# roeiherz/CanonicalSg2Im

Hardware: AMD Instinct MI355X
Metric: 256x256 images/sec/node (G+D step) (higher is better)
Workload: dtype f32; 1 GPU; BASELINE config C3: COCO-shaped AttSPADE 256x256, batch 16/GPU, 1-30 objects/img, ngf=64 ndf=64, --no_vgg_loss --use_img_disc 0; Sg2Layout GCN + SPADE G + 2-scale PatchGAN D + object-crop D, fwd+bwd+Adam; global_batch=16, parallelism=dp1

## Files before the change

canonicalsg2im_amd/_lib.py:

```python
import ctypes
import os

import torch

_HERE = os.path.dirname(os.path.abspath(__file__))
LIB_PATH = os.environ.get("CSG_HIP_LIB") or os.path.join(_HERE, "libcsg_hip.so")

MAX_TAPS = 16
ACT_NONE, ACT_LEAKY, ACT_TANH = 0, 1, 2

c_i32, c_i64, c_f32, c_f64, c_p = ctypes.c_int32, ctypes.c_int64, ctypes.c_float, ctypes.c_double, ctypes.c_void_p


class ConvDesc(ctypes.Structure):
    _fields_ = [
        ("B", c_i32), ("IHp", c_i32), ("IWp", c_i32), ("Cin", c_i32), ("x_cs", c_i32),
        ("IHv", c_i32), ("IWv", c_i32), ("in_up", c_i32),
        ("OHg", c_i32), ("OWg", c_i32), ("OHf", c_i32), ("OWf", c_i32), ("os", c_i32), ("ooy", c_i32), ("oox", c_i32),
        ("Cout", c_i32), ("y_cs", c_i32),
        ("istride", c_i32), ("ntaps", c_i32), ("wtaps", c_i32),
        ("tap_dy", c_i32 * MAX_TAPS), ("tap_dx", c_i32 * MAX_TAPS), ("tap_w", c_i32 * MAX_TAPS),
        ("act", c_i32), ("slope", c_f32), ("accumulate", c_i32), ("res_gate", c_i32),
    ]

# ... 22 lines not shown
                ("sigma", c_p), ("u_used", c_p), ("v_used", c_p), ("workspace", c_p), ("workspace_bytes", c_i64)]


class SnBwdItem(ctypes.Structure):
    _fields_ = [("dweff", c_p), ("Cout", c_i64), ("Cin", c_i64), ("KH", c_i64), ("KW", c_i64), ("s0", c_i64), ("s1", c_i64),
                ("s2", c_i64), ("s3", c_i64), ("w", c_p), ("u_used", c_p), ("v_used", c_p), ("sigma", c_p), ("dw", c_p),
                ("workspace", c_p), ("workspace_bytes", c_i64)]


class GemmDesc(ctypes.Structure):
    _fields_ = [("M", ctypes.c_int64), ("N", ctypes.c_int64), ("K", ctypes.c_int64),
                ("lda", ctypes.c_int64), ("ldb", ctypes.c_int64), ("ldy", ctypes.c_int64), ("ldg", ctypes.c_int64),
                ("act", ctypes.c_int32), ("slope", ctypes.c_float), ("gate_slope", ctypes.c_float)]


SIGNATURES = {
    "csg_version": (c_i32, []),
    "csg_last_error": (ctypes.c_char_p, []),
    "csg_prof_enable": (c_i32, [c_i32]),
    "csg_prof_reset": (c_i32, []),
    "csg_prof_num_kernels": (c_i32, []),
    "csg_prof_kernel_name": (ctypes.c_char_p, [c_i32]),
    "csg_prof_read": (c_i32, [c_i32, ctypes.POINTER(c_f64), ctypes.POINTER(c_i64), ctypes.POINTER(c_f64)]),
    "csg_embed_fwd": (c_i32, [c_p, c_i64, c_i64, c_p, c_i64, c_i64, c_p, c_i64, c_i64, c_p]),
    "csg_embed_bwd_workspace": (c_i64, [c_i64, c_i64, c_i64]),
    "csg_embed_bwd": (c_i32, [c_p, c_i64, c_i64, c_p, c_i64, c_i64, c_i64, c_i64, c_p, c_p, c_i64, c_p]),
    "csg_real_object_mask": (c_i32, [c_p, c_i64, c_i64, c_i64, c_i64, c_p, c_p]),
    "csg_graph_csr_build": (c_i32, [c_p, c_i64, c_i64, c_i64, c_p, c_p, c_p]),
    "csg_gather_concat_fwd": (c_i32, [c_p, c_p, c_p, c_i64, c_i64, c_i64, c_i64, c_i64, c_p, c_p]),
    "csg_gather_concat_bwd_workspace": (c_i64, [c_i64, c_i64, c_i64, c_i64]),
    "csg_gather_concat_bwd": (c_i32, [c_p, c_p, c_p, c_i64, c_i64, c_i64, c_i64, c_i64, c_p, c_p, c_p, c_i64, c_p]),
    "csg_segment_avg_fwd_workspace": (c_i64, [c_i64, c_i64, c_i64, c_i64]),
    "csg_segment_avg_fwd": (c_i32, [c_p, c_p, c_p, c_p, c_p, c_i64, c_i64, c_i64, c_i64, c_i64, c_p, c_p, c_p, c_p,
                                    c_i64, c_p]),
    "csg_segment_avg_bwd": (c_i32, [c_p, c_p, c_p, c_p, c_p, c_p, c_p, c_p, c_i64, c_i64, c_i64, c_i64, c_i64, c_i32,
                                    c_p, c_p, c_p, c_p]),
    "csg_layout_fwd": (c_i32, [c_p, c_p, c_p, c_p, c_i64, c_i64, c_i64, c_i64, c_i64, c_i64, c_i64, c_i64, c_p, c_i64,
                               c_i64, c_p]),
    "csg_disc_input_fwd": (c_i32, [c_p, c_p, c_p, c_p, c_i64, c_i64, c_i64, c_i64, c_i64, c_i64, c_p, c_i64, c_i64, c_i64,
                                   c_i64, c_p, c_i64, c_p]),
    "csg_layout_bwd_workspace": (c_i64, [c_i64, c_i64, c_i64, c_i64, c_i64, c_i32, c_i32]),
    "csg_layout_bwd": (c_i32, [c_p, c_i64, c_i64, c_p, c_p, c_p, c_i64, c_i64, c_i64, c_i64, c_i64, c_i64, c_i64,
                               c_i64, c_p, c_i32, c_p, c_p, c_p, c_i64, c_p]),
    "csg_layout_bwd_masks": (c_i32, [c_p, c_i64, c_i64, c_p, c_p, c_i64, c_i64, c_i64, c_i64, c_i64, c_i64, c_i64, c_i64,
                                     c_p, c_p, c_i32, c_p]),
    "csg_layout_mass": (c_i32, [c_p, c_p, c_p, c_p, c_i64, c_i64, c_i64, c_i64, c_i64, c_i64, c_p, c_p]),
    "csg_layout_paint": (c_i32, [c_p, c_p, c_p, c_i64, c_p, c_i64, c_i64, c_i64, c_i64, c_i64, c_i64, c_i64, c_p, c_i64,
                                 c_i64, c_p]),
    "csg_conv_fwd_workspace": (c_i64, [ctypes.POINTER(ConvDesc)]),
    "csg_conv_fwd": (c_i32, [ctypes.POINTER(ConvDesc), c_p, c_p, c_p, c_p, c_p, c_p, c_i64, c_p]),
    "csg_conv_bwd_weight_workspace": (c_i64, [ctypes.POINTER(ConvDesc)]),
    "csg_conv_bwd_weight": (c_i32, [ctypes.POINTER(ConvDesc), c_p, c_p, c_p, c_p, c_p, c_i64, c_p]),
    "csg_wino_pack_bytes": (c_i64, [c_i64, c_i64]),
    "csg_wino_pack_weights": (c_i32, [c_p, c_i64, c_i64, c_i64, c_i64, c_i64, c_i64, c_i32, c_p, c_p, c_p]),
    "csg_conv_fwd_multi_workspace": (c_i64, [ctypes.POINTER(ConvDesc), c_i32]),
    "csg_conv_fwd_multi": (c_i32, [ctypes.POINTER(ConvDesc), c_i32, c_p, c_p, c_p, c_p, c_p, c_p, c_i64, c_p]),
    "csg_gemm_supported": (c_i32, [ctypes.POINTER(GemmDesc)]),
    "csg_gemm_nt": (c_i32, [ctypes.POINTER(GemmDesc), c_p, c_p, c_p, c_p, c_p, c_p]),
    "csg_gemm_tn_workspace": (c_i64, [c_i64, c_i64, c_i64]),
    "csg_gemm_tn": (c_i32, [c_i64, c_i64, c_i64, c_p, c_i64, c_p, c_i64, c_p, c_p, c_p, c_i64, c_p]),
    "csg_conv_few_supported": (c_i32, [ctypes.POINTER(FewDesc)]),
    "csg_conv_few_fwd_workspace": (c_i64, [ctypes.POINTER(FewDesc)]),
    "csg_conv_few_fwd": (c_i32, [ctypes.POINTER(FewDesc), c_p, c_p, c_p, c_p, c_p, c_i64, c_p]),
    "csg_conv_few_bwd_data": (c_i32, [ctypes.POINTER(FewDesc), c_p, c_p, c_p, c_p]),
    "csg_conv_few_bwd_weight_workspace": (c_i64, [ctypes.POINTER(FewDesc)]),
    "csg_conv_few_bwd_weight": (c_i32, [ctypes.POINTER(FewDesc), c_p, c_p, c_p, c_p, c_p, c_i64, c_p]),
    "csg_wino_conv_workspace": (c_i64, [ctypes.POINTER(WinoDesc)]),
    "csg_wino_conv": (c_i32, [ctypes.POINTER(WinoDesc), c_p, c_p, c_p, c_p, c_p, c_f32, c_p, c_p, c_i64, c_p]),
    "csg_wino_bwd_weight_workspace": (c_i64, [ctypes.POINTER(WinoDesc)]),
    "csg_wino_bwd_weight": (c_i32, [ctypes.POINTER(WinoDesc), c_p, c_p, c_p, c_p, c_p, c_i64, c_p]),
    "csg_wino4_bwd_weight_workspace": (c_i64, [ctypes.POINTER(WinoDesc)]),
    "csg_wino4_bwd_weight": (c_i32, [ctypes.POINTER(WinoDesc), c_p, c_p, c_p, c_p, c_p, c_i64, c_p]),
    "csg_wino4_supported": (c_i32, [ctypes.POINTER(WinoDesc)]),
    "csg_wino4_persistent": (c_i32, [c_i32]),
    "csg_wino_pack_weights_multi": (c_i32, [ctypes.POINTER(WinoPackItem), c_i32, c_p]),
    "csg_wino4_pack_bytes": (c_i64, [c_i64, c_i64]),
    "csg_wino4_pack_weights": (c_i32, [c_p, c_i64, c_i64, c_i64, c_i64, c_i64, c_i64, c_i32, c_p, c_p, c_p]),
    "csg_wino4_conv_workspace": (c_i64, [ctypes.POINTER(WinoDesc)]),
    "csg_wino4_conv": (c_i32, [ctypes.POINTER(WinoDesc), c_p, c_p, c_p, c_p, c_p, c_f32, c_p, c_p, c_i64, c_p]),
    "csg_wino4_conv_part": (c_i32, [ctypes.POINTER(WinoDesc), c_p, c_p, c_i64, c_i64, c_p, c_p, c_p, c_i64, c_p, c_p, c_f32,
                                    c_p, c_p]),
    "csg_wino4_conv_spade_supported": (c_i32, [ctypes.POINTER(WinoDesc)]),
    "csg_wino4_conv_spade": (c_i32, [ctypes.POINTER(WinoDesc), c_p, c_p, c_p, c_p, c_p, c_i64, c_p, c_p, c_f32, c_p, c_p]),
    "csg_wino34_supported": (c_i32, [ctypes.POINTER(WinoDesc), c_i32]),
    "csg_wino34_pack_weights": (c_i32, [c_p, c_i64, c_i64, c_i64, c_i64, c_i64, c_i64, c_i32, c_p, c_p, c_p]),
    "csg_wino34_conv_workspace": (c_i64, [ctypes.POINTER(WinoDesc), c_i32]),
    "csg_wino34_conv": (c_i32, [ctypes.POINTER(WinoDesc), c_i32, c_p, c_p, c_p, c_p, c_p, c_f32, c_p, c_p, c_i64, c_p]),
    "csg_act_bwd": (c_i32, [c_p, c_p, c_i64, c_i32, c_f32, c_p, c_p]),
    "csg_colsum": (c_i32, [c_p, c_i64, c_i64, c_i64, c_p, c_p, c_i64, c_p]),
    "csg_norm_stats": (c_i32, [c_p, c_i64, c_i64, c_i64, c_p, c_p, c_i64, c_p]),
    "csg_norm_finalize": (c_i32, [c_p, c_i64, c_i64, c_f64, c_f32, c_i32, c_p, c_p, c_p, c_p, c_f32, c_p]),
    "csg_norm_stats_finalize": (c_i32, [c_p, c_i64, c_i64, c_i64, c_p, c_i64, c_f64, c_f32, c_p, c_p, c_p, c_p, c_p, c_p, c_f32,
                                        c_p]),
    "csg_norm_apply_fwd": (c_i32, [c_p, c_p, c_p, c_p, c_f32, c_i64, c_i64, c_i64, c_p, c_p, c_f32, c_p, c_p]),
    "csg_norm_apply_bwd_reduce": (c_i32, [c_p, c_p, c_p, c_p, c_p, c_p, c_f32, c_i64, c_i64, c_i64, c_p, c_p, c_p, c_i64,
                                          c_i64, c_p]),
    "csg_norm_apply_bwd_dx": (c_i32, [c_p, c_p, c_p, c_p, c_p, c_f32, c_p, c_f64, c_i64, c_i64, c_i64, c_p, c_p, c_p, c_f32,
                                      c_p, c_p, c_i64, c_p]),
    "csg_nearest_resize_fwd": (c_i32, [c_p, c_i64, c_i64, c_i64, c_i64, c_i64, c_i64, c_p, c_p]),
    "csg_nearest_resize_bwd": (c_i32, [c_p, c_i64, c_i64, c_i64, c_i64, c_i64, c_i64, c_p, c_p]),
    "csg_upsample2x_fwd": (c_i32, [c_p, c_i64, c_i64, c_i64, c_i64, c_p, c_p]),
    "csg_upsample2x_bwd": (c_i32, [c_p, c_i64, c_i64, c_i64, c_i64, c_p, c_p]),
    "csg_avgpool3s2_fwd": (c_i32, [c_p, c_i64, c_i64, c_i64, c_i64, c_p, c_p]),
    "csg_avgpool3s2_bwd": (c_i32, [c_p, c_i64, c_i64, c_i64, c_i64, c_p, c_p]),
    "csg_avgpool3s2_bwd_add": (c_i32, [c_p, c_i64, c_i64, c_i64, c_i64, c_p, c_p, c_p]),
    "csg_crop_fwd": (c_i32, [c_p, c_i64, c_i64, c_i64, c_i64, c_i64, c_p, c_p, c_i64, c_i64, c_i64, c_p, c_i64, c_p]),
    "csg_crop_bwd": (c_i32, [c_p, c_i64, c_i64, c_i64, c_i64, c_i64, c_p, c_p, c_i64, c_i64, c_i64, c_i64, c_p, c_p]),
    "csg_crop_bwd_boxes": (c_i32, [c_p, c_p, c_i64, c_i64, c_i64, c_i64, c_i64, c_p, c_p, c_i64, c_i64, c_i64, c_i64, c_p,
                                   c_p]),
    "csg_maxpool2_fwd": (c_i32, [c_p, c_i64, c_i64, c_i64, c_i64, c_p, c_p]),
    "csg_maxpool2_bwd": (c_i32, [c_p, c_p, c_i64, c_i64, c_i64, c_i64, c_p, c_p]),
    "csg_avgpool2_fwd": (c_i32, [c_p, c_i64, c_i64, c_i64, c_i64, c_p, c_p]),
    "csg_avgpool2_bwd": (c_i32, [c_p, c_i64, c_i64, c_i64, c_i64, c_p, c_p]),
    "csg_l1_mean_workspace": (c_i64, [c_i64]),
    "csg_l1_mean_fwd": (c_i32, [c_p, c_p, c_i64, c_p, c_p, c_i64, c_p]),
    "csg_l1_mean_bwd": (c_i32, [c_p, c_p, c_p, c_i64, c_p, c_p]),
    "csg_hinge_mean_fwd": (c_i32, [ctypes.POINTER(HingeItem), c_i32, c_i32, c_p, c_p]),
    "csg_hinge_mean_bwd": (c_i32, [ctypes.POINTER(HingeItem), c_i32, c_i32, c_p, c_p]),
    "csg_spectral_norm_workspace": (c_i64, [c_i64, c_i64]),
    "csg_spectral_norm_fwd": (c_i32, [c_p, c_p, c_p, c_i64, c_i64, c_i32, c_f32, c_p, c_i64, c_p, c_p, c_p, c_p, c_i64,
                                      c_p]),
    "csg_spectral_norm_bwd": (c_i32, [c_p, c_i64, c_i64, c_i64, c_i64, c_i64, c_i64, c_i64, c_i64, c_p, c_p, c_p, c_p,
                                      c_p, c_p, c_i64, c_p]),
    "csg_spectral_norm_fwd_multi": (c_i32, [ctypes.POINTER(SnFwdItem), c_i32, c_i32, c_f32, c_p]),
    "csg_spectral_norm_bwd_multi": (c_i32, [ctypes.POINTER(SnBwdItem), c_i32, c_p]),
    "csg_canon_workspace": (c_i64, [c_i64]),
    "csg_canon_build": (c_i32, [c_p, c_p, c_p, c_p, c_i64, c_i64, ctypes.POINTER(c_i32), c_i64, c_i32, c_i32, c_p, c_i64,
                                c_p, c_p]),
    "csg_canon_emit": (c_i32, [c_p, c_p, c_i64, c_i64, ctypes.POINTER(c_i32), c_i64, c_i32, c_i32, c_p, c_p, c_i64, c_p,
                               c_p, c_p]),
    "csg_canon_converse": (c_i32, [c_p, c_p, c_i64, c_i64, ctypes.POINTER(c_i32), c_i64, c_i32, c_i32, c_p, c_p, c_p, c_p,
                                   c_i64, c_p, c_p, c_p]),
    "csg_canon_general_workspace": (c_i64, [c_i64, c_i64, c_i64]),
    "csg_canon_general_build": (c_i32, [c_p, c_p, c_p, c_p, c_i64, c_i64, c_p, c_p, c_i64, ctypes.POINTER(c_i32), c_i64,
                                        c_i64, c_i32, c_p, c_i64, c_p, c_p]),
    "csg_canon_general_converse": (c_i32, [c_i64, ctypes.POINTER(c_i32), c_i64, c_p, c_i64, c_p, c_p, c_p, c_p, c_p]),
    "csg_canon_general_close": (c_i32, [c_i64, ctypes.POINTER(c_i32), c_i64, c_i32, c_p, c_i64, c_p, c_p]),
    "csg_canon_general_emit": (c_i32, [c_i64, ctypes.POINTER(c_i32), c_i64, c_p, c_i64, c_p, c_i64, c_p, c_p, c_p]),
}


def _load():
    if not os.path.exists(LIB_PATH):
        raise ImportError(
            "libcsg_hip.so is not built (%s). Run `python -c 'import __graft_entry__ as g; g.build()'` "
            "from the repository root; there is no CPU fallback." % LIB_PATH)
    lib = ctypes.CDLL(LIB_PATH)
    for name, (res, args) in SIGNATURES.items():
        fn = getattr(lib, name)
        fn.restype = res
        fn.argtypes = args
    return lib


lib = _load()


def last_error():
    return lib.csg_last_error().decode("utf-8", "replace")


def check(rc, what=""):
    if rc != 0:
        raise RuntimeError("libcsg_hip %s failed (%d): %s" % (what, rc, last_error()))


# ... 35 lines not shown
```

canonicalsg2im_amd/csrc/csg_api.hip:

```cpp
#include <stdarg.h>
#include <string.h>

#include <mutex>
#include <vector>

#include "csg_common.h"

namespace csg {

static thread_local char g_err[512] = "";

void set_error(const char* fmt, ...) {
  va_list ap;
  va_start(ap, fmt);
  vsnprintf(g_err, sizeof(g_err), fmt, ap);
  va_end(ap);
}

int check_launch(const char* what) {
  hipError_t e = hipGetLastError();
  if (e != hipSuccess) {
    set_error("%s: %s", what, hipGetErrorString(e));
    return CSG_E_LAUNCH;
  }
// ... 22 lines not shown
      return true;
    default:
      return false;
  }
}

bool prof_on(int kid) {
  return g_prof == 1 || (g_prof == 2 && (kid == K_IGEMM_FWD || kid == K_WINO_CONV || kid == K_WINO4_CONV)) ||
         (g_prof == 3 && hbm_kernel(kid));
}

bool prof_serialize() { return g_prof == 1 || g_prof == 3; }

ProfCur& prof_cur() {
  static thread_local ProfCur cur = {0, 0.0, false, false};
  return cur;
}

static hipEvent_t get_event() {
  std::lock_guard<std::mutex> lk(g_mu);
  if (!g_free.empty()) {
    hipEvent_t e = g_free.back();
    g_free.pop_back();
    return e;
  }
  hipEvent_t e;
  hipEventCreate(&e);
  return e;
}

void prof_begin(int kid, double work) {
  ProfCur& c = prof_cur();
  c.kid = kid;
  c.work = work;
  c.armed = true;
  c.used = false;
}

void prof_next(hipEvent_t& e0, hipEvent_t& e1) {
  ProfCur& c = prof_cur();
  e0 = get_event();
  e1 = get_event();
  std::lock_guard<std::mutex> lk(g_mu);
  g_pending.push_back(Rec{c.kid, c.used ? 0.0 : c.work, e0, e1, !c.used});
  c.used = true;
}

void prof_end() {
  ProfCur& c = prof_cur();
  c.armed = c.used = false;
}

static void resolve() {
  std::lock_guard<std::mutex> lk(g_mu);
  for (auto& r : g_pending) {
    hipEventSynchronize(r.e1);
    float ms = 0.f;
    hipEventElapsedTime(&ms, r.e0, r.e1);
    g_ms[r.kid] += ms;
    g_work[r.kid] += r.work;
    g_n[r.kid] += r.first ? 1 : 0;
    g_free.push_back(r.e0);
    g_free.push_back(r.e1);
  }
  g_pending.clear();
}

static const char* kNames[K_COUNT] = {
    "embed_fwd",      "embed_bwd",      "real_object_mask", "graph_csr_build", "gather_concat_fwd", "gather_concat_bwd",
    "segment_avg_fwd", "segment_avg_bwd", "layout_fwd",       "layout_bwd",      "igemm_fwd",         "igemm_fwd64",   "splitk_epilogue", "igemm_wgrad",
    "wgrad_reduce",   "act_bwd",        "colsum",           "norm_stats",      "norm_finalize",     "norm_apply_fwd",
    "norm_bwd_reduce", "norm_bwd_dx",    "upsample2x_fwd",   "upsample2x_bwd",  "avgpool3s2_fwd",    "avgpool3s2_bwd", "crop_fwd", "crop_bwd",
    "maxpool2_fwd",   "maxpool2_bwd",   "l1_mean_fwd",      "l1_mean_bwd",
    "canon_build",    "canon_emit",     "spectral_norm_fwd", "spectral_norm_bwd",
    "wino_conv",      "wino_pack",      "wino_wgrad",
    "few_fwd",        "few_bwd_data",   "few_bwd_weight",
    "wino4_conv",     "wino4_wgrad",
    "gemm_nt",        "gemm_tn"};

}

extern "C" {

int csg_version(void) { return 109; }
const char* csg_last_error(void) { return csg::g_err; }

int csg_prof_enable(int on) {
  csg::resolve();
  csg::g_prof = on < 0 ? 0 : (on > 3 ? 1 : on);
  return CSG_OK;
}

int csg_prof_reset(void) {
  csg::resolve();
  memset(csg::g_ms, 0, sizeof(csg::g_ms));
  memset(csg::g_work, 0, sizeof(csg::g_work));
  memset(csg::g_n, 0, sizeof(csg::g_n));
  return CSG_OK;
}

int csg_prof_num_kernels(void) { return csg::K_COUNT; }

const char* csg_prof_kernel_name(int kid) {
  if (kid < 0 || kid >= csg::K_COUNT) return "";
  return csg::kNames[kid];
}

int csg_prof_read(int kid, double* ms, int64_t* launches, double* work) {
  CSG_REQUIRE(kid >= 0 && kid < csg::K_COUNT, CSG_E_BADSHAPE, "csg_prof_read: bad kernel id %d", kid);
  csg::resolve();
  if (ms) *ms = csg::g_ms[kid];
  if (launches) *launches = csg::g_n[kid];
  if (work) *work = csg::g_work[kid];
  return CSG_OK;
}

}
```

canonicalsg2im_amd/csrc/norm.hip:

```cpp
#include "csg_common.h"

using namespace csg;

__device__ __forceinline__ float4 f4(float v) { return make_float4(v, v, v, v); }
__device__ __forceinline__ float4 ld4(const float* p) { return *(const float4*)p; }
__device__ __forceinline__ void st4(float* p, float4 v) { *(float4*)p = v; }
__device__ __forceinline__ float lrelu(float v, float s) { return v > 0.f ? v : v * s; }
__device__ __forceinline__ float lrelu_g(float pre, float s) { return pre > 0.f ? 1.f : s; }

struct d4 {
  double x, y, z, w;
};
__device__ __forceinline__ d4 d4zero() { return d4{0.0, 0.0, 0.0, 0.0}; }

__global__ __launch_bounds__(256) void k_norm_stats_partial(const float* __restrict__ x, int64_t P, int C,
                                                             int64_t x_cs, int nchunk, double* __restrict__ partial) {
  extern __shared__ __attribute__((aligned(16))) double smd[];
  const int tid = threadIdx.x;
  const int chunk = blockIdx.x, g = blockIdx.y;
  const int64_t per = (P + nchunk - 1) / nchunk;
  const int64_t p0 = chunk * per, p1 = min(P, p0 + per);
  const int Q = C >> 2;
  double* out = partial + ((int64_t)g * nchunk + chunk) * 2 * C;
  for (int qb = 0; qb < Q; qb += 256) {
    const int Qc = min(256, Q - qb);
    const int R = 256 / Qc;
    const int q = tid % Qc, rr = tid / Qc;
    d4 s = d4zero(), ss = d4zero();
    if (rr < R) {
      const float* xp = x + ((int64_t)g * P) * x_cs + (qb + q) * 4;
      int64_t p = p0 + rr;
      for (; p + 3 * R < p1; p += 4 * R) {
        float4 v[4];
#pragma unroll
        for (int u = 0; u < 4; ++u) v[u] = ld4(xp + (p + u * R) * x_cs);
#pragma unroll
        for (int u = 0; u < 4; ++u) {
          const double a = v[u].x, b = v[u].y, c = v[u].z, d = v[u].w;
          s.x += a; s.y += b; s.z += c; s.w += d;
          ss.x += a * a; ss.y += b * b; ss.z += c * c; ss.w += d * d;
        }
      }
      for (; p < p1; p += R) {
        const float4 v = ld4(xp + p * x_cs);
        const double a = v.x, b = v.y, c = v.z, d = v.w;
        s.x += a; s.y += b; s.z += c; s.w += d;
        ss.x += a * a; ss.y += b * b; ss.z += c * c; ss.w += d * d;
      }
      double* o = &smd[(rr * Qc + q) * 8];
      o[0] = s.x; o[1] = s.y; o[2] = s.z; o[3] = s.w;
      o[4] = ss.x; o[5] = ss.y; o[6] = ss.z; o[7] = ss.w;
    }
    __syncthreads();
    if (tid < Qc) {
      double a[8] = {0, 0, 0, 0, 0, 0, 0, 0};
      for (int r = 0; r < R; ++r)
#pragma unroll
        for (int e = 0; e < 8; ++e) a[e] += smd[(r * Qc + tid) * 8 + e];
#pragma unroll
      for (int e = 0; e < 4; ++e) {
        out[(qb + tid) * 4 + e] = a[e];
        out[C + (qb + tid) * 4 + e] = a[4 + e];
      }
    }
    __syncthreads();
  }
}

template <typename OutT>
__global__ __launch_bounds__(256) void k_partial_reduce(const double* __restrict__ partial, int ncols, int nchunk,
                                                         int out_cols, OutT* __restrict__ out) {
  __shared__ double sm[8][32];
  const int cl = threadIdx.x & 31, rl = threadIdx.x >> 5;
  const int j = blockIdx.x * 32 + cl, g = blockIdx.y;
  double a = 0.0;
  if (j < out_cols) {
    const double* p = partial + (int64_t)g * nchunk * ncols + j;
    int c = rl;
    for (; c + 24 < nchunk; c += 32) {
      const double v0 = p[(int64_t)c * ncols], v1 = p[(int64_t)(c + 8) * ncols];
      const double v2 = p[(int64_t)(c + 16) * ncols], v3 = p[(int64_t)(c + 24) * ncols];
      a += v0;
      a += v1;
      a += v2;
      a += v3;
    }
    for (; c < nchunk; c += 8) a += p[(int64_t)c * ncols];
  }
  sm[rl][cl] = a;
  __syncthreads();
  if (rl == 0 && j < out_cols) {
    double t = 0.0;
#pragma unroll
    for (int r = 0; r < 8; ++r) t += sm[r][cl];
    out[(int64_t)g * out_cols + j] = (OutT)t;
  }
}

__global__ __launch_bounds__(256) void k_partial_reduce_finalize(const double* __restrict__ partial, int C, int nchunk,
                                                                  double count, float eps, float* __restrict__ mean,
                                                                  float* __restrict__ invstd, float* __restrict__ rmean,
                                                                  float* __restrict__ rvar, float* __restrict__ rmean2,
                                                                  float* __restrict__ rvar2, float momentum) {
  __shared__ double sm[8][32];
  __shared__ double tot[32];
  const int cl = threadIdx.x & 31, rl = threadIdx.x >> 5;
  const int g = blockIdx.y, c = blockIdx.x * 16 + (cl & 15);
  const int ncols = 2 * C;
  const int j = (cl < 16 ? 0 : C) + c;
  double a = 0.0;
  if (c < C) {
    const double* p = partial + (int64_t)g * nchunk * ncols + j;
    int k = rl;
    for (; k + 24 < nchunk; k += 32) {
      const double v0 = p[(int64_t)k * ncols], v1 = p[(int64_t)(k + 8) * ncols];
      const double v2 = p[(int64_t)(k + 16) * ncols], v3 = p[(int64_t)(k + 24) * ncols];
      a += v0;
      a += v1;
      a += v2;
      a += v3;
    }
    for (; k < nchunk; k += 8) a += p[(int64_t)k * ncols];
  }
  sm[rl][cl] = a;
  __syncthreads();
  if (rl == 0) {
    double t = 0.0;
#pragma unroll
    for (int r = 0; r < 8; ++r) t += sm[r][cl];
    tot[cl] = t;
  }
  __syncthreads();
  if (threadIdx.x < 16 && c < C) {
    const double S = tot[threadIdx.x], SS = tot[threadIdx.x + 16];
    const double m = S / count;
    double var = (SS - S * m) / count;
    if (var < 0.0) var = 0.0;
    const float fv = (float)var;
    mean[(int64_t)g * C + c] = (float)m;
    invstd[(int64_t)g * C + c] = 1.0f / sqrtf(fv + eps);
    if (g == 0) {
      const double unb = count > 1.0 ? var * count / (count - 1.0) : var;
      if (rmean != nullptr) {
        rmean[c] = (1.0f - momentum) * rmean[c] + momentum * (float)m;
        rvar[c] = (1.0f - momentum) * rvar[c] + momentum * (float)unb;
      }
      if (rmean2 != nullptr) {
        rmean2[c] = (1.0f - momentum) * rmean2[c] + momentum * (float)m;
        rvar2[c] = (1.0f - momentum) * rvar2[c] + momentum * (float)unb;
      }
    }
  }
}

__global__ void k_norm_finalize(const double* __restrict__ sums, int G, int C, double count, float eps, int mode,
                                float* __restrict__ mean, float* __restrict__ invstd, float* __restrict__ rmean,
                                float* __restrict__ rvar, float momentum) {
  int i = blockIdx.x * blockDim.x + threadIdx.x;
  if (i >= G * C) return;
  int g = i / C, c = i - g * C;
  double S = sums[(int64_t)g * 2 * C + c], SS = sums[(int64_t)g * 2 * C + C + c];
  double m = S / count;
  double var = (SS - S * m) / count;
  if (var < 0.0) var = 0.0;
  float fv = (float)var;
  float is = (mode == 1) ? 1.0f / sqrtf(fmaxf(fv, eps)) : 1.0f / sqrtf(fv + eps);
  mean[i] = (float)m;
  invstd[i] = is;
  if (rmean != nullptr && g == 0) {
    double unb = count > 1.0 ? var * count / (count - 1.0) : var;
    rmean[c] = (1.0f - momentum) * rmean[c] + momentum * (float)m;
    rvar[c] = (1.0f - momentum) * rvar[c] + momentum * (float)unb;
  }
}

__global__ __launch_bounds__(256) void k_norm_apply_fwd(const float* __restrict__ x, const float* __restrict__ mean,
                                                         const float* __restrict__ invstd,
                                                         const float* __restrict__ gb, float slope, int64_t P, int C,
                                                         int64_t n4, float* __restrict__ y,
                                                         const float* __restrict__ gb2, float slope2,
                                                         float* __restrict__ y2) {
  const int Q = C >> 2;
#pragma unroll 2
  for (int64_t e = (int64_t)blockIdx.x * blockDim.x + threadIdx.x; e < n4; e += (int64_t)gridDim.x * blockDim.x) {
    const int64_t pix = e / Q;
    const int q = (int)(e - pix * Q);
    const int64_t g = pix / P;
    float4 v = ld4(x + e * 4);
    const float4 m = ld4(mean + g * C + q * 4), r = ld4(invstd + g * C + q * 4);
    v.x = (v.x - m.x) * r.x; v.y = (v.y - m.y) * r.y; v.z = (v.z - m.z) * r.z; v.w = (v.w - m.w) * r.w;
    if (y2 != nullptr) {
      const float4 ga = ld4(gb2 + pix * 2 * C + q * 4), be = ld4(gb2 + pix * 2 * C + C + q * 4);
      float4 u = make_float4(v.x * (1.f + ga.x) + be.x, v.y * (1.f + ga.y) + be.y, v.z * (1.f + ga.z) + be.z,
                             v.w * (1.f + ga.w) + be.w);
      if (slope2 != 1.0f) { u.x = lrelu(u.x, slope2); u.y = lrelu(u.y, slope2); u.z = lrelu(u.z, slope2); u.w = lrelu(u.w, slope2); }
      st4(y2 + e * 4, u);
    }
    if (gb != nullptr) {
      const float4 ga = ld4(gb + pix * 2 * C + q * 4), be = ld4(gb + pix * 2 * C + C + q * 4);
      v.x = v.x * (1.f + ga.x) + be.x; v.y = v.y * (1.f + ga.y) + be.y;
      v.z = v.z * (1.f + ga.z) + be.z; v.w = v.w * (1.f + ga.w) + be.w;
    }
    if (slope != 1.0f) { v.x = lrelu(v.x, slope); v.y = lrelu(v.y, slope); v.z = lrelu(v.z, slope); v.w = lrelu(v.w, slope); }
    st4(y + e * 4, v);
  }
}

__global__ __launch_bounds__(256) void k_norm_bwd_reduce(const float* __restrict__ dy, const float* __restrict__ x,
                                                          const float* __restrict__ mean,
                                                          const float* __restrict__ invstd,
                                                          const float* __restrict__ gb,
                                                          const float* __restrict__ yact, float slope, int64_t P, int C,
                                                          int nchunk, float* __restrict__ dgb,
                                                          double* __restrict__ partial, int gcs) {
  extern __shared__ __attribute__((aligned(16))) double smd[];
  const int tid = threadIdx.x;
  const int chunk = blockIdx.x, g = blockIdx.y;
  const int64_t per = (P + nchunk - 1) / nchunk;
  const int64_t p0 = chunk * per, p1 = min(P, p0 + per);
  const int Q = C >> 2;
  double* out = partial + ((int64_t)g * nchunk + chunk) * 2 * C;
  for (int qb = 0; qb < Q; qb += 256) {
    const int Qc = min(256, Q - qb);
    const int R = 256 / Qc;
    const int q = tid % Qc, rr = tid / Qc;
    d4 s = d4zero(), ss = d4zero();
    if (rr < R) {
      const int co = (qb + q) * 4;
      const float4 m = ld4(mean + (int64_t)g * C + co), r = ld4(invstd + (int64_t)g * C + co);
#pragma unroll 2
      for (int64_t p = p0 + rr; p < p1; p += R) {
        const int64_t pix = (int64_t)g * P + p;
        const float4 xv = ld4(x + pix * C + co);
        float4 d = ld4(dy + pix * C + co);
        float4 xh = make_float4((xv.x - m.x) * r.x, (xv.y - m.y) * r.y, (xv.z - m.z) * r.z, (xv.w - m.w) * r.w);
        float4 dn = d;
        if (gb != nullptr) {
          const float4 ga = ld4(gb + pix * gcs + co);
          if (slope != 1.0f) {
            if (yact != nullptr) {
              const float4 yv = ld4(yact + pix * C + co);
              d.x *= lrelu_g(yv.x, slope); d.y *= lrelu_g(yv.y, slope); d.z *= lrelu_g(yv.z, slope); d.w *= lrelu_g(yv.w, slope);
            } else {
              const float4 be = ld4(gb + pix * gcs + C + co);
              d.x *= lrelu_g(xh.x * (1.f + ga.x) + be.x, slope); d.y *= lrelu_g(xh.y * (1.f + ga.y) + be.y, slope);
              d.z *= lrelu_g(xh.z * (1.f + ga.z) + be.z, slope); d.w *= lrelu_g(xh.w * (1.f + ga.w) + be.w, slope);
            }
          }
          st4(dgb + pix * 2 * C + co, make_float4(d.x * xh.x, d.y * xh.y, d.z * xh.z, d.w * xh.w));
          st4(dgb + pix * 2 * C + C + co, d);
          dn = make_float4(d.x * (1.f + ga.x), d.y * (1.f + ga.y), d.z * (1.f + ga.z), d.w * (1.f + ga.w));
        } else if (slope != 1.0f) {
          dn.x *= lrelu_g(xh.x, slope); dn.y *= lrelu_g(xh.y, slope); dn.z *= lrelu_g(xh.z, slope); dn.w *= lrelu_g(xh.w, slope);
        }
        s.x += dn.x; s.y += dn.y; s.z += dn.z; s.w += dn.w;
        ss.x += (double)dn.x * xh.x; ss.y += (double)dn.y * xh.y; ss.z += (double)dn.z * xh.z; ss.w += (double)dn.w * xh.w;
      }
      double* o = &smd[(rr * Qc + q) * 8];
      o[0] = s.x; o[1] = s.y; o[2] = s.z; o[3] = s.w;
      o[4] = ss.x; o[5] = ss.y; o[6] = ss.z; o[7] = ss.w;
    }
    __syncthreads();
    if (tid < Qc) {
      double a[8] = {0, 0, 0, 0, 0, 0, 0, 0};
      for (int r = 0; r < R; ++r)
#pragma unroll
        for (int e = 0; e < 8; ++e) a[e] += smd[(r * Qc + tid) * 8 + e];
#pragma unroll
      for (int e = 0; e < 4; ++e) {
        out[(qb + tid) * 4 + e] = a[e];
        out[C + (qb + tid) * 4 + e] = a[4 + e];
      }
    }
    __syncthreads();
  }
}

__global__ __launch_bounds__(256) void k_norm_bwd_dx(const float* __restrict__ dy, const float* __restrict__ x,
                                                      const float* __restrict__ mean, const float* __restrict__ invstd,
                                                      const float* __restrict__ gb, float slope,
                                                      const double* __restrict__ dsums, double inv_count, int64_t P,
                                                      int C, int64_t n4, float* __restrict__ dx,
                                                      const float* __restrict__ dy2, const float* __restrict__ gb2,
                                                      float slope2, const float* __restrict__ dgb,
                                                      const float* __restrict__ dgb2, int gcs) {
  const int Q = C >> 2;
#pragma unroll 2
  for (int64_t e = (int64_t)blockIdx.x * blockDim.x + threadIdx.x; e < n4; e += (int64_t)gridDim.x * blockDim.x) {
    const int64_t pix = e / Q;
    const int q = (int)(e - pix * Q);
    const int64_t g = pix / P;
    const int co = q * 4;
    const float4 xv = ld4(x + e * 4);
    float4 d = (gb != nullptr && dgb != nullptr) ? make_float4(0.f, 0.f, 0.f, 0.f) : ld4(dy + e * 4);
    const float4 m = ld4(mean + g * C + co), r = ld4(invstd + g * C + co);
    const float4 xh = make_float4((xv.x - m.x) * r.x, (xv.y - m.y) * r.y, (xv.z - m.z) * r.z, (xv.w - m.w) * r.w);
    float4 dn = d;
    if (gb != nullptr && dgb != nullptr) {
      const float4 ga = ld4(gb + pix * gcs + co);
      d = ld4(dgb + pix * 2 * C + C + co);
      dn = make_float4(d.x * (1.f + ga.x), d.y * (1.f + ga.y), d.z * (1.f + ga.z), d.w * (1.f + ga.w));
    } else if (gb != nullptr) {
      const float4 ga = ld4(gb + pix * gcs + co);
      if (slope != 1.0f) {
        const float4 be = ld4(gb + pix * gcs + C + co);
        d.x *= lrelu_g(xh.x * (1.f + ga.x) + be.x, slope); d.y *= lrelu_g(xh.y * (1.f + ga.y) + be.y, slope);
        d.z *= lrelu_g(xh.z * (1.f + ga.z) + be.z, slope); d.w *= lrelu_g(xh.w * (1.f + ga.w) + be.w, slope);
      }
      dn = make_float4(d.x * (1.f + ga.x), d.y * (1.f + ga.y), d.z * (1.f + ga.z), d.w * (1.f + ga.w));
    } else if (slope != 1.0f) {
      dn.x *= lrelu_g(xh.x, slope); dn.y *= lrelu_g(xh.y, slope); dn.z *= lrelu_g(xh.z, slope); dn.w *= lrelu_g(xh.w, slope);
    }
    if (dy2 != nullptr) {
      const float4 ga = ld4(gb2 + pix * gcs + co);
      float4 d2 = dgb2 != nullptr ? ld4(dgb2 + pix * 2 * C + C + co) : ld4(dy2 + e * 4);
      if (slope2 != 1.0f && dgb2 == nullptr) {
        const float4 be = ld4(gb2 + pix * gcs + C + co);
        d2.x *= lrelu_g(xh.x * (1.f + ga.x) + be.x, slope2); d2.y *= lrelu_g(xh.y * (1.f + ga.y) + be.y, slope2);
        d2.z *= lrelu_g(xh.z * (1.f + ga.z) + be.z, slope2); d2.w *= lrelu_g(xh.w * (1.f + ga.w) + be.w, slope2);
      }
      dn.x += d2.x * (1.f + ga.x); dn.y += d2.y * (1.f + ga.y); dn.z += d2.z * (1.f + ga.z); dn.w += d2.w * (1.f + ga.w);
    }
    const double* ds = dsums + g * 2 * C;
    float4 a = make_float4((float)(ds[co] * inv_count), (float)(ds[co + 1] * inv_count), (float)(ds[co + 2] * inv_count),
                           (float)(ds[co + 3] * inv_count));
    float4 b = make_float4((float)(ds[C + co] * inv_count), (float)(ds[C + co + 1] * inv_count),
                           (float)(ds[C + co + 2] * inv_count), (float)(ds[C + co + 3] * inv_count));
    float4 o;
    o.x = r.x * (dn.x - a.x - xh.x * b.x); o.y = r.y * (dn.y - a.y - xh.y * b.y);
    o.z = r.z * (dn.z - a.z - xh.z * b.z); o.w = r.w * (dn.w - a.w - xh.w * b.w);
    st4(dx + e * 4, o);
  }
}

__global__ void k_act_bwd(const float* __restrict__ dy, const float* __restrict__ y, int64_t n, int act, float slope,
                          float* __restrict__ dpre) {
  for (int64_t i = (int64_t)blockIdx.x * blockDim.x + threadIdx.x; i < n; i += (int64_t)gridDim.x * blockDim.x) {
    float g = dy[i], v = y[i];
    if (act == CSG_ACT_LEAKY)
      g *= (v > 0.f ? 1.f : slope);
    else if (act == CSG_ACT_TANH)
      g *= (1.f - v * v);
    dpre[i] = g;
  }
}

__device__ __forceinline__ int nearest_src(int dst, float scale, int in) { return min((int)floorf(dst * scale), in - 1); }

__global__ void k_nearest_fwd(const float* __restrict__ x, int IH, int IW, int OH, int OW, int Q, float sy, float sx,
                              int64_t n4, float* __restrict__ y) {
  for (int64_t e = (int64_t)blockIdx.x * blockDim.x + threadIdx.x; e < n4; e += (int64_t)gridDim.x * blockDim.x) {
    const int64_t pix = e / Q;
    const int q = (int)(e - pix * Q);
    const int X = (int)(pix % OW);
    const int64_t t = pix / OW;
    const int Y = (int)(t % OH);
    const int64_t b = t / OH;
    st4(y + e * 4, ld4(x + (((b * IH + nearest_src(Y, sy, IH)) * IW + nearest_src(X, sx, IW)) * (int64_t)Q + q) * 4));
  }
}

__global__ void k_nearest_bwd(const float* __restrict__ dy, int IH, int IW, int OH, int OW, int Q, float sy, float sx,
                              int64_t n4, float* __restrict__ dx) {
  for (int64_t e = (int64_t)blockIdx.x * blockDim.x + threadIdx.x; e < n4; e += (int64_t)gridDim.x * blockDim.x) {
    const int64_t pix = e / Q;
    const int q = (int)(e - pix * Q);
    const int ix = (int)(pix % IW);
    const int64_t t = pix / IW;
    const int iy = (int)(t % IH);
    const int64_t b = t / IH;
    int y0 = max(0, (int)((float)iy / sy) - 2), x0 = max(0, (int)((float)ix / sx) - 2);
    while (y0 < OH && nearest_src(y0, sy, IH) < iy) ++y0;
    while (x0 < OW && nearest_src(x0, sx, IW) < ix) ++x0;
    float4 acc = make_float4(0.f, 0.f, 0.f, 0.f);
    for (int Y = y0; Y < OH && nearest_src(Y, sy, IH) == iy; ++Y)
      for (int X = x0; X < OW && nearest_src(X, sx, IW) == ix; ++X) {
        const float4 g = ld4(dy + (((b * OH + Y) * OW + X) * (int64_t)Q + q) * 4);
        acc.x += g.x; acc.y += g.y; acc.z += g.z; acc.w += g.w;
      }
    st4(dx + e * 4, acc);
  }
}

__global__ void k_upsample2x_fwd(const float* __restrict__ x, int H, int W, int Q, int64_t n4, float* __restrict__ y) {
  for (int64_t e = (int64_t)blockIdx.x * blockDim.x + threadIdx.x; e < n4; e += (int64_t)gridDim.x * blockDim.x) {
    int64_t pix = e / Q;
    int q = (int)(e - pix * Q);
    int X = (int)(pix % (2 * W));
    int64_t t = pix / (2 * W);
    int Y = (int)(t % (2 * H));
    int64_t b = t / (2 * H);
    st4(y + e * 4, ld4(x + (((b * H + (Y >> 1)) * W + (X >> 1)) * (int64_t)Q + q) * 4));
  }
}

__global__ void k_upsample2x_bwd(const float* __restrict__ dy, int H, int W, int Q, int64_t n4,
                                 float* __restrict__ dx) {
  for (int64_t e = (int64_t)blockIdx.x * blockDim.x + threadIdx.x; e < n4; e += (int64_t)gridDim.x * blockDim.x) {
    int64_t pix = e / Q;
    int q = (int)(e - pix * Q);
    int xw = (int)(pix % W);
    int64_t t = pix / W;
    int yh = (int)(t % H);
    int64_t b = t / H;
    const float* base = dy + (((b * 2 * H + 2 * yh) * 2 * W + 2 * xw) * (int64_t)Q + q) * 4;
    const int64_t rs = (int64_t)2 * W * Q * 4;
    float4 a = ld4(base), c = ld4(base + Q * 4), d = ld4(base + rs), f = ld4(base + rs + Q * 4);
    st4(dx + e * 4, make_float4(a.x + c.x + d.x + f.x, a.y + c.y + d.y + f.y, a.z + c.z + d.z + f.z, a.w + c.w + d.w + f.w));
  }
}

__global__ void k_avgpool3s2_fwd(const float* __restrict__ x, int H, int W, int OH, int OW, int Q, int64_t n4,
                                 float* __restrict__ y) {
  for (int64_t e = (int64_t)blockIdx.x * blockDim.x + threadIdx.x; e < n4; e += (int64_t)gridDim.x * blockDim.x) {
    int64_t pix = e / Q;
    int q = (int)(e - pix * Q);
    int ox = (int)(pix % OW);
// ... 16 lines not shown
    float inv = 1.0f / (float)cnt;
    st4(y + e * 4, make_float4(a.x * inv, a.y * inv, a.z * inv, a.w * inv));
  }
}

__device__ __forceinline__ int win_count(int o, int n) {
  int lo = o * 2 - 1, hi = o * 2 + 1;
  if (lo < 0) lo = 0;
  if (hi > n - 1) hi = n - 1;
  return hi - lo + 1;
}

__global__ void k_avgpool3s2_bwd(const float* __restrict__ dy, int H, int W, int OH, int OW, int Q, int64_t n4,
                                 const float* add, float* dx) {
  for (int64_t e = (int64_t)blockIdx.x * blockDim.x + threadIdx.x; e < n4; e += (int64_t)gridDim.x * blockDim.x) {
    int64_t pix = e / Q;
    int q = (int)(e - pix * Q);
    int ix = (int)(pix % W);
    int64_t t = pix / W;
    int iy = (int)(t % H);
    int64_t b = t / H;
    float4 a = f4(0.f);
    for (int oy = iy / 2; oy <= (iy + 1) / 2; ++oy) {
      if (oy < 0 || oy >= OH) continue;
      int cy = win_count(oy, H);
      for (int ox = ix / 2; ox <= (ix + 1) / 2; ++ox) {
        if (ox < 0 || ox >= OW) continue;
        float inv = 1.0f / (float)(cy * win_count(ox, W));
        float4 v = ld4(dy + (((b * OH + oy) * OW + ox) * (int64_t)Q + q) * 4);
        a.x += v.x * inv; a.y += v.y * inv; a.z += v.z * inv; a.w += v.w * inv;
      }
    }
    if (add != nullptr) {
      const float4 o = ld4(add + e * 4);
      a.x += o.x; a.y += o.y; a.z += o.z; a.w += o.w;
    }
    st4(dx + e * 4, a);
  }
}

static inline unsigned ew_grid(int64_t n) {
  int64_t g = cdiv(n, 256);
  if (g > 256 * 16) g = 256 * 16;
  if (g < 1) g = 1;
  return (unsigned)g;
}

extern "C" {

int csg_norm_stats(const float* x, int64_t G, int64_t P, int64_t C, double* sums, double* partial, int64_t nchunk,
                   void* stream) {
  CSG_REQUIRE(G > 0 && P > 0 && C > 0 && C % 4 == 0, CSG_E_BADSHAPE, "csg_norm_stats: bad shape G=%ld P=%ld C=%ld",
              (long)G, (long)P, (long)C);
  CSG_REQUIRE(nchunk >= 1 && nchunk <= 65535 && G <= 65535, CSG_E_BADSHAPE, "csg_norm_stats: bad nchunk");
  hipStream_t s = (hipStream_t)stream;
  {
    ProfScope p(K_NORM_STATS, (double)G * P * C * 4, s);
    CSG_LAUNCH(k_norm_stats_partial, dim3((unsigned)nchunk, (unsigned)G), dim3(256), 256 * 8 * 8, s, x, P,
                       (int)C, C, (int)nchunk, partial);
  }
  CSG_LAUNCH(k_partial_reduce<double>, dim3((unsigned)cdiv(2 * C, 32), (unsigned)G), dim3(256), 0, s, partial,
                     (int)(2 * C), (int)nchunk, (int)(2 * C), sums);
  return check_launch("csg_norm_stats");
}

int csg_norm_stats_finalize(const float* x, int64_t G, int64_t P, int64_t C, double* partial, int64_t nchunk, double count,
                            float eps, float* mean, float* invstd, float* running_mean, float* running_var,
                            float* running_mean2, float* running_var2, float momentum, void* stream) {
  CSG_REQUIRE(G > 0 && P > 0 && C > 0 && C % 4 == 0 && count > 0, CSG_E_BADSHAPE,
              "csg_norm_stats_finalize: bad shape G=%ld P=%ld C=%ld", (long)G, (long)P, (long)C);
  CSG_REQUIRE(nchunk >= 1 && nchunk <= 65535 && G <= 65535, CSG_E_BADSHAPE, "csg_norm_stats_finalize: bad nchunk");
  CSG_REQUIRE((running_mean == nullptr && running_mean2 == nullptr) || G == 1, CSG_E_UNSUPPORTED,
              "csg_norm_stats_finalize: running stats need G == 1");
  CSG_REQUIRE((running_mean == nullptr) == (running_var == nullptr) && (running_mean2 == nullptr) == (running_var2 == nullptr),
              CSG_E_BADSHAPE, "csg_norm_stats_finalize: running mean and variance come together");
  hipStream_t s = (hipStream_t)stream;
  {
    ProfScope p(K_NORM_STATS, (double)G * P * C * 4, s);
    CSG_LAUNCH(k_norm_stats_partial, dim3((unsigned)nchunk, (unsigned)G), dim3(256), 256 * 8 * 8, s, x, P, (int)C, C,
               (int)nchunk, partial);
  }
  ProfScope p(K_NORM_FINALIZE, (double)G * C * 24, s);
  CSG_LAUNCH(k_partial_reduce_finalize, dim3((unsigned)cdiv(C, 16), (unsigned)G), dim3(256), 0, s, partial, (int)C, (int)nchunk,
             count, eps, mean, invstd, running_mean, running_var, running_mean2, running_var2, momentum);
  return check_launch("csg_norm_stats_finalize");
}

int csg_norm_finalize(const double* sums, int64_t G, int64_t C, double count, float eps, int32_t mode, float* mean,
                      float* invstd, float* running_mean, float* running_var, float momentum, void* stream) {
  CSG_REQUIRE(G > 0 && C > 0 && count > 0, CSG_E_BADSHAPE, "csg_norm_finalize: bad shape");
  CSG_REQUIRE(running_mean == nullptr || G == 1, CSG_E_UNSUPPORTED, "csg_norm_finalize: running stats need G == 1");
  hipStream_t s = (hipStream_t)stream;
  ProfScope p(K_NORM_FINALIZE, (double)G * C * 24, s);
  CSG_LAUNCH(k_norm_finalize, dim3((unsigned)cdiv(G * C, 256)), dim3(256), 0, s, sums, (int)G, (int)C, count,
                     eps, mode, mean, invstd, running_mean, running_var, momentum);
  return check_launch("csg_norm_finalize");
}

int csg_norm_apply_fwd(const float* x, const float* mean, const float* invstd, const float* gb, float slope,
                       int64_t G, int64_t P, int64_t C, float* y, const float* gb2, float slope2, float* y2,
                       void* stream) {
  CSG_REQUIRE(G > 0 && P > 0 && C > 0 && C % 4 == 0, CSG_E_BADSHAPE, "csg_norm_apply_fwd: bad shape");
  CSG_REQUIRE((gb2 == nullptr) == (y2 == nullptr), CSG_E_BADSHAPE, "csg_norm_apply_fwd: gb2 and y2 come together");
  hipStream_t s = (hipStream_t)stream;
  const int64_t n4 = G * P * C / 4;
  ProfScope p(K_NORM_APPLY_FWD, (double)G * P * C * 4 * ((gb ? 4 : 2) + (y2 ? 3 : 0)), s);
  CSG_LAUNCH(k_norm_apply_fwd, dim3(ew_grid(n4)), dim3(256), 0, s, x, mean, invstd, gb, slope, P, (int)C, n4, y, gb2,
                     slope2, y2);
  return check_launch("csg_norm_apply_fwd");
}

int csg_norm_apply_bwd_reduce(const float* dy, const float* x, const float* mean, const float* invstd,
                              const float* gb, const float* yact, float slope, int64_t G, int64_t P, int64_t C, float* dgb,
                              double* dsums, double* partial, int64_t nchunk, int64_t gb_cs, void* stream) {
  CSG_REQUIRE(yact == nullptr || gb != nullptr, CSG_E_BADSHAPE, "csg_norm_apply_bwd_reduce: yact goes with a modulation");
  CSG_REQUIRE(gb == nullptr || gb_cs == 2 * C || (gb_cs == C && yact != nullptr), CSG_E_BADSHAPE,
              "csg_norm_apply_bwd_reduce: gb_cs is 2C ([gamma | beta]) or, with yact, C (gamma only)");
  CSG_REQUIRE(G > 0 && P > 0 && C > 0 && C % 4 == 0, CSG_E_BADSHAPE, "csg_norm_apply_bwd_reduce: bad shape");
  CSG_REQUIRE((gb == nullptr) == (dgb == nullptr), CSG_E_BADSHAPE, "csg_norm_apply_bwd_reduce: gb/dgb mismatch");
  CSG_REQUIRE(nchunk >= 1 && nchunk <= 65535 && G <= 65535, CSG_E_BADSHAPE, "csg_norm_apply_bwd_reduce: bad nchunk");
  hipStream_t s = (hipStream_t)stream;
  {
    ProfScope p(K_NORM_BWD_REDUCE, (double)G * P * C * 4 * (gb ? 6 : 2), s);
    CSG_LAUNCH(k_norm_bwd_reduce, dim3((unsigned)nchunk, (unsigned)G), dim3(256), 256 * 8 * 8, s, dy, x, mean,
                       invstd, gb, yact, slope, P, (int)C, (int)nchunk, dgb, partial, (int)gb_cs);
  }
  CSG_LAUNCH(k_partial_reduce<double>, dim3((unsigned)cdiv(2 * C, 32), (unsigned)G), dim3(256), 0, s, partial,
                     (int)(2 * C), (int)nchunk, (int)(2 * C), dsums);
  return check_launch("csg_norm_apply_bwd_reduce");
}

int csg_norm_apply_bwd_dx(const float* dy, const float* x, const float* mean, const float* invstd, const float* gb,
                          float slope, const double* dsums, double count, int64_t G, int64_t P, int64_t C, float* dx,
                          const float* dy2, const float* gb2, float slope2, const float* dgb, const float* dgb2,
                          int64_t gb_cs, void* stream) {
  CSG_REQUIRE(G > 0 && P > 0 && C > 0 && C % 4 == 0 && count > 0, CSG_E_BADSHAPE, "csg_norm_apply_bwd_dx: bad shape");
  CSG_REQUIRE(gb == nullptr || gb_cs == 2 * C || (gb_cs == C && dgb != nullptr && (gb2 == nullptr || dgb2 != nullptr)),
              CSG_E_BADSHAPE, "csg_norm_apply_bwd_dx: gb_cs is 2C ([gamma | beta]) or, with dgb (and dgb2), C (gamma only)");
  CSG_REQUIRE((dy2 == nullptr) == (gb2 == nullptr), CSG_E_BADSHAPE, "csg_norm_apply_bwd_dx: dy2 and gb2 come together");
  hipStream_t s = (hipStream_t)stream;
  const int64_t n4 = G * P * C / 4;
  ProfScope p(K_NORM_BWD_DX, (double)G * P * C * 4 * ((gb ? (dgb ? 4 : 5) : 3) + (dy2 ? (dgb2 ? 2 : 3) : 0)), s);
  CSG_LAUNCH(k_norm_bwd_dx, dim3(ew_grid(n4)), dim3(256), 0, s, dy, x, mean, invstd, gb, slope, dsums,
                     1.0 / count, P, (int)C, n4, dx, dy2, gb2, slope2, dgb, dgb2, (int)gb_cs);
  return check_launch("csg_norm_apply_bwd_dx");
}

int csg_act_bwd(const float* dy, const float* y, int64_t n, int32_t act, float slope, float* dpre, void* stream) {
  CSG_REQUIRE(n >= 0, CSG_E_BADSHAPE, "csg_act_bwd: bad n");
  if (n == 0) return CSG_OK;
  hipStream_t s = (hipStream_t)stream;
  ProfScope p(K_ACT_BWD, (double)n * 12, s);
  CSG_LAUNCH(k_act_bwd, dim3(ew_grid(n)), dim3(256), 0, s, dy, y, n, act, slope, dpre);
  return check_launch("csg_act_bwd");
}

int csg_colsum(const float* x, int64_t rows, int64_t C, int64_t x_cs, float* out, double* partial, int64_t nchunk,
               void* stream) {
  CSG_REQUIRE(rows > 0 && C > 0 && C % 4 == 0 && x_cs % 4 == 0, CSG_E_BADSHAPE, "csg_colsum: bad shape");
  CSG_REQUIRE(nchunk >= 1 && nchunk <= 65535, CSG_E_BADSHAPE, "csg_colsum: bad nchunk");
  hipStream_t s = (hipStream_t)stream;
  ProfScope p(K_COLSUM, (double)rows * C * 4, s);
  CSG_LAUNCH(k_norm_stats_partial, dim3((unsigned)nchunk, 1), dim3(256), 256 * 8 * 8, s, x, rows, (int)C, x_cs,
                     (int)nchunk, partial);
  CSG_LAUNCH(k_partial_reduce<float>, dim3((unsigned)cdiv(C, 32), 1), dim3(256), 0, s, partial, (int)(2 * C),
                     (int)nchunk, (int)C, out);
  return check_launch("csg_colsum");
}

int csg_nearest_resize_fwd(const float* x, int64_t B, int64_t IH, int64_t IW, int64_t C, int64_t OH, int64_t OW, float* y,
                           void* stream) {
  CSG_REQUIRE(B > 0 && IH > 0 && IW > 0 && OH > 0 && OW > 0 && C > 0 && C % 4 == 0, CSG_E_BADSHAPE,
              "csg_nearest_resize_fwd: bad shape");
  hipStream_t s = (hipStream_t)stream;
  const int64_t n4 = B * OH * OW * C / 4;
  ProfScope p(K_UPSAMPLE_FWD, (double)n4 * 32, s);
  CSG_LAUNCH(k_nearest_fwd, dim3(ew_grid(n4)), dim3(256), 0, s, x, (int)IH, (int)IW, (int)OH, (int)OW, (int)(C / 4),
             (float)IH / (float)OH, (float)IW / (float)OW, n4, y);
  return check_launch("csg_nearest_resize_fwd");
}

int csg_nearest_resize_bwd(const float* dy, int64_t B, int64_t IH, int64_t IW, int64_t C, int64_t OH, int64_t OW, float* dx,
                           void* stream) {
  CSG_REQUIRE(B > 0 && IH > 0 && IW > 0 && OH > 0 && OW > 0 && C > 0 && C % 4 == 0, CSG_E_BADSHAPE,
              "csg_nearest_resize_bwd: bad shape");
  hipStream_t s = (hipStream_t)stream;
  const int64_t n4 = B * IH * IW * C / 4;
  ProfScope p(K_UPSAMPLE_BWD, (double)(n4 + B * OH * OW * C / 4) * 16, s);
  CSG_LAUNCH(k_nearest_bwd, dim3(ew_grid(n4)), dim3(256), 0, s, dy, (int)IH, (int)IW, (int)OH, (int)OW, (int)(C / 4),
             (float)IH / (float)OH, (float)IW / (float)OW, n4, dx);
  return check_launch("csg_nearest_resize_bwd");
}

int csg_upsample2x_fwd(const float* x, int64_t B, int64_t H, int64_t W, int64_t C, float* y, void* stream) {
  CSG_REQUIRE(B > 0 && H > 0 && W > 0 && C > 0 && C % 4 == 0, CSG_E_BADSHAPE, "csg_upsample2x_fwd: bad shape");
  hipStream_t s = (hipStream_t)stream;
  const int64_t n4 = B * 4 * H * W * C / 4;
  ProfScope p(K_UPSAMPLE_FWD, (double)n4 * 16 * 1.25, s);
  CSG_LAUNCH(k_upsample2x_fwd, dim3(ew_grid(n4)), dim3(256), 0, s, x, (int)H, (int)W, (int)(C / 4), n4, y);
  return check_launch("csg_upsample2x_fwd");
}

int csg_upsample2x_bwd(const float* dy, int64_t B, int64_t H, int64_t W, int64_t C, float* dx, void* stream) {
  CSG_REQUIRE(B > 0 && H > 0 && W > 0 && C > 0 && C % 4 == 0, CSG_E_BADSHAPE, "csg_upsample2x_bwd: bad shape");
  hipStream_t s = (hipStream_t)stream;
  const int64_t n4 = B * H * W * C / 4;
  ProfScope p(K_UPSAMPLE_BWD, (double)n4 * 16 * 5, s);
  CSG_LAUNCH(k_upsample2x_bwd, dim3(ew_grid(n4)), dim3(256), 0, s, dy, (int)H, (int)W, (int)(C / 4), n4, dx);
  return check_launch("csg_upsample2x_bwd");
}

int csg_avgpool3s2_fwd(const float* x, int64_t B, int64_t H, int64_t W, int64_t C, float* y, void* stream) {
  CSG_REQUIRE(B > 0 && H > 0 && W > 0 && C > 0 && C % 4 == 0, CSG_E_BADSHAPE, "csg_avgpool3s2_fwd: bad shape");
  hipStream_t s = (hipStream_t)stream;
  const int64_t OH = (H - 1) / 2 + 1, OW = (W - 1) / 2 + 1;
  const int64_t n4 = B * OH * OW * C / 4;
  ProfScope p(K_AVGPOOL_FWD, (double)(B * H * W * C + n4 * 4) * 4, s);
  CSG_LAUNCH(k_avgpool3s2_fwd, dim3(ew_grid(n4)), dim3(256), 0, s, x, (int)H, (int)W, (int)OH, (int)OW,
                     (int)(C / 4), n4, y);
  return check_launch("csg_avgpool3s2_fwd");
}

static int avgpool3s2_bwd_launch(const float* dy, int64_t B, int64_t H, int64_t W, int64_t C, const float* add, float* dx,
                                 void* stream, const char* who) {
  CSG_REQUIRE(B > 0 && H > 0 && W > 0 && C > 0 && C % 4 == 0, CSG_E_BADSHAPE, "%s: bad shape", who);
  hipStream_t s = (hipStream_t)stream;
  const int64_t OH = (H - 1) / 2 + 1, OW = (W - 1) / 2 + 1;
  const int64_t n4 = B * H * W * C / 4;
  ProfScope p(K_AVGPOOL_BWD, (double)(B * H * W * C * (add != nullptr ? 2 : 1) + B * OH * OW * C) * 4, s);
  CSG_LAUNCH(k_avgpool3s2_bwd, dim3(ew_grid(n4)), dim3(256), 0, s, dy, (int)H, (int)W, (int)OH, (int)OW,
// ... 16 lines not shown
```

canonicalsg2im_amd/csrc/wino4.hip:

```cpp
#include <stddef.h>
#include <stdlib.h>

#include <type_traits>

#include "csg_buffer.h"
#include "csg_common.h"
#include "csg_pack.h"
#include "csg_reduce.h"

using namespace csg;

typedef __attribute__((ext_vector_type(16))) float f32x16;
typedef const volatile __attribute__((address_space(3))) csg_f32x2* w4_lds_cv2;

#define W4_TW 8
#define W4_TH 4
#define W4_CQ 9
#define W4_PS 8
#define W4_RSE 36
#define W4_NLD 2
#define W4_THREADS 768
#define W4_RBUF (6 * 2 * 32 * W4_RSE)

struct Wino4Params {
  int B, H, W, Cin, x_cs, Cout, y_cs;
  int Ho, Wo, pad;
  int tbx, tby;
  int nblocks;
  int NT32, Q8;
  int act;
  float slope;
  float gate_slope;
  int nt_off;
  int mod, g_cs;
  int gb_off;
  float mod_slope;
  const float* mod_mean;
  const float* mod_invstd;
  int nstage;
  int ksplit, sps;
  long long slab;
  int nitems;
};

__device__ __forceinline__ int w4_xcd_remap(int bid, int nblk) {
  const int q = nblk >> 3, r = nblk & 7;
  const int xcd = bid & 7, idx = bid >> 3;
  return (xcd < r ? xcd * (q + 1) : r * (q + 1) + (xcd - r) * q) + idx;
}


#define WP4_LD 33
template <int RT>
__device__ __forceinline__ void w4_pack_tile(const float* __restrict__ w, int64_t s_n, int64_t s_k, int64_t s_h,
                                             int64_t s_w, int flip, int N, int K, const float* __restrict__ sigma,
                                             int NT32, int Q8, float4* __restrict__ up, int qb, int nt) {
  __shared__ float g[RT][32][WP4_LD];
  const int tid = threadIdx.x;
  const bool k_fast = s_k <= s_n;
  const float sg = sigma != nullptr ? sigma[0] : 1.0f;
  const int lane = tid & 63, ql = tid >> 6;
  const int q = qb * 4 + ql;
  const int nl = lane & 31, h = lane >> 5;
  const float Gp[5] = {0.0f, 1.0f, -1.0f, 0.5f, -2.0f};
  const float Gc[5] = {1.0f, (float)(1.0 / 3.0), (float)(-1.0 / 3.0), (float)(-16.0 / 15.0), (float)(1.0 / 15.0)};
  float G[6][RT];
#pragma unroll
  for (int k = 0; k < 5; ++k) {
    float pw = 1.0f;
#pragma unroll
    for (int a = 0; a < RT; ++a) {
      G[k][a] = (float)((double)Gc[k] * (double)pw);
      pw *= Gp[k];
    }
  }
#pragma unroll
  for (int a = 0; a < RT; ++a) G[5][a] = a == RT - 1 ? 1.0f : 0.0f;
  float stage[RT * RT * 4];
#pragma unroll
  for (int it = 0; it < RT * RT * 4; ++it) {
    const int tap = it >> 2, r = tid + 256 * (it & 3);
    const int nl2 = k_fast ? (r >> 5) : (r & 31), kl = k_fast ? (r & 31) : (r >> 5);
    const int n = nt * 32 + nl2, k = qb * 32 + kl;
    const int a = tap / RT, b = tap - RT * a;
    const int aa = flip ? RT - 1 - a : a, bb = flip ? RT - 1 - b : b;
    stage[it] = (n < N && k < K) ? w[(int64_t)n * s_n + (int64_t)k * s_k + aa * s_h + bb * s_w] : 0.f;
  }
  float t[4][6][RT];
#pragma unroll
  for (int b = 0; b < RT; ++b) {
    if (b) __syncthreads();
#pragma unroll
    for (int it = 0; it < RT * 4; ++it) {
      const int a = it >> 2, r = tid + 256 * (it & 3);
      const int nl2 = k_fast ? (r >> 5) : (r & 31), kl = k_fast ? (r & 31) : (r >> 5);
      const float v = stage[(a * RT + b) * 4 + (it & 3)];
      g[a][nl2][kl] = sigma != nullptr ? v / sg : v;
    }
    __syncthreads();
#pragma unroll
    for (int e = 0; e < 4; ++e) {
      const int kl = 8 * ql + (e >> 1) * 4 + 2 * h + (e & 1);
#pragma unroll
      for (int xi = 0; xi < 6; ++xi) {
        float acc = G[xi][0] * g[0][nl][kl];
#pragma unroll
        for (int a = 1; a < RT; ++a) acc += G[xi][a] * g[a][nl][kl];
        t[e][xi][b] = acc;
      }
    }
  }
  if (q >= Q8) return;
#pragma unroll
  for (int xi = 0; xi < 6; ++xi)
#pragma unroll
    for (int nu = 0; nu < 6; ++nu) {
      float u[4];
#pragma unroll
      for (int e = 0; e < 4; ++e) {
        float acc = t[e][xi][0] * G[nu][0];
#pragma unroll
        for (int b = 1; b < RT; ++b) acc += t[e][xi][b] * G[nu][b];
        u[e] = acc;
      }
      up[(((int64_t)(xi * 6 + nu) * NT32 + nt) * Q8 + q) * 64 + lane] = make_float4(u[0], u[1], u[2], u[3]);
    }
}

template <int RT>
__global__ __launch_bounds__(256) void k_wino4_pack(const float* __restrict__ w, int64_t s_n, int64_t s_k, int64_t s_h,
                                                     int64_t s_w, int flip, int N, int K, const float* __restrict__ sigma,
                                                     int NT32, int Q8, float4* __restrict__ up) {
  w4_pack_tile<RT>(w, s_n, s_k, s_h, s_w, flip, N, K, sigma, NT32, Q8, up, blockIdx.x, blockIdx.y);
}

__global__ __launch_bounds__(256) void k_wino4_pack_multi(PackMulti pm) {
  int i = 0;
  while (i + 1 < pm.n && (int)blockIdx.x >= pm.it[i + 1].start) ++i;
  const PackMultiItem& d = pm.it[i];
  const int local = blockIdx.x - d.start, nqb = (d.Q8 + 3) >> 2;
  w4_pack_tile<3>(d.w, d.s_n, d.s_k, d.s_h, d.s_w, d.flip, d.N, d.K, nullptr, d.NT32, d.Q8, d.up, local % nqb, local / nqb);
}

__device__ __forceinline__ csg_f32x2 w4_pfma(float c, csg_f32x2 a, csg_f32x2 b) {
  return __builtin_elementwise_fma(csg_f32x2{c, c}, a, b);
}

template <int MODE, int NB>
__device__ __forceinline__ void w4_store_columns(const Wino4Params& p, const float* rbuf, int tig, int round, int nt32,
                                                 int img, int X0, int Y0, const float* __restrict__ bias,
                                                 const float* __restrict__ res, const float* __restrict__ gate,
                                                 float* __restrict__ y) {
  for (int item = tig; item < 256 * NB; item += W4_THREADS / 2) {
    const int cq = item & 7, tile = (item >> 3) & 31, bb = item >> 8;
    const int n = nt32 * 32 + cq * 4;
    const int ttx = tile & (W4_TW - 1), tty = tile >> 3;
    const int oy = Y0 + 4 * tty, ox = X0 + 4 * ttx + NB * round + bb;
    if (n < p.Cout && oy < p.Ho && ox < p.Wo) {
      csg_f32x2 lo[6], hi[6];
#pragma unroll
      for (int xi = 0; xi < 6; ++xi) {
        const csg_f32x4 r = *(const csg_f32x4*)(rbuf + ((xi * NB + bb) * 32 + tile) * W4_RSE + cq * 4);
        lo[xi] = __builtin_shufflevector(r, r, 0, 1);
        hi[xi] = __builtin_shufflevector(r, r, 2, 3);
      }
      csg_f32x2 blo = {0.f, 0.f}, bhi = {0.f, 0.f};
      if (bias != nullptr) {
        const csg_f32x4 bv = *(const csg_f32x4*)(bias + n);
        blo = __builtin_shufflevector(bv, bv, 0, 1);
        bhi = __builtin_shufflevector(bv, bv, 2, 3);
      }
      const int64_t rowstride = (int64_t)p.Wo * p.y_cs;
      const int64_t pix0 = ((int64_t)img * p.Ho + oy) * p.Wo + ox;
      int64_t off = pix0 * p.y_cs + n;
      float4 mx[4], mg[4], mm, mr;
      if (MODE == 2) {
        mm = *(const float4*)(p.mod_mean + n);
        mr = *(const float4*)(p.mod_invstd + n);
#pragma unroll
        for (int a = 0; a < 4; ++a) {
          mx[a] = *(const float4*)(res + off + a * rowstride);
          mg[a] = *(const float4*)(gate + (pix0 + (int64_t)a * p.Wo) * p.g_cs + n);
        }
      }
#pragma unroll
      for (int a = 0; a < 4; ++a, off += rowstride) {
        csg_f32x2 vl, vh;
        if (a == 0) {
          vl = ((lo[0] + lo[1]) + (lo[2] + lo[3])) + lo[4];
          vh = ((hi[0] + hi[1]) + (hi[2] + hi[3])) + hi[4];
        } else if (a == 1) {
          vl = w4_pfma(-2.0f, lo[4], w4_pfma(0.5f, lo[3], lo[1] - lo[2]));
          vh = w4_pfma(-2.0f, hi[4], w4_pfma(0.5f, hi[3], hi[1] - hi[2]));
        } else if (a == 2) {
          vl = w4_pfma(4.0f, lo[4], w4_pfma(0.25f, lo[3], lo[1] + lo[2]));
          vh = w4_pfma(4.0f, hi[4], w4_pfma(0.25f, hi[3], hi[1] + hi[2]));
        } else {
          vl = w4_pfma(-8.0f, lo[4], w4_pfma(0.125f, lo[3], lo[1] - lo[2])) + lo[5];
          vh = w4_pfma(-8.0f, hi[4], w4_pfma(0.125f, hi[3], hi[1] - hi[2])) + hi[5];
        }
        vl += blo;
        vh += bhi;
        float vv[4] = {vl.x, vl.y, vh.x, vh.y};
        if (MODE == 2) {
          const float xs[4] = {mx[a].x, mx[a].y, mx[a].z, mx[a].w}, gs[4] = {mg[a].x, mg[a].y, mg[a].z, mg[a].w};
          const float ms[4] = {mm.x, mm.y, mm.z, mm.w}, rs[4] = {mr.x, mr.y, mr.z, mr.w};
#pragma unroll
          for (int e = 0; e < 4; ++e) {
            const float xh = (xs[e] - ms[e]) * rs[e];
            float o = xh * (1.f + gs[e]) + vv[e];
            if (p.mod_slope != 1.0f) o = o > 0.f ? o : o * p.mod_slope;
            vv[e] = o;
          }
        }
        if (MODE == 1) {
#pragma unroll
          for (int e = 0; e < 4; ++e) {
            if (p.act == CSG_ACT_LEAKY)
              vv[e] = vv[e] > 0.f ? vv[e] : vv[e] * p.slope;
            else if (p.act == CSG_ACT_TANH)
              vv[e] = tanhf(vv[e]);
          }
          if (res != nullptr) {
            const float4 rv = *(const float4*)(res + off);
            vv[0] += rv.x; vv[1] += rv.y; vv[2] += rv.z; vv[3] += rv.w;
          }
          if (gate != nullptr) {
            const float4 gv = *(const float4*)(gate + off);
            vv[0] *= gv.x > 0.f ? 1.f : p.gate_slope; vv[1] *= gv.y > 0.f ? 1.f : p.gate_slope;
            vv[2] *= gv.z > 0.f ? 1.f : p.gate_slope; vv[3] *= gv.w > 0.f ? 1.f : p.gate_slope;
          }
        }
        *(float4*)(y + off) = make_float4(vv[0], vv[1], vv[2], vv[3]);
      }
    }
  }
}

__device__ __forceinline__ csg_f32x2 w4_out_row(int a, const csg_f32x2 (&m)[6]) {
  if (a == 0) return ((m[0] + m[1]) + (m[2] + m[3])) + m[4];
  if (a == 1) return w4_pfma(-2.0f, m[4], w4_pfma(0.5f, m[3], m[1] - m[2]));
  if (a == 2) return w4_pfma(4.0f, m[4], w4_pfma(0.25f, m[3], m[1] + m[2]));
  return w4_pfma(-8.0f, m[4], w4_pfma(0.125f, m[3], m[1] - m[2])) + m[5];
}
template <int NB>
__device__ __forceinline__ void w4_store_joint(const Wino4Params& p, const float* rbuf0, int tid, int round, int nb, int img,
                                               int X0, int Y0, const float* __restrict__ bias, const float* __restrict__ xin,
                                               float* __restrict__ gout, float* __restrict__ y) {
  const float* rbuf1 = rbuf0 + W4_RBUF / 2 * NB;
  for (int item = tid; item < 512 * NB; item += W4_THREADS) {
    const int cq = item & 7, tile = (item >> 3) & 31, half = (item >> 8) & 1, bb = item >> 9;
    const int n = nb * 32 + cq * 4;
    const int ttx = tile & (W4_TW - 1), tty = tile >> 3;
    const int oy = Y0 + 4 * tty, ox = X0 + 4 * ttx + NB * round + bb;
    if (oy < p.Ho && ox < p.Wo) {
      csg_f32x2 gl2[2], gh2[2], bl2[2], bh2[2];
      {
        csg_f32x2 lo[6], hi[6];
#pragma unroll
        for (int xi = 0; xi < 6; ++xi) {
          const csg_f32x4 g = *(const csg_f32x4*)(rbuf0 + ((xi * NB + bb) * 32 + tile) * W4_RSE + cq * 4);
          lo[xi] = __builtin_shufflevector(g, g, 0, 1);
          hi[xi] = __builtin_shufflevector(g, g, 2, 3);
        }
        const csg_f32x4 bg = *(const csg_f32x4*)(bias + n);
#pragma unroll
        for (int r = 0; r < 2; ++r) {
          gl2[r] = w4_out_row(2 * half + r, lo) + csg_f32x2{bg.x, bg.y};
          gh2[r] = w4_out_row(2 * half + r, hi) + csg_f32x2{bg.z, bg.w};
        }
      }
      {
        csg_f32x2 lo[6], hi[6];
#pragma unroll
        for (int xi = 0; xi < 6; ++xi) {
          const csg_f32x4 b = *(const csg_f32x4*)(rbuf1 + ((xi * NB + bb) * 32 + tile) * W4_RSE + cq * 4);
          lo[xi] = __builtin_shufflevector(b, b, 0, 1);
          hi[xi] = __builtin_shufflevector(b, b, 2, 3);
        }
        const csg_f32x4 bbv = *(const csg_f32x4*)(bias + p.Cout + n);
#pragma unroll
        for (int r = 0; r < 2; ++r) {
          bl2[r] = w4_out_row(2 * half + r, lo) + csg_f32x2{bbv.x, bbv.y};
          bh2[r] = w4_out_row(2 * half + r, hi) + csg_f32x2{bbv.z, bbv.w};
        }
      }
      const float4 mm = *(const float4*)(p.mod_mean + n), mr = *(const float4*)(p.mod_invstd + n);
      const int64_t rowstride = (int64_t)p.Wo * p.y_cs;
      const int64_t pix0 = ((int64_t)img * p.Ho + oy + 2 * half) * p.Wo + ox;
      const int64_t off = pix0 * p.y_cs + n;
      float4 mx[2];
#pragma unroll
      for (int r = 0; r < 2; ++r) mx[r] = *(const float4*)(xin + off + r * rowstride);
#pragma unroll
      for (int r = 0; r < 2; ++r) {
        const csg_f32x2 gl = gl2[r], gh = gh2[r], bl = bl2[r], bh = bh2[r];
        const float gs[4] = {gl.x, gl.y, gh.x, gh.y}, vv[4] = {bl.x, bl.y, bh.x, bh.y};
        const float xs[4] = {mx[r].x, mx[r].y, mx[r].z, mx[r].w};
        const float ms[4] = {mm.x, mm.y, mm.z, mm.w}, rs[4] = {mr.x, mr.y, mr.z, mr.w};
        float out[4];
#pragma unroll
        for (int e = 0; e < 4; ++e) {
          const float xh = (xs[e] - ms[e]) * rs[e];
          float o = xh * (1.f + gs[e]) + vv[e];
          if (p.mod_slope != 1.0f) o = o > 0.f ? o : o * p.mod_slope;
          out[e] = o;
        }
        if (gout != nullptr)
          *(float4*)(gout + (pix0 + (int64_t)r * p.Wo) * p.g_cs + n) = make_float4(gs[0], gs[1], gs[2], gs[3]);
        *(float4*)(y + off + r * rowstride) = make_float4(out[0], out[1], out[2], out[3]);
      }
    }
  }
}

template <int NB>
__device__ __forceinline__ void w4_epilogue(f32x16 (&acc)[6], const Wino4Params& p, float* rbase, int tid, int wave, int grp,
                                            int j, int h, int nt32, int img, int X0, int Y0, const float* __restrict__ bias,
                                            const float* __restrict__ res, const float* __restrict__ gate,
                                            float* __restrict__ y) {
  float* rbuf = rbase + grp * (W4_RBUF / 2 * NB);
  const int tig = tid - grp * (W4_THREADS / 2);
  const bool plain = p.act == CSG_ACT_NONE && res == nullptr && gate == nullptr;
  if (NB == 2) __syncthreads();
  csg_f32x2 rr[NB == 1 ? 4 : 1][8];
  if (NB == 1) {
#pragma unroll
    for (int ge = 0; ge < 8; ++ge) {
#define W4_M(K) csg_f32x2{acc[K][2 * ge], acc[K][2 * ge + 1]}
      const csg_f32x2 m0 = W4_M(0), m1 = W4_M(1), m2 = W4_M(2), m3 = W4_M(3), m4 = W4_M(4), m5 = W4_M(5);
#undef W4_M
      rr[0][ge] = ((m0 + m1) + (m2 + m3)) + m4;
      rr[NB == 1 ? 1 : 0][ge] = w4_pfma(-2.0f, m4, w4_pfma(0.5f, m3, m1 - m2));
      rr[NB == 1 ? 2 : 0][ge] = w4_pfma(4.0f, m4, w4_pfma(0.25f, m3, m1 + m2));
      rr[NB == 1 ? 3 : 0][ge] = w4_pfma(-8.0f, m4, w4_pfma(0.125f, m3, m1 - m2)) + m5;
    }
#pragma unroll
    for (int b = 0; b < (NB == 1 ? 4 : 1); ++b)
#pragma unroll
      for (int ge = 0; ge < 8; ++ge) asm volatile("" : "+v"(rr[b][ge]));
  }
#pragma unroll
  for (int round = 0; round < 4 / NB; ++round) {
#pragma unroll
    for (int g = 0; g < 4; ++g) {
      csg_f32x2 r0[2], r1[2];
#pragma unroll
      for (int e = 0; e < 2; ++e) {
        if (NB == 1) {
          r0[e] = rr[NB == 1 ? round : 0][2 * g + e];
          continue;
        }
#define W4_M(K) csg_f32x2{acc[K][4 * g + 2 * e], acc[K][4 * g + 2 * e + 1]}
        const csg_f32x2 m0 = W4_M(0), m1 = W4_M(1), m2 = W4_M(2), m3 = W4_M(3), m4 = W4_M(4), m5 = W4_M(5);
#undef W4_M
        const int b0 = NB * round;
        if (b0 == 0) r0[e] = ((m0 + m1) + (m2 + m3)) + m4;
        if (b0 == 2) r0[e] = w4_pfma(4.0f, m4, w4_pfma(0.25f, m3, m1 + m2));
        if (b0 == 0) r1[e] = w4_pfma(-2.0f, m4, w4_pfma(0.5f, m3, m1 - m2));
        if (b0 == 2) r1[e] = w4_pfma(-8.0f, m4, w4_pfma(0.125f, m3, m1 - m2)) + m5;
      }
      const int ch = 8 * g + 4 * h;
      *(float4*)(rbuf + ((wave * NB + 0) * 32 + j) * W4_RSE + ch) = make_float4(r0[0].x, r0[0].y, r0[1].x, r0[1].y);
      if (NB == 2)
        *(float4*)(rbuf + ((wave * NB + 1) * 32 + j) * W4_RSE + ch) = make_float4(r1[0].x, r1[0].y, r1[1].x, r1[1].y);
    }
    __syncthreads();
    if (NB == 1 && p.mod == 2)
      w4_store_joint<NB>(p, rbase, tid, round, nt32 - grp * p.gb_off, img, X0, Y0, bias, res, const_cast<float*>(gate), y);
    else if (p.mod)
      w4_store_columns<2, NB>(p, rbuf, tig, round, nt32, img, X0, Y0, bias, res, gate, y);
    else if (plain)
      w4_store_columns<0, NB>(p, rbuf, tig, round, nt32, img, X0, Y0, bias, res, gate, y);
    else
      w4_store_columns<1, NB>(p, rbuf, tig, round, nt32, img, X0, Y0, bias, res, gate, y);
    if (round + 1 < 4 / NB) __syncthreads();
// ... 283 lines not shown
  };
  auto consume = [&](auto lo_tag, auto hi_tag, int vbufsel, int s) {
#pragma unroll
    for (int nu = decltype(lo_tag)::value; nu < decltype(hi_tag)::value; ++nu) {
      const float4 v = *(const float4*)(pv + vbufsel * W4_VBUF + nu * 256);
      const int slot = nu % 3;
      acc[nu] = __builtin_amdgcn_mfma_f32_32x32x2f32(ur[slot].x, v.x, acc[nu], 0, 0, 0);
      acc[nu] = __builtin_amdgcn_mfma_f32_32x32x2f32(ur[slot].y, v.y, acc[nu], 0, 0, 0);
      acc[nu] = __builtin_amdgcn_mfma_f32_32x32x2f32(ur[slot].z, v.z, acc[nu], 0, 0, 0);
      acc[nu] = __builtin_amdgcn_mfma_f32_32x32x2f32(ur[slot].w, v.w, acc[nu], 0, 0, 0);
      if (nu < 3) load_ur(slot, nu + 3, s); else load_ur(slot, nu - 3, s + 1);
    }
  };
  constexpr int SPLIT = 3;
  auto stage = [&](int s, auto par_tag) {
    constexpr int par = decltype(par_tag)::value;
    typedef std::integral_constant<int, 0> I0;
    typedef std::integral_constant<int, SPLIT> IS;
    typedef std::integral_constant<int, 6> I6;
    consume(I0(), IS(), par, s);
    __builtin_amdgcn_sched_barrier(0);
    if (s + 1 < s_end) produce(par ^ 1, par ^ 1);
    __builtin_amdgcn_sched_barrier(0);
    consume(IS(), I6(), par, s);
    store_stage(smem + W4V_RAW0 + par * W4_BUFW);
    __syncthreads();
    load_stage(s + 3);
  };

  y += (long long)split * p.slab;
  {
    const uint2 go = *(const uint2*)W4_TAB(0);
    const csg_f32x4 a0 = csg_buf_load_x4(rsX, (int)go.x, s_begin * (W4_PS * 4), 0);
    const csg_f32x4 a1 = csg_buf_load_x4(rsX, (int)go.y, s_begin * (W4_PS * 4), 0);
    load_stage(s_begin + 1);
#pragma unroll
    for (int nu = 0; nu < 3; ++nu) load_ur(nu, nu, s_begin);
    const csg_f32x4 b0 = st[0], b1 = st[1];
    st[0] = a0;
    st[1] = a1;
    store_stage(smem + W4V_RAW0);
    __syncthreads();
    st[0] = b0;
    st[1] = b1;
    produce(0, 0);
    store_stage(smem + W4V_RAW0 + W4_BUFW);
    __syncthreads();
    load_stage(s_begin + 2);
  }
  for (;;) {
#pragma unroll
    for (int nu = 0; nu < 6; ++nu)
#pragma unroll
      for (int e = 0; e < 16; ++e) acc[nu][e] = 0.f;
    bool more = false;
    int item_n = 0;
    int nb_n = nb, img_n = img, X0_n = X0, Y0_n = Y0;
    if (P) {
      const int nb_c = nb, img_c = img, X0_c = X0, Y0_c = Y0;
      more = v + v_step < v_hi;
      item_n = more ? v + v_step : v;
      if (more) decode(item_n);
      fill_plan(W4_TAB(tsel ^ 1), more);
      nt32 = p.gb_off ? nb + grp * p.gb_off : nb * 2 + grp;
      ubase_nxt = u_tile();
      nb_n = nb; img_n = img; X0_n = X0; Y0_n = Y0;
      nb = nb_c; img = img_c; X0 = X0_c; Y0 = Y0_c;
      nt32 = p.gb_off ? nb + grp * p.gb_off : nb * 2 + grp;
    }
    int s = s_begin;
    for (; s + 1 < s_end; s += 2) {
      stage(s, std::integral_constant<int, 0>());
      stage(s + 1, std::integral_constant<int, 1>());
    }
    if (s < s_end) stage(s, std::integral_constant<int, 0>());
    if (T == 4 && P) {
      int tid_o = (int)(s_tab - (unsigned*)(smem + W4V_OFFTAB)) >> 2;
      asm volatile("" : "+v"(tid_o));
      w4_kernargs_ptr ka = (w4_kernargs_ptr)__builtin_amdgcn_kernarg_segment_ptr();
      asm volatile("" : "+s"(ka));
      Wino4Params pe = p;
#define W4_F(f) pe.f = ka->p.f;
      W4_F(Cout) W4_F(y_cs) W4_F(Ho) W4_F(Wo) W4_F(act) W4_F(slope) W4_F(gate_slope) W4_F(mod) W4_F(g_cs) W4_F(gb_off) W4_F(mod_slope)
      W4_F(mod_mean) W4_F(mod_invstd)
#undef W4_F
      w4_epilogue<1>(acc, pe, smem + W4V_V0, tid_o, wave, grp, tid_o & 31, (tid_o >> 5) & 1, nt32, img, X0, Y0, ka->bias,
                     ka->res, ka->gate, ka->y);
    } else if (T == 4) {
      w4_epilogue<2>(acc, p, smem, tid, wave, grp, j, h, nt32, img, X0, Y0, bias, res, gate, y);
    } else {
      w3_epilogue(acc, p, smem, tid, wave, grp, j, h, nt32, img, X0, Y0, bias, res, gate, y);
    }
    if (!P || !more) break;
    v = item_n;
    nb = nb_n; img = img_n; X0 = X0_n; Y0 = Y0_n;
    nt32 = p.gb_off ? nb + grp * p.gb_off : nb * 2 + grp;
    ubase = ubase_nxt;
    tsel ^= 1;
    __syncthreads();
    produce(0, 0);
    __syncthreads();
  }
#undef W4_TAB
}

static int w4_plan(const csg_wino_desc* d, int T, int pad, Wino4Params& p, size_t& shm, const char* who) {
  CSG_REQUIRE(d != nullptr, CSG_E_BADSHAPE, "%s: null descriptor", who);
  CSG_REQUIRE(d->B > 0 && d->H > 0 && d->W > 0 && d->Cin > 0 && d->Cout > 0, CSG_E_BADSHAPE, "%s: non-positive dimension", who);
  if (T == 4)
    CSG_REQUIRE(d->H % 4 == 0 && d->W % 4 == 0 && d->W >= 32 && d->H >= 16, CSG_E_UNSUPPORTED,
                "%s: F(4x4,3x3) needs H=%d, W=%d multiples of 4, W >= 32, H >= 16", who, d->H, d->W);
  else
    CSG_REQUIRE((pad == 1 || pad == 2) && d->H + 2 * pad >= 4 && d->W + 2 * pad >= 4, CSG_E_UNSUPPORTED,
                "%s: F(3x3,4x4) serves pad 1 or 2 (got %d) on maps of at least 4 - 2 pad pixels", who, pad);
  const int Ho = T == 4 ? d->H : d->H + 2 * pad - 3, Wo = T == 4 ? d->W : d->W + 2 * pad - 3;
  CSG_REQUIRE(d->Cin % 8 == 0 && d->x_cs % 4 == 0 && d->x_cs >= d->Cin && d->Cout % 4 == 0 && d->y_cs % 4 == 0 &&
                  d->y_cs >= d->Cout,
              CSG_E_UNSUPPORTED, "%s: Cin must be a multiple of 8, the other channel counts and strides of 4", who);
  CSG_REQUIRE((int64_t)d->B * (d->H + 1) * (d->W + 1) * (int64_t)(d->x_cs > d->y_cs ? d->x_cs : d->y_cs) * 4 < CSG_MAX_RECORDS,
              CSG_E_UNSUPPORTED, "%s: tensor too large for 32-bit byte offsets", who);
  CSG_REQUIRE((int64_t)36 * ((d->Cout + 31) / 32) * ((d->Cin + 7) / 8) * 1024 < CSG_MAX_RECORDS, CSG_E_UNSUPPORTED,
              "%s: packed weights too large for 32-bit byte offsets", who);
  p.B = d->B; p.H = d->H; p.W = d->W; p.Cin = d->Cin; p.x_cs = d->x_cs; p.Cout = d->Cout; p.y_cs = d->y_cs;
  p.Ho = Ho; p.Wo = Wo; p.pad = pad;
  p.tbx = (Wo + T * W4_TW - 1) / (T * W4_TW);
  p.tby = (Ho + T * W4_TH - 1) / (T * W4_TH);
  p.nblocks = (d->Cout + 63) / 64;
  p.NT32 = (d->Cout + 31) / 32;
  p.Q8 = (d->Cin + 7) / 8;
  p.act = d->act; p.slope = d->slope; p.gate_slope = 0.f;
  p.nt_off = 0; p.mod = 0; p.g_cs = 0; p.gb_off = 0; p.mod_slope = 1.f; p.mod_mean = nullptr; p.mod_invstd = nullptr;
  p.nstage = d->Cin / W4_PS;
  p.ksplit = 1;
  p.sps = p.nstage;
  p.slab = (long long)d->B * Ho * Wo * d->y_cs;
  p.nitems = 0;
  shm = (size_t)((T == 4 ? W4Geo<4>::OFFTAB : W4Geo<3>::OFFTAB) + W4_THREADS * 4) * 4;
  return CSG_OK;
}

template <int T, bool P>
static int w4_set_lds_limit(const char* who) {
  static DeviceOnce attr_once;
  int dev = 0;
  (void)hipGetDevice(&dev);
  if (attr_once.pending(dev)) {
    hipError_t e = hipFuncSetAttribute((const void*)k_wino4_conv_v<T, P>, hipFuncAttributeMaxDynamicSharedMemorySize,
                                       (P ? 160 : 128) * 1024);
    CSG_REQUIRE(e == hipSuccess, CSG_E_LAUNCH, "%s: cannot raise the dynamic LDS limit: %s", who, hipGetErrorString(e));
    attr_once.mark(dev);
  }
  return CSG_OK;
}

static std::atomic<int> w4_persist_on{-1};
static int w4_persistent_blocks(const Wino4Params& p, int64_t items) {
  static std::atomic<int> cus[32];
  int on = w4_persist_on.load(std::memory_order_relaxed);
  if (on < 0) {
    on = getenv("CSG_WINO4_PERSIST") ? atoi(getenv("CSG_WINO4_PERSIST")) : 1;
    int expect = -1;
    w4_persist_on.compare_exchange_strong(expect, on);
    on = w4_persist_on.load(std::memory_order_relaxed);
  }
  int dev = 0;
  (void)hipGetDevice(&dev);
  if (!on || dev < 0) return 0;
  int ncu = dev < 32 ? cus[dev].load(std::memory_order_relaxed) : 0;
  if (ncu == 0) {
    if (hipDeviceGetAttribute(&ncu, hipDeviceAttributeMultiprocessorCount, dev) != hipSuccess || ncu < 8) ncu = -1;
    if (dev < 32) cus[dev].store(ncu, std::memory_order_relaxed);
  }
  const int g = ncu > 0 ? (ncu & ~7) : 0;
  if (g == 0 || p.ksplit != 1 || (p.nstage & 1) || p.nstage < 4 || (p.gb_off == 0 && (p.Cout & 63)) || items < 2 * (int64_t)g) return 0;
  return g;
}

template <int T>
static int w4_launch(Wino4Params& p, size_t shm, int kid, double flops, const float* x, const float* packed,
                     const float* bias, const float* residual, const float* gate, float* y, float* workspace,
                     float* y_final, hipStream_t s, const char* who) {
  CSG_REQUIRE(shm <= 128 * 1024, CSG_E_UNSUPPORTED, "%s: %zu bytes of LDS", who, shm);
  const int64_t grid = (int64_t)p.B * p.tby * p.tbx * p.nblocks * p.ksplit;
  CSG_REQUIRE(grid < (1ll << 31), CSG_E_UNSUPPORTED, "%s: grid too large", who);
  p.nitems = (int)grid;
  const int pblocks = T == 4 ? w4_persistent_blocks(p, grid) : 0;
  int rc = pblocks ? w4_set_lds_limit<4, true>(who) : w4_set_lds_limit<T, false>(who);
  if (rc) return rc;
  ProfScope ps(kid, flops, s);
  if (pblocks)
    CSG_LAUNCH((k_wino4_conv_v<4, true>), dim3((unsigned)pblocks), dim3(W4_THREADS), shm + W4_THREADS * 16, s, p, x,
               (const float4*)packed, bias, residual, gate, y);
  else
    CSG_LAUNCH((k_wino4_conv_v<T, false>), dim3((unsigned)grid), dim3(W4_THREADS), shm, s, p, x, (const float4*)packed, bias,
               residual, gate, y);
  rc = check_launch(who);
  if (rc == CSG_OK && p.ksplit > 1) {
    launch_slab_reduce(workspace, p.slab, y_final, nullptr, 0, nullptr, p.ksplit, s);
    rc = check_launch("csg_wino4_conv(slab sum)");
  }
  return rc;
}

static void w4_split_plan(Wino4Params& p, bool plain) {
  if (!plain || p.y_cs != p.Cout) return;
  const int64_t blocks = (int64_t)p.B * p.tby * p.tbx * p.nblocks;
  if (blocks >= 384 || p.nstage < 32) return;
  int ks = (int)((512 + blocks - 1) / blocks);
  if (ks > p.nstage / 16) ks = p.nstage / 16;
  if (ks < 2) return;
  p.sps = (p.nstage + ks - 1) / ks;
  p.ksplit = (p.nstage + p.sps - 1) / p.sps;
}

// ... 93 lines not shown
  const int64_t N = backward_data ? Cin : Cout, K = backward_data ? Cout : Cin;
  const int64_t s_n = backward_data ? s_i : s_o, s_k = backward_data ? s_o : s_i;
  const int NT32 = (int)cdiv(N, 32), Q8 = (int)cdiv(K, 8);
  const int64_t total = (int64_t)36 * NT32 * Q8 * 64;
  hipStream_t s = (hipStream_t)stream;
  ProfScope ps(K_WINO_PACK, (double)Cout * Cin * 16 * 4 + (double)total * 16, s);
  CSG_LAUNCH(k_wino4_pack<4>, dim3((unsigned)cdiv(Q8, 4), (unsigned)NT32), dim3(256), 0, s, w, s_n, s_k, s_h, s_w,
                     backward_data ? 1 : 0, (int)N, (int)K, sigma, NT32, Q8, (float4*)packed);
  return check_launch("csg_wino34_pack_weights");
}

int32_t csg_wino34_supported(const csg_wino_desc* d, int32_t pad) {
  static const int on = getenv("CSG_WINO34") ? atoi(getenv("CSG_WINO34")) : 1;
  if (!on || d == nullptr) return 0;
  return ((pad == 1 || pad == 2) && d->H >= 15 && d->W >= 15 && d->Cin % 8 == 0 && d->Cout % 4 == 0 && d->Cin >= 64 &&
          d->Cout >= 32) ? 1 : 0;
}

int64_t csg_wino34_conv_workspace(const csg_wino_desc* d, int32_t pad) {
  Wino4Params p;
  size_t shm = 0;
  if (w4_plan(d, 3, pad, p, shm, "csg_wino34_conv_workspace")) return -1;
  w4_split_plan(p, d->act == CSG_ACT_NONE);
  return p.ksplit > 1 ? (int64_t)p.ksplit * p.slab * 4 : 0;
}

int csg_wino34_conv(const csg_wino_desc* d, int32_t pad, const float* x, const float* packed, const float* bias,
                    const float* residual, const float* gate, float gate_slope, float* y, float* workspace,
                    int64_t workspace_bytes, void* stream) {
  Wino4Params p;
  size_t shm = 0;
  int rc = w4_plan(d, 3, pad, p, shm, "csg_wino34_conv");
  if (rc) return rc;
  w4_split_plan(p, d->act == CSG_ACT_NONE && bias == nullptr && residual == nullptr && gate == nullptr);
  p.gate_slope = gate_slope;
  if (p.ksplit > 1 && (workspace == nullptr || workspace_bytes < (int64_t)p.ksplit * p.slab * 4)) {
    p.ksplit = 1;
    p.sps = p.nstage;
  }
  float* const y_final = y;
  if (p.ksplit > 1) {
    CSG_REQUIRE(((uintptr_t)workspace % 16) == 0, CSG_E_UNSUPPORTED, "csg_wino34_conv: workspace must be 16-byte aligned");
    y = workspace;
  }
  CSG_REQUIRE(((uintptr_t)x % 16) == 0 && ((uintptr_t)packed % 16) == 0 && ((uintptr_t)y % 16) == 0 &&
                  (gate == nullptr || ((uintptr_t)gate % 16) == 0),
              CSG_E_UNSUPPORTED, "csg_wino34_conv: pointers must be 16-byte aligned");
  return w4_launch<3>(p, shm, K_WINO4_CONV, 2.0 * p.B * p.Ho * p.Wo * 16.0 * p.Cin * p.Cout, x, packed, bias, residual, gate,
                      y, workspace, y_final, (hipStream_t)stream, "csg_wino34_conv");
}

int64_t csg_wino4_conv_workspace(const csg_wino_desc* d) {
  Wino4Params p;
  size_t shm = 0;
  if (w4_plan(d, 4, 1, p, shm, "csg_wino4_conv_workspace")) return -1;
  w4_split_plan(p, d->act == CSG_ACT_NONE);
  return p.ksplit > 1 ? (int64_t)p.ksplit * p.slab * 4 : 0;
}

int csg_wino4_conv(const csg_wino_desc* d, const float* x, const float* packed, const float* bias, const float* residual,
                   const float* gate, float gate_slope, float* y, float* workspace, int64_t workspace_bytes, void* stream) {
  Wino4Params p;
  size_t shm = 0;
  int rc = w4_plan(d, 4, 1, p, shm, "csg_wino4_conv");
  if (rc) return rc;
  w4_split_plan(p, d->act == CSG_ACT_NONE && bias == nullptr && residual == nullptr && gate == nullptr);
  p.gate_slope = gate_slope;
  CSG_REQUIRE(gate == nullptr || ((uintptr_t)gate % 16) == 0, CSG_E_UNSUPPORTED, "csg_wino4_conv: gate must be 16-byte aligned");
  if (p.ksplit > 1 && (workspace == nullptr || workspace_bytes < (int64_t)p.ksplit * p.slab * 4)) {
    p.ksplit = 1;
    p.sps = p.nstage;
  }
  float* const y_final = y;
  if (p.ksplit > 1) {
    CSG_REQUIRE(((uintptr_t)workspace % 16) == 0, CSG_E_UNSUPPORTED, "csg_wino4_conv: workspace must be 16-byte aligned");
    y = workspace;
  }
  CSG_REQUIRE(((uintptr_t)x % 16) == 0 && ((uintptr_t)packed % 16) == 0 && ((uintptr_t)y % 16) == 0, CSG_E_UNSUPPORTED,
              "csg_wino4_conv: pointers must be 16-byte aligned");
  return w4_launch<4>(p, shm, K_WINO4_CONV, 2.0 * p.B * p.H * p.W * 9.0 * p.Cin * p.Cout, x, packed, bias, residual, gate, y,
                      workspace, y_final, (hipStream_t)stream, "csg_wino4_conv");
}

int csg_wino4_conv_part(const csg_wino_desc* d, const float* x, const float* packed, int64_t tile_off, int64_t tiles_total,
                        const float* bias, const float* mod_x, const float* mod_gamma, int64_t gamma_cs,
                        const float* mod_mean, const float* mod_invstd, float mod_slope, float* y, void* stream) {
  Wino4Params p;
  size_t shm = 0;
  int rc = w4_plan(d, 4, 1, p, shm, "csg_wino4_conv_part");
  if (rc) return rc;
  CSG_REQUIRE(d->act == CSG_ACT_NONE, CSG_E_UNSUPPORTED, "csg_wino4_conv_part: no activation (the modulation has its own)");
  CSG_REQUIRE(tile_off >= 0 && tiles_total >= tile_off + p.NT32 && d->Cout % 32 == 0, CSG_E_BADSHAPE,
              "csg_wino4_conv_part: tiles [%ld, %ld) of %ld with Cout=%d", (long)tile_off, (long)(tile_off + p.NT32),
              (long)tiles_total, d->Cout);
  CSG_REQUIRE((int64_t)36 * tiles_total * p.Q8 * 1024 < CSG_MAX_RECORDS, CSG_E_UNSUPPORTED,
              "csg_wino4_conv_part: packed weights too large for 32-bit byte offsets");
  p.nt_off = (int)tile_off;
  p.NT32 = (int)tiles_total;
  if (mod_x != nullptr) {
    CSG_REQUIRE(mod_gamma != nullptr && mod_mean != nullptr && mod_invstd != nullptr && gamma_cs >= d->Cout &&
                    gamma_cs % 4 == 0,
                CSG_E_BADSHAPE, "csg_wino4_conv_part: the modulation needs gamma, mean, invstd");
    CSG_REQUIRE(((uintptr_t)mod_x % 16) == 0 && ((uintptr_t)mod_gamma % 16) == 0 && ((uintptr_t)mod_mean % 16) == 0 &&
                    ((uintptr_t)mod_invstd % 16) == 0,
                CSG_E_UNSUPPORTED, "csg_wino4_conv_part: pointers must be 16-byte aligned");
    p.mod = 1; p.g_cs = (int)gamma_cs; p.mod_slope = mod_slope; p.mod_mean = mod_mean; p.mod_invstd = mod_invstd;
  }
  CSG_REQUIRE(((uintptr_t)x % 16) == 0 && ((uintptr_t)packed % 16) == 0 && ((uintptr_t)y % 16) == 0 &&
                  (bias == nullptr || ((uintptr_t)bias % 16) == 0),
              CSG_E_UNSUPPORTED, "csg_wino4_conv_part: pointers must be 16-byte aligned");
  return w4_launch<4>(p, shm, K_WINO4_CONV, 2.0 * p.B * p.H * p.W * 9.0 * p.Cin * p.Cout, x, packed, bias, mod_x, mod_gamma, y,
                      nullptr, y, (hipStream_t)stream, "csg_wino4_conv_part");
}

static int w4_spade_plan(const csg_wino_desc* d, Wino4Params& p, size_t& shm, const char* who) {
  CSG_REQUIRE(d != nullptr && d->Cout % 32 == 0, CSG_E_UNSUPPORTED, "%s: C must be a multiple of 32", who);
  int rc = w4_plan(d, 4, 1, p, shm, who);
  if (rc) return rc;
  const int tiles = d->Cout / 32;
  p.NT32 = 2 * tiles;
  p.nblocks = tiles;
  p.gb_off = tiles;
  p.mod = 2;
  const int64_t items = (int64_t)p.B * p.tby * p.tbx * p.nblocks;
  CSG_REQUIRE(items < (1ll << 31) && w4_persistent_blocks(p, items) > 0, CSG_E_UNSUPPORTED,
              "%s: the launch does not qualify for the persistent form (%ld items, %d stages)", who, (long)items, p.nstage);
  return CSG_OK;
}

int32_t csg_wino4_conv_spade_supported(const csg_wino_desc* d) {
  if (!csg_wino4_supported(d)) return 0;
  Wino4Params p;
  size_t shm = 0;
  const int rc = w4_spade_plan(d, p, shm, "csg_wino4_conv_spade_supported");
  return rc == CSG_OK ? 1 : 0;
}

int csg_wino4_conv_spade(const csg_wino_desc* d, const float* x, const float* packed, const float* bias, const float* mod_x,
                         float* gamma_out, int64_t gamma_cs, const float* mod_mean, const float* mod_invstd, float mod_slope,
                         float* y, void* stream) {
  Wino4Params p;
  size_t shm = 0;
  int rc = w4_spade_plan(d, p, shm, "csg_wino4_conv_spade");
  if (rc) return rc;
  CSG_REQUIRE(d->act == CSG_ACT_NONE, CSG_E_UNSUPPORTED, "csg_wino4_conv_spade: no activation (the modulation has its own)");
  CSG_REQUIRE(bias != nullptr && mod_x != nullptr && mod_mean != nullptr && mod_invstd != nullptr,
              CSG_E_BADSHAPE, "csg_wino4_conv_spade: needs the 2C biases, x, mean, invstd");
  CSG_REQUIRE(gamma_out == nullptr || (gamma_cs >= d->Cout && gamma_cs % 4 == 0 && ((uintptr_t)gamma_out % 16) == 0),
              CSG_E_BADSHAPE, "csg_wino4_conv_spade: bad gamma buffer");
  const int tiles = d->Cout / 32;
  CSG_REQUIRE((int64_t)36 * 2 * tiles * p.Q8 * 1024 < CSG_MAX_RECORDS, CSG_E_UNSUPPORTED,
              "csg_wino4_conv_spade: packed weights too large for 32-bit byte offsets");
  CSG_REQUIRE(((uintptr_t)x % 16) == 0 && ((uintptr_t)packed % 16) == 0 && ((uintptr_t)y % 16) == 0 && ((uintptr_t)bias % 16) == 0 &&
                  ((uintptr_t)mod_x % 16) == 0 && ((uintptr_t)mod_mean % 16) == 0 && ((uintptr_t)mod_invstd % 16) == 0,
              CSG_E_UNSUPPORTED, "csg_wino4_conv_spade: pointers must be 16-byte aligned");
  p.g_cs = (int)gamma_cs; p.mod_slope = mod_slope; p.mod_mean = mod_mean; p.mod_invstd = mod_invstd;
  return w4_launch<4>(p, shm, K_WINO4_CONV, 2.0 * p.B * p.H * p.W * 9.0 * p.Cin * 2.0 * p.Cout, x, packed, bias, mod_x, gamma_out,
                      y, nullptr, y, (hipStream_t)stream, "csg_wino4_conv_spade");
}

}
```

canonicalsg2im_amd/ops.py:

```python
import collections
import ctypes
import os

import torch
import torch.distributed as dist
import torch.nn.functional as F
from torch.optim.optimizer import register_optimizer_step_post_hook as _register_optimizer_step_post_hook

from . import _lib
from . import dist as csg_dist
from ._lib import ACT_LEAKY, ACT_NONE, ACT_TANH, ConvDesc, FewDesc, GemmDesc, HingeItem, WinoDesc, WinoPackItem, check, lib, ptr, stream

__all__ = [
    "nhwc", "empty_nhwc", "conv2d", "linear", "norm_act", "upsample2x", "nearest_resize", "avgpool3s2", "embed", "real_object_mask",
    "norm_act_pair", "graph_csr", "gather_concat", "segment_avg", "layout_pyramid", "layout_paint", "disc_input", "crop_objects", "maxpool2", "avgpool2", "l1_mean",
    "invalidate_weight_caches", "pack_conv_weight", "wino_pack", "prepack_weights", "wino_eligible", "wino_variant", "plan_conv", "spectral_weight", "spectral_weights", "ACT_NONE", "ACT_LEAKY", "ACT_TANH",
]


def nhwc(t):
    if t.permute(0, 2, 3, 1).is_contiguous():
        return t
    return t.permute(0, 2, 3, 1).contiguous().permute(0, 3, 1, 2)

# ... 907 lines not shown
        if ctx.needs_input_grad[0]:
            if not use_batch_stats:
                dsums.zero_()
            elif multi:
                csg_dist.all_reduce_stats(_drop_clamped_invstd_term(dsums, invstd, eps, C))
            dx = torch.empty_like(x)
            check(lib.csg_norm_apply_bwd_dx(ptr(dy), ptr(x), ptr(mean), ptr(invstd), ptr(gb), slope, ptr(dsums), count,
                                            G, P, C, ptr(dx), None, None, 1.0, ptr(dgb), None, 2 * C, stream()), "norm_bwd_dx")
        return dx, dgb, None, None, None, None, None, None, None, None


class _NormActPair(torch.autograd.Function):

    @staticmethod
    def forward(ctx, x, gb0, gb1, rm0, rv0, rm1, rv1, slope0, slope1, eps, momentum, sync):
        x = nhwc(_f32(x))
        B, C, H, W = x.shape
        P = B * H * W
        dev = x.device
        world = _sync_world() if sync else 1
        multi = _multi(world, sync)
        count = float(P * world)
        mean = torch.empty(C, device=dev, dtype=torch.float32)
        invstd = torch.empty(C, device=dev, dtype=torch.float32)
        nch = _chunks(P, 1)
        part = torch.empty(nch * 2 * C, device=dev, dtype=torch.float64)
        if not multi:
            check(lib.csg_norm_stats_finalize(ptr(x), 1, P, C, ptr(part), nch, count, eps, ptr(mean), ptr(invstd), ptr(rm0),
                                              ptr(rv0 if rm0 is not None else None), ptr(rm1),
                                              ptr(rv1 if rm1 is not None else None), momentum, stream()), "norm_stats_finalize")
        else:
            sums = torch.empty(2 * C, device=dev, dtype=torch.float64)
            check(lib.csg_norm_stats(ptr(x), 1, P, C, ptr(sums), ptr(part), nch, stream()), "norm_stats")
            csg_dist.all_reduce_stats(sums)
            for rm, rv in ((rm0, rv0), (rm1, rv1)):
                check(lib.csg_norm_finalize(ptr(sums), 1, C, count, eps, 1, ptr(mean), ptr(invstd), ptr(rm),
                                            ptr(rv if rm is not None else None), momentum, stream()), "norm_finalize")
        gb0, gb1 = nhwc(gb0), nhwc(gb1)
        y0, y1 = torch.empty_like(x), torch.empty_like(x)
        check(lib.csg_norm_apply_fwd(ptr(x), ptr(mean), ptr(invstd), ptr(gb0), slope0, 1, P, C, ptr(y0), ptr(gb1), slope1,
                                     ptr(y1), stream()), "norm_apply_fwd")
        ctx.save_for_backward(x, gb0, gb1, mean, invstd)
        ctx.cfg = (P, C, slope0, slope1, multi, count, eps)
        return y0, y1

    @staticmethod
    def backward(ctx, dy0, dy1):
        x, gb0, gb1, mean, invstd = ctx.saved_tensors
        P, C, slope0, slope1, multi, count, eps = ctx.cfg
        dy0, dy1 = nhwc(dy0), nhwc(dy1)
        dev = x.device
        nch = _chunks(P, 1)
        part = torch.empty(nch * 2 * C, device=dev, dtype=torch.float64)
        dsums = torch.empty(2, 2 * C, device=dev, dtype=torch.float64)
        dgb0, dgb1 = torch.empty_like(gb0), torch.empty_like(gb1)
        check(lib.csg_norm_apply_bwd_reduce(ptr(dy0), ptr(x), ptr(mean), ptr(invstd), ptr(gb0), None, slope0, 1, P, C, ptr(dgb0),
                                            ptr(dsums[0]), ptr(part), nch, 2 * C, stream()), "norm_bwd_reduce")
        check(lib.csg_norm_apply_bwd_reduce(ptr(dy1), ptr(x), ptr(mean), ptr(invstd), ptr(gb1), None, slope1, 1, P, C, ptr(dgb1),
                                            ptr(dsums[1]), ptr(part), nch, 2 * C, stream()), "norm_bwd_reduce")
        dx = None
        if ctx.needs_input_grad[0]:
            both = dsums[0] + dsums[1]
            if multi:
                csg_dist.all_reduce_stats(_drop_clamped_invstd_term(both, invstd, eps, C))
            dx = torch.empty_like(x)
            check(lib.csg_norm_apply_bwd_dx(ptr(dy0), ptr(x), ptr(mean), ptr(invstd), ptr(gb0), slope0, ptr(both), count,
                                            1, P, C, ptr(dx), ptr(dy1), ptr(gb1), slope1, ptr(dgb0), ptr(dgb1), 2 * C, stream()),
                  "norm_bwd_dx")
        return dx, dgb0, dgb1, None, None, None, None, None, None, None, None, None


SPADE_FUSED = os.environ.get("CSG_SPADE_FUSED", "1") != "0"
SPADE_JOINED = os.environ.get("CSG_SPADE_JOINED", "1") != "0"


def spade_fused_eligible(x, nhidden, C, ks, training):
    if not (SPADE_FUSED and WINO_ENABLED and training and ks == 3 and x.dim() == 4 and C % 32 == 0):
        return False
    B, _, H, W = x.shape
    return lib.csg_wino4_supported(_wino_desc(B, H, W, nhidden, C)) == 1


SPADE_JOINT = os.environ.get("CSG_SPADE_JOINT", "1") != "0"


class _SpadeFused(torch.autograd.Function):

    NARG = 7

    @staticmethod
    def forward(ctx, x, eps, momentum, sync, *mods):
        K = len(mods) // _SpadeFused.NARG
        x = nhwc(_f32(x))
        B, C, H, W = x.shape
        if C % 32 != 0:
            raise RuntimeError("spade_fused: C = %d must be a multiple of 32 (the modulation rides on 32-channel tiles)" % C)
        for k in range(K):
            actv, w = mods[k * 7], mods[k * 7 + 1]
            if actv.dim() != 4 or tuple(w.shape) != (2 * C, actv.shape[1], 3, 3) or tuple(actv.shape) != (B, actv.shape[1], H, W):
                raise RuntimeError("spade_fused: weight %s / actv %s do not fit x %s" % (tuple(w.shape), tuple(actv.shape),
                                                                                         tuple(x.shape)))
        P = B * H * W
        dev = x.device
        world = _sync_world() if sync else 1
        multi = _multi(world, sync)
        count = float(P * world)
        mean = torch.empty(C, device=dev, dtype=torch.float32)
        invstd = torch.empty(C, device=dev, dtype=torch.float32)
        nch = _chunks(P, 1)
        part = torch.empty(nch * 2 * C, device=dev, dtype=torch.float64)
        pending = sums = None
        if not multi:
            r0, r1 = (mods[3], mods[4]), ((mods[10], mods[11]) if K == 2 else (None, None))
            check(lib.csg_norm_stats_finalize(ptr(x), 1, P, C, ptr(part), nch, count, eps, ptr(mean), ptr(invstd), ptr(r0[0]),
                                              ptr(r0[1] if r0[0] is not None else None), ptr(r1[0]),
                                              ptr(r1[1] if r1[0] is not None else None), momentum, stream()),
                  "norm_stats_finalize")
        else:
            sums = torch.empty(2 * C, device=dev, dtype=torch.float64)
            check(lib.csg_norm_stats(ptr(x), 1, P, C, ptr(sums), ptr(part), nch, stream()), "norm_stats")
            pending = csg_dist.all_reduce_stats_async(sums)
        outs, groups, launches, plans, pres = [None] * K, [None] * K, [], [], []
        joint = SPADE_JOINT and not multi and C % 32 == 0
        for k in range(K):
            actv, w, b, rm, rv, slope, in_slope = mods[k * 7:(k + 1) * 7]
            actv = nhwc(_f32(actv))
            nh = actv.shape[1]
            up = wino_pack(w, False, None, 4)
            plans.append(plan_conv(B, H, W, nh, 2 * C, 3, 3, 1, 1, has_bias=True,
                                   in_act=(ACT_LEAKY, in_slope) if in_slope is not None else None,
                                   need=ctx.needs_input_grad[4 + 7 * k:7 + 7 * k]))
            pres.append(_take_dx_operand(plans[k], w))
            bd = b.detach().contiguous()
            gbuf = empty_nhwc(B, C, H, W, dev)
            d = _wino_desc(B, H, W, nh, C)
            d.y_cs = C
            if joint and lib.csg_wino4_conv_spade_supported(d):
                y = torch.empty_like(x)
                _wino4_audit("spade_joint", B * H * W, nh + 3 * C, up)
                check(lib.csg_wino4_conv_spade(d, ptr(actv), ptr(up), ptr(bd), ptr(x), ptr(gbuf), C, ptr(mean), ptr(invstd),
                                               slope, ptr(y), stream()), "wino4_conv_spade")
                outs[k], groups[k] = y, [actv, w, gbuf, y]
                continue
            _wino4_audit("spade_gamma", B * H * W, nh + C, up)
            _wino4_audit("spade_beta", B * H * W, nh + 3 * C, up)
            check(lib.csg_wino4_conv_part(d, ptr(actv), ptr(up), 0, 2 * C // 32, ptr(bd), None, None, 0, None, None, 1.0,
                                          ptr(gbuf), stream()), "wino4_conv_part(gamma)")
            launches.append((k, actv, w, up, bd, gbuf, nh, slope))
        if pending is not None:
            pending.wait()
        for k in range(K if multi else 0):
            rm, rv = mods[k * 7 + 3], mods[k * 7 + 4]
            check(lib.csg_norm_finalize(ptr(sums), 1, C, count, eps, 1, ptr(mean), ptr(invstd), ptr(rm),
                                        ptr(rv if rm is not None else None), momentum, stream()), "norm_finalize")
        for (k, actv, w, up, bd, gbuf, nh, slope) in launches:
            y = torch.empty_like(x)
            d = _wino_desc(B, H, W, nh, C)
            d.y_cs = C
            check(lib.csg_wino4_conv_part(d, ptr(actv), ptr(up), C // 32, 2 * C // 32, ptr(bd[C:]), ptr(x), ptr(gbuf), C,
                                          ptr(mean), ptr(invstd), slope, ptr(y), stream()), "wino4_conv_part(beta)")
            outs[k], groups[k] = y, [actv, w, gbuf, y]
        ctx.save_for_backward(x, mean, invstd, *[t for g in groups for t in g])
        ctx.cfg = (K, P, C, B, H, W, multi, count, eps, tuple(mods[k * 7 + 5] for k in range(K)))
        ctx.plans, ctx.ut_pres = plans, pres
        return tuple(outs)

    @staticmethod
    def backward(ctx, *dys):
        K, P, C, B, H, W, multi, count, eps, slopes = ctx.cfg
        sv = ctx.saved_tensors
        x, mean, invstd = sv[0], sv[1], sv[2]
        dev = x.device
        nch = _chunks(P, 1)
        part = torch.empty(nch * 2 * C, device=dev, dtype=torch.float64)
        dsums = torch.empty(K, 2 * C, device=dev, dtype=torch.float64)
        dys = [nhwc(dy) for dy in dys]
        dgbs = []
        for k in range(K):
            actv, w, gbuf, y = sv[3 + 4 * k:7 + 4 * k]
            dgb = empty_nhwc(B, 2 * C, H, W, dev)
            check(lib.csg_norm_apply_bwd_reduce(ptr(dys[k]), ptr(x), ptr(mean), ptr(invstd), ptr(gbuf), ptr(y), slopes[k], 1, P,
                                                C, ptr(dgb), ptr(dsums[k]), ptr(part), nch, C, stream()), "norm_bwd_reduce")
            dgbs.append(dgb)
        dx, both, pending = None, None, None
        if ctx.needs_input_grad[0]:
            both = dsums[0] + dsums[1] if K == 2 else dsums[0]
            pending = csg_dist.all_reduce_stats_async(_drop_clamped_invstd_term(both, invstd, eps, C)) if multi else None
        grads = [None, None, None, None]
        for k in range(K):
            actv, w, gbuf, y = sv[3 + 4 * k:7 + 4 * k]
            need = ctx.needs_input_grad[4 + 7 * k:7 + 7 * k]
            grads += list(_conv_bwd(ctx.plans[k], dgbs[k], actv, w, None, need, None, ctx.ut_pres[k])) + [None] * 4
        if ctx.needs_input_grad[0]:
            if pending is not None:
                pending.wait()
            dx = torch.empty_like(x)
            two = K == 2
            check(lib.csg_norm_apply_bwd_dx(ptr(dys[0]), ptr(x), ptr(mean), ptr(invstd), ptr(sv[5]), slopes[0], ptr(both), count,
                                            1, P, C, ptr(dx), ptr(dys[1]) if two else None, ptr(sv[9]) if two else None,
                                            slopes[1] if two else 1.0, ptr(dgbs[0]), ptr(dgbs[1]) if two else None, C, stream()),
                  "norm_bwd_dx")
            grads[0] = dx
        return tuple(grads)


class _SpadeJoined(torch.autograd.Function):

    @staticmethod
    def forward(ctx, x, actv, w, b, running_mean, running_var, pad, slope, in_slope, eps, momentum, sync):
        x = nhwc(_f32(x))
        B, C, H, W = x.shape
        P = B * H * W
        dev = x.device
        world = _sync_world() if sync else 1
        multi = _multi(world, sync)
        count = float(P * world)
        mean = torch.empty(C, device=dev, dtype=torch.float32)
        invstd = torch.empty(C, device=dev, dtype=torch.float32)
        nch = _chunks(P, 1)
        part = torch.empty(nch * 2 * C, device=dev, dtype=torch.float64)
        pending = sums = None
        if not multi:
            check(lib.csg_norm_stats_finalize(ptr(x), 1, P, C, ptr(part), nch, count, eps, ptr(mean), ptr(invstd),
                                              ptr(running_mean), ptr(running_var if running_mean is not None else None), None,
                                              None, momentum, stream()), "norm_stats_finalize")
        else:
            sums = torch.empty(2 * C, device=dev, dtype=torch.float64)
            check(lib.csg_norm_stats(ptr(x), 1, P, C, ptr(sums), ptr(part), nch, stream()), "norm_stats")
            pending = csg_dist.all_reduce_stats_async(sums)
        actv = nhwc(_f32(actv))
        ctx.plan = plan_conv(B, H, W, actv.shape[1], w.shape[0], w.shape[2], w.shape[3], 1, int(pad), has_bias=b is not None,
                             in_act=(ACT_LEAKY, float(in_slope)) if in_slope is not None else None, need=(True, True, True))
        gb, ctx.ut_pre = _conv_fwd(ctx.plan, actv, w, b, None, None)
        if pending is not None:
            pending.wait()
        if multi:
            check(lib.csg_norm_finalize(ptr(sums), 1, C, count, eps, 1, ptr(mean), ptr(invstd),
                                        ptr(running_mean), ptr(running_var if running_mean is not None else None), momentum,
                                        stream()), "norm_finalize")
        y = torch.empty_like(x)
        check(lib.csg_norm_apply_fwd(ptr(x), ptr(mean), ptr(invstd), ptr(gb), slope, 1, P, C, ptr(y), None, 1.0, None, stream()),
              "norm_apply_fwd")
        ctx.save_for_backward(x, gb, mean, invstd, actv, w)
        ctx.cfg = (P, C, slope, multi, count, eps)
        return y

    @staticmethod
    def backward(ctx, dy):
        x, gb, mean, invstd, cx, cw = ctx.saved_tensors
        P, C, slope, multi, count, eps = ctx.cfg
        dy = nhwc(dy)
        dev = x.device
        nch = _chunks(P, 1)
        part = torch.empty(nch * 2 * C, device=dev, dtype=torch.float64)
        dsums = torch.empty(2 * C, device=dev, dtype=torch.float64)
        dgb = torch.empty_like(gb)
        check(lib.csg_norm_apply_bwd_reduce(ptr(dy), ptr(x), ptr(mean), ptr(invstd), ptr(gb), None, slope, 1, P, C, ptr(dgb),
                                            ptr(dsums), ptr(part), nch, 2 * C, stream()), "norm_bwd_reduce")
        pending = (csg_dist.all_reduce_stats_async(_drop_clamped_invstd_term(dsums, invstd, eps, C))
                   if (multi and ctx.needs_input_grad[0]) else None)
        r = _conv_bwd(ctx.plan, dgb, cx, cw, None, ctx.needs_input_grad[1:4], None, ctx.ut_pre)
        dx = None
        if ctx.needs_input_grad[0]:
            if pending is not None:
                pending.wait()
            dx = torch.empty_like(x)
            check(lib.csg_norm_apply_bwd_dx(ptr(dy), ptr(x), ptr(mean), ptr(invstd), ptr(gb), slope, ptr(dsums), count,
                                            1, P, C, ptr(dx), None, None, 1.0, ptr(dgb), None, 2 * C, stream()), "norm_bwd_dx")
        return dx, r[0], r[1], r[2], None, None, None, None, None, None, None, None


def spade_joined(x, actv, w, b, running_mean, running_var, pad, slope, in_slope, eps=1e-5, momentum=0.1, sync=True):
    return _SpadeJoined.apply(x, actv, w, b, running_mean, running_var, int(pad), float(slope),
                              None if in_slope is None else float(in_slope), float(eps), float(momentum), bool(sync))


def spade_fused(x, mods, eps=1e-5, momentum=0.1, sync=True):
    flat = []
    for (actv, w, b, rm, rv, slope, in_slope) in mods:
        flat += [actv, w, b, rm, rv, float(slope), None if in_slope is None else float(in_slope)]
    return list(_SpadeFused.apply(x, float(eps), float(momentum), bool(sync), *flat))


def norm_act_pair(x, gb0, gb1, rm0, rv0, rm1, rv1, slope0, slope1, eps=1e-5, momentum=0.1, sync=True):
    return _NormActPair.apply(x, gb0, gb1, rm0, rv0, rm1, rv1, float(slope0), float(slope1), float(eps), float(momentum),
                              bool(sync))


def norm_act(x, gb=None, running_mean=None, running_var=None, instance=False, training=True, slope=1.0, eps=1e-5,
             momentum=0.1, sync=True):
    return _NormAct.apply(x, gb, running_mean, running_var, bool(instance), bool(training), float(slope), float(eps),
                          float(momentum), bool(sync))


class _Upsample2x(torch.autograd.Function):
    @staticmethod
    def forward(ctx, x):
        x = nhwc(_f32(x))
        B, C, H, W = x.shape
        y = empty_nhwc(B, C, 2 * H, 2 * W, x.device)
        check(lib.csg_upsample2x_fwd(ptr(x), B, H, W, C, ptr(y), stream()), "upsample2x_fwd")
        ctx.shape = (B, C, H, W)
        return y

    @staticmethod
    def backward(ctx, dy):
        B, C, H, W = ctx.shape
        dy = nhwc(dy)
        dx = empty_nhwc(B, C, H, W, dy.device)
        check(lib.csg_upsample2x_bwd(ptr(dy), B, H, W, C, ptr(dx), stream()), "upsample2x_bwd")
        return dx


def upsample2x(x):
    return _Upsample2x.apply(x)


class _NearestResize(torch.autograd.Function):

    @staticmethod
    def forward(ctx, x, OH, OW):
        x = nhwc(_f32(x))
        B, C, IH, IW = x.shape
        if C % 4:
            raise RuntimeError("nearest_resize: the channel count must be a multiple of 4")
        y = empty_nhwc(B, C, OH, OW, x.device)
        check(lib.csg_nearest_resize_fwd(ptr(x), B, IH, IW, C, OH, OW, ptr(y), stream()), "nearest_resize_fwd")
        ctx.shape = (B, C, IH, IW, OH, OW)
        return y

    @staticmethod
    def backward(ctx, dy):
        B, C, IH, IW, OH, OW = ctx.shape
        dy = nhwc(dy)
        dx = empty_nhwc(B, C, IH, IW, dy.device)
        check(lib.csg_nearest_resize_bwd(ptr(dy), B, IH, IW, C, OH, OW, ptr(dx), stream()), "nearest_resize_bwd")
        return dx, None, None


def nearest_resize(x, size):
    return _NearestResize.apply(x, int(size[0]), int(size[1]))


class _AvgPool3s2(torch.autograd.Function):
    @staticmethod
    def forward(ctx, x):
        x = nhwc(_f32(x))
        B, C, H, W = x.shape
        y = empty_nhwc(B, C, (H - 1) // 2 + 1, (W - 1) // 2 + 1, x.device)
        check(lib.csg_avgpool3s2_fwd(ptr(x), B, H, W, C, ptr(y), stream()), "avgpool_fwd")
        ctx.shape = (B, C, H, W)
        return y

    @staticmethod
    def backward(ctx, dy):
        B, C, H, W = ctx.shape
        dy = nhwc(dy)
        dx = empty_nhwc(B, C, H, W, dy.device)
        check(lib.csg_avgpool3s2_bwd(ptr(dy), B, H, W, C, ptr(dx), stream()), "avgpool_bwd")
        return dx


def avgpool3s2(x):
    return _AvgPool3s2.apply(x)
# ... 471 lines not shown
```

canonicalsg2im_amd/spade/models/networks/architecture.py:

```python
import torch
import torch.nn as nn

from .... import ops
from ....spectral_norm import spectral_norm
from ....sg2im.layers import Conv2d
from .normalization import SPADE, spade_pair


class SPADEResnetBlock(nn.Module):
    def __init__(self, fin, fout, opt):
        super().__init__()
        self.learned_shortcut = (fin != fout)
        fmiddle = min(fin, fout)
        self.conv_0 = Conv2d(fin, fmiddle, kernel_size=3, padding=1)
        self.conv_1 = Conv2d(fmiddle, fout, kernel_size=3, padding=1)
        if self.learned_shortcut:
            self.conv_s = Conv2d(fin, fout, kernel_size=1, bias=False)
        if 'spectral' in opt.norm_G:
            self.conv_0 = spectral_norm(self.conv_0)
            self.conv_1 = spectral_norm(self.conv_1)
            if self.learned_shortcut:
                self.conv_s = spectral_norm(self.conv_s)
        cfg = opt.norm_G.replace('spectral', '')
        self.norm_0 = SPADE(cfg, fin, opt.semantic_nc)
        self.norm_1 = SPADE(cfg, fmiddle, opt.semantic_nc)
        if self.learned_shortcut:
            self.norm_s = SPADE(cfg, fin, opt.semantic_nc)

    def forward(self, x, seg):
        if self.learned_shortcut:
            xs, h = spade_pair(self.norm_s, self.norm_0, x, seg, 1.0, 0.2)
            x_s = self.conv_s(xs)
        else:
            x_s, h = x, self.norm_0(x, seg, fused_slope=0.2)
        dx = self.conv_0(h)
        return self.conv_1(self.norm_1(dx, seg, fused_slope=0.2), residual=x_s)

    def shortcut(self, x, seg):
        return self.conv_s(self.norm_s(x, seg)) if self.learned_shortcut else x


_VGG19_CFG = (64, 64, 'M', 128, 128, 'M', 256, 256, 256, 256, 'M', 512, 512, 512, 512, 'M', 512)
_VGG19_SLICES = ((0, 2), (2, 7), (7, 12), (12, 21), (21, 30))


class _VGGConv(nn.Module):

    def __init__(self, cin, cout):
        super().__init__()
        self.weight = nn.Parameter(torch.empty(cout, cin, 3, 3))
        self.bias = nn.Parameter(torch.empty(cout))
        nn.init.kaiming_normal_(self.weight, mode='fan_out', nonlinearity='relu')
        nn.init.zeros_(self.bias)
        self._packs = None

    def forward(self, x):
        if self.weight.requires_grad:
            return ops.conv2d(x, self.weight, self.bias, 1, 1, act=ops.ACT_LEAKY, slope=0.0)
        if self._packs is None or self._packs[1] != self.weight._version or self._packs[0].fwd.device != x.device:
            self._packs = (ops.pack_conv_weight(self.weight), self.weight._version)
        return ops.conv2d(x, self.weight, self.bias, 1, 1, act=ops.ACT_LEAKY, slope=0.0, packs=self._packs[0])


class _VGGPool(nn.Module):
    def forward(self, x):
        return ops.maxpool2(x)


class _Slice(nn.Module):

    def forward(self, x):
        for m in self.children():
            x = m(x)
        return x


def _find_vgg19_weights():
    import os
    path = os.environ.get("CSG_VGG19_WEIGHTS")
    if path:
        sd = torch.load(path, map_location="cpu")
        return sd.get("state_dict", sd)
    try:
        import torchvision
        return torchvision.models.vgg19(pretrained=True).state_dict()
    except Exception:
        return None


class VGG19(nn.Module):

    def __init__(self, requires_grad=False, weights=None):
        super().__init__()
        import os
        idx, cin, layers = 0, 3, {}
        for v in _VGG19_CFG:
            if v == 'M':
                layers[idx] = _VGGPool()
                idx += 1
            else:
                layers[idx] = _VGGConv(cin, v)
                cin = v
                idx += 2
        for k, (lo, hi) in enumerate(_VGG19_SLICES):
            sl = _Slice()
            for i in range(lo, hi):
                if i in layers:
                    sl.add_module(str(i), layers[i])
            setattr(self, "slice%d" % (k + 1), sl)
        if weights is None and os.environ.get("CSG_VGG19_RANDOM") == "1":
            weights = "random"
        if weights != "random":
            sd = weights if isinstance(weights, dict) else _find_vgg19_weights()
            if sd is None:
                raise RuntimeError(
                    "VGG19: no pretrained weights. Point CSG_VGG19_WEIGHTS at torchvision's vgg19 state dict "
# ... 23 lines not shown
```

canonicalsg2im_amd/spade/models/networks/generator.py:

```python
import torch.nn as nn

from .... import ops
from .... import spectral_norm as csg_spectral_norm
from ....sg2im.attribute_embed import AttributeEmbeddings
from ....sg2im.layers import Conv2d, GlobalAvgPool, build_cnn, build_mlp
from ....sg2im.utils import real_object_mask
from .architecture import SPADEResnetBlock
from .base_network import BaseNetwork
from .normalization import SegPyramid


class AppearanceEncoder(nn.Module):

    def __init__(self, vocab, arch, normalization='none', activation='relu', padding='same', vecs_size=1024,
                 pooling='avg'):
        super().__init__()
        self.vocab = vocab
        cnn, channels = build_cnn(arch=arch, normalization=normalization, activation=activation, pooling=pooling,
                                  padding=padding)
        self.cnn = nn.Sequential(cnn, GlobalAvgPool(), nn.Linear(channels, vecs_size))

    def forward(self, crops):
        return self.cnn(crops)


_BLOCKS = (("head_0", 16, 16), ("G_middle_0", 16, 16), ("G_middle_1", 16, 16),
           ("up_0", 16, 8), ("up_1", 8, 4), ("up_2", 4, 2), ("up_3", 2, 1))
_LATENT_HALVINGS = {'normal': 5, 'more': 6, 'most': 7}


class SPADEGenerator(BaseNetwork):

    def __init__(self, opt):
        super().__init__()
        if opt.use_vae:
            raise NotImplementedError("--use_vae is never wired in the reference trainer (SURVEY.md §2 row 22)")
        self.attribute_embedding = AttributeEmbeddings(opt.vocab['attributes'], opt.embedding_dim)
        self.opt = opt
        nf = opt.ngf
        self.sw, self.sh = self.compute_latent_vector_size(opt)
        self.fc = Conv2d(opt.semantic_nc, 16 * nf, 3, padding=1)
        blocks = list(_BLOCKS)
        if opt.num_upsampling_layers == 'most':
            blocks.append(("up_4", 1, 0.5))
        for name, win, wout in blocks:
            setattr(self, name, SPADEResnetBlock(int(win * nf), int(wout * nf), opt))
        self._block_names = [b[0] for b in blocks]
        self.conv_img = Conv2d(int(blocks[-1][2] * nf), 3, 3, padding=1, act=ops.ACT_TANH)
        self.up = nn.Upsample(scale_factor=2)
        self.repr_input = opt.g_mask_dim
        self.repr_net = build_mlp([self.repr_input, 64, opt.rep_size], batch_norm=opt.mlp_normalization)
        self.image_encoder = AppearanceEncoder(vocab=opt.vocab, arch='C4-64-2,C4-128-2,C4-256-2', padding='valid',
                                               normalization=opt.appearance_normalization,
                                               activation=opt.a_activation, vecs_size=opt.g_mask_dim)

    def compute_latent_vector_size(self, opt):
        if opt.num_upsampling_layers not in _LATENT_HALVINGS:
            raise ValueError('opt.num_upsampling_layers [%s] not recognized' % opt.num_upsampling_layers)
        sw = opt.image_size[0] >> _LATENT_HALVINGS[opt.num_upsampling_layers]
        return sw, round(sw / opt.aspect_ratio)

    def forward(self, objs, layout_boxes, layout_masks, test_mode=False):
        if self.sw != self.sh:
            raise NotImplementedError("aspect_ratio != 1 is not on the hot path")
        csg_spectral_norm.prepare(self)
        ops.prepack_weights(self)
        H = self.opt.image_size[0]
        levels = [self.sw << k for k in range(H.bit_length()) if (self.sw << k) <= H]
        valid = real_object_mask(objs, self.opt.vocab)
        if layout_masks is not None and test_mode:
            maps = ops.layout_paint(self.attribute_embedding(objs), layout_boxes, valid, layout_masks, H, levels)
        else:
            maps = ops.layout_pyramid(self.attribute_embedding(objs), layout_boxes, valid, H, levels, masks=layout_masks)
        seg = SegPyramid(zip(levels, maps))
        x = self.fc(seg.at(self.sw))
        no_upsample = {"head_0"} | (set() if self.opt.num_upsampling_layers in ('more', 'most') else {"G_middle_1"})
        for name in self._block_names:
            if name not in no_upsample:
                x = ops.upsample2x(x)
            x = getattr(self, name)(x, seg)
        return self.conv_img(x, pre_slope=2e-1)
```

canonicalsg2im_amd/spade/models/networks/normalization.py:

```python
import re

import torch
import torch.nn as nn

from .... import ops
from ....spectral_norm import spectral_norm
from ....sg2im.layers import Conv2d, _FusedActivation
from .sync_batchnorm import LocalBatchNorm2d, SynchronizedBatchNorm2d


class SegPyramid:

    def __init__(self, levels):
        self.levels = dict(levels)

    def at(self, h):
        return self.levels[int(h)]


class InstanceNormAct(nn.InstanceNorm2d):

    def __init__(self, num_features, fused_slope=1.0):
        super().__init__(num_features, affine=False)
        self.fused_slope = fused_slope
# ... 42 lines not shown

    @staticmethod
    def forward(ctx, a, b, joined):
        ctx.n = a.shape[0]
        return joined.view_as(joined)

    @staticmethod
    def backward(ctx, g):
        return g[:ctx.n], g[ctx.n:], None


def _join_storage(pa, pb):
    cl = pa.dim() == 4
    joined = torch.empty((2 * pa.shape[0],) + tuple(pa.shape[1:]), device=pa.device, dtype=pa.dtype)
    if cl:
        joined = joined.contiguous(memory_format=torch.channels_last)
    n = pa.shape[0]
    with torch.no_grad():
        joined[:n].copy_(pa)
        joined[n:].copy_(pb)
    pa.data = joined[:n]
    pb.data = joined[n:]
    return joined


def _joined(mod, name, pa, pb):
    j = getattr(mod, name, None)
    n = pa.shape[0]
    if (j is None or j.device != pa.device or pa.data_ptr() != j.data_ptr() or
            pb.data_ptr() != j.data_ptr() + n * j.stride(0) * j.element_size() or pa.stride() != j.stride()
            or pb.stride() != j.stride()):
        j = _join_storage(pa, pb)
        object.__setattr__(mod, name, j)
    return _JoinedPair.apply(pa, pb, j)


class SPADE(nn.Module):
    def __init__(self, config_text, norm_nc, label_nc):
        super().__init__()
        assert config_text.startswith('spade')
        parsed = re.search(r'spade(\D+)(\d)x\d', config_text)
        kind, ks = str(parsed.group(1)), int(parsed.group(2))
        if kind == 'instance':
            self.param_free_norm = InstanceNormAct(norm_nc)
        elif kind == 'syncbatch':
            self.param_free_norm = SynchronizedBatchNorm2d(norm_nc, affine=False)
        elif kind == 'batch':
            self.param_free_norm = LocalBatchNorm2d(norm_nc, affine=False)
        else:
            raise ValueError('%s is not a recognized param-free norm type in SPADE' % kind)
        nhidden = 128
        self.pw = ks // 2
        self.mlp_shared = nn.Sequential(Conv2d(label_nc, nhidden, kernel_size=ks, padding=self.pw,
                                               act=ops.ACT_LEAKY, slope=0.0), _FusedActivation())
        self.mlp_gamma = Conv2d(nhidden, norm_nc, kernel_size=ks, padding=self.pw)
        self.mlp_beta = Conv2d(nhidden, norm_nc, kernel_size=ks, padding=self.pw)

    def forward(self, x, segmap, fused_slope=1.0):
        if self.fusable(x):
            return ops.spade_fused(x, [self.fused_operands(x, segmap, fused_slope)], self.param_free_norm.eps,
                                   self.param_free_norm.momentum, getattr(self.param_free_norm, "sync", True))[0]
        pn = self.param_free_norm
        if self.joinable(x):
            actv, w, b, rm, rv, slope, in_slope = self.fused_operands(x, segmap, fused_slope)
            return ops.spade_joined(x, actv, w, b, rm, rv, self.pw, slope, in_slope, pn.eps, pn.momentum,
                                    getattr(pn, "sync", True))
        return pn(x, gb=self.modulation(x, segmap), fused_slope=fused_slope)

    def joinable(self, x):
        pn = self.param_free_norm
        return (ops.SPADE_JOINED and isinstance(pn, (SynchronizedBatchNorm2d, LocalBatchNorm2d)) and not pn.affine
                and pn.training and x.dim() == 4 and x.is_cuda and self.mlp_gamma.weight.shape[0] % 4 == 0)

    def fusable(self, x):
        pn = self.param_free_norm
        return (isinstance(pn, (SynchronizedBatchNorm2d, LocalBatchNorm2d)) and not pn.affine and pn.training
                and ops.spade_fused_eligible(x, self.mlp_gamma.weight.shape[1], self.mlp_gamma.weight.shape[0],
                                             self.mlp_gamma.weight.shape[2], pn.training))

    def joined_weight(self):
        _joined(self, "_joined_w", self.mlp_gamma.weight, self.mlp_beta.weight)
        return self.__dict__.get("_joined_w")

    def fused_operands(self, x, segmap, slope):
        if isinstance(segmap, SegPyramid):
            seg = segmap.at(x.size(2))
        else:
            seg = segmap if segmap.shape[2:] == x.shape[2:] else ops.nearest_resize(segmap, x.shape[2:])
        sh = self.mlp_shared[0]
        actv = ops.conv2d(seg, sh.weight, sh.bias, 1, sh.padding[0], sh.act, sh.slope, grad_is_pre=True)
        w = _joined(self, "_joined_w", self.mlp_gamma.weight, self.mlp_beta.weight)
        b = _joined(self, "_joined_b", self.mlp_gamma.bias, self.mlp_beta.bias)
        pn = self.param_free_norm
        return (actv, w, b, pn.running_mean, pn.running_var, slope, sh.slope)

    def modulation(self, x, segmap):
        if isinstance(segmap, SegPyramid):
            seg = segmap.at(x.size(2))
        else:
            seg = segmap if segmap.shape[2:] == x.shape[2:] else ops.nearest_resize(segmap, x.shape[2:])
        sh = self.mlp_shared[0]
        actv = ops.conv2d(seg, sh.weight, sh.bias, 1, sh.padding[0], sh.act, sh.slope, grad_is_pre=True)
        w = _joined(self, "_joined_w", self.mlp_gamma.weight, self.mlp_beta.weight)
        b = _joined(self, "_joined_b", self.mlp_gamma.bias, self.mlp_beta.bias)
        return ops.conv2d(actv, w, b, 1, self.pw, in_act=(sh.act, sh.slope))


def spade_pair(norm_a, norm_b, x, segmap, slope_a, slope_b):
    pa, pb = norm_a.param_free_norm, norm_b.param_free_norm
    same = (type(pa) is type(pb) and isinstance(pa, (SynchronizedBatchNorm2d, LocalBatchNorm2d)) and not pa.affine
            and not pb.affine and pa.training and pb.training and pa.eps == pb.eps and pa.momentum == pb.momentum
            and getattr(pa, "sync", True) == getattr(pb, "sync", True) and x.dim() == 4)
    if not same:
        return norm_a(x, segmap, fused_slope=slope_a), norm_b(x, segmap, fused_slope=slope_b)
    if norm_a.fusable(x) and norm_b.fusable(x):
        ya, yb = ops.spade_fused(x, [norm_a.fused_operands(x, segmap, slope_a), norm_b.fused_operands(x, segmap, slope_b)],
                                 pa.eps, pa.momentum, getattr(pa, "sync", True))
        return ya, yb
    return ops.norm_act_pair(x, norm_a.modulation(x, segmap), norm_b.modulation(x, segmap), pa.running_mean, pa.running_var,
                             pb.running_mean, pb.running_var, slope_a, slope_b, pa.eps, pa.momentum,
                             getattr(pa, "sync", True))
```

include/csg_hip.h:

```cpp
#ifndef CSG_HIP_H
#define CSG_HIP_H

#include <stdint.h>

#ifdef __cplusplus
extern "C" {
#endif

#define CSG_OK 0
#define CSG_E_BADSHAPE (-1)
#define CSG_E_UNSUPPORTED (-2)
#define CSG_E_LAUNCH (-3)
#define CSG_E_WORKSPACE (-4)

#define CSG_ACT_NONE 0
#define CSG_ACT_LEAKY 1
#define CSG_ACT_TANH 2

#define CSG_MAX_TAPS 16

int csg_version(void);
const char* csg_last_error(void);

int csg_prof_enable(int mode);
// ... 44 lines not shown
                   int64_t OW, float* dvecs, int accumulate, const float* vecs, float* dboxes, void* workspace,
                   int64_t workspace_bytes, void* stream);
int csg_layout_bwd_masks(const float* dout, int64_t out_cs, int64_t out_off, const float* boxes, const uint8_t* valid,
                         int64_t M, int64_t B, int64_t O, int64_t S, int64_t H, int64_t W, int64_t OH, int64_t OW,
                         const float* vecs, float* dmasks, int accumulate, void* stream);
int csg_layout_mass(const float* vecs, const float* boxes, const uint8_t* valid, const float* masks, int64_t M,
                    int64_t B, int64_t O, int64_t S, int64_t H, int64_t W, float* mass, void* stream);
int csg_layout_paint(const float* vecs, const float* boxes, const float* masks, int64_t M, const int32_t* order,
                     int64_t B, int64_t O, int64_t S, int64_t H, int64_t W, int64_t OH, int64_t OW, float* out,
                     int64_t out_cs, int64_t out_off, void* stream);

typedef struct csg_conv_desc {
  int32_t B, IHp, IWp, Cin, x_cs;
  int32_t IHv, IWv, in_up;
  int32_t OHg, OWg, OHf, OWf, os, ooy, oox;
  int32_t Cout, y_cs;
  int32_t istride, ntaps, wtaps;
  int32_t tap_dy[CSG_MAX_TAPS], tap_dx[CSG_MAX_TAPS], tap_w[CSG_MAX_TAPS];
  int32_t act;
  float slope;
  int32_t accumulate;
  int32_t res_gate;
} csg_conv_desc;

int64_t csg_conv_fwd_workspace(const csg_conv_desc* d);
int csg_conv_fwd(const csg_conv_desc* d, const float* x, const float* w, const float* bias, const float* residual,
                 float* y, float* workspace, int64_t workspace_bytes, void* stream);
int64_t csg_conv_fwd_multi_workspace(const csg_conv_desc* descs, int32_t n);
int csg_conv_fwd_multi(const csg_conv_desc* descs, int32_t n, const float* x, const float* w, const float* bias,
                       const float* residual, float* y, float* workspace, int64_t workspace_bytes, void* stream);
int64_t csg_conv_bwd_weight_workspace(const csg_conv_desc* d);
int csg_conv_bwd_weight(const csg_conv_desc* d, const float* x, const float* dy, float* dw, float* db,
                        float* workspace, int64_t workspace_bytes, void* stream);

typedef struct csg_wino_desc {
  int32_t B, H, W;
  int32_t Cin, x_cs;
  int32_t Cout, y_cs;
  int32_t act;
  float slope;
} csg_wino_desc;
int64_t csg_wino_pack_bytes(int64_t N, int64_t K);
int csg_wino_pack_weights(const float* w, int64_t s_o, int64_t s_i, int64_t s_h, int64_t s_w, int64_t Cout, int64_t Cin,
                          int32_t backward_data, const float* sigma, float* packed, void* stream);
int64_t csg_wino_conv_workspace(const csg_wino_desc* d);
int csg_wino_conv(const csg_wino_desc* d, const float* x, const float* packed, const float* bias,
                  const float* residual, const float* gate, float gate_slope, float* y, float* workspace,
                  int64_t workspace_bytes, void* stream);
int64_t csg_wino_bwd_weight_workspace(const csg_wino_desc* d);
int csg_wino_bwd_weight(const csg_wino_desc* d, const float* x, const float* dy, float* dw, float* db, float* workspace,
                        int64_t workspace_bytes, void* stream);

int64_t csg_wino4_bwd_weight_workspace(const csg_wino_desc* d);
int csg_wino4_bwd_weight(const csg_wino_desc* d, const float* x, const float* dy, float* dw, float* db, float* workspace,
                         int64_t workspace_bytes, void* stream);

int32_t csg_wino4_supported(const csg_wino_desc* d);
typedef struct csg_wino_pack_item {
  const float* w;
  int64_t s_o, s_i, s_h, s_w;
  int64_t Cout, Cin;
  int32_t backward_data;
  int32_t variant;
  float* packed;
} csg_wino_pack_item;
int csg_wino_pack_weights_multi(const csg_wino_pack_item* items, int32_t n, void* stream);
int32_t csg_wino4_persistent(int32_t on);
int64_t csg_wino4_pack_bytes(int64_t N, int64_t K);
int csg_wino4_pack_weights(const float* w, int64_t s_o, int64_t s_i, int64_t s_h, int64_t s_w, int64_t Cout, int64_t Cin,
                           int32_t backward_data, const float* sigma, float* packed, void* stream);
int64_t csg_wino4_conv_workspace(const csg_wino_desc* d);
int csg_wino4_conv(const csg_wino_desc* d, const float* x, const float* packed, const float* bias,
                   const float* residual, const float* gate, float gate_slope, float* y, float* workspace,
                   int64_t workspace_bytes, void* stream);

int csg_wino4_conv_part(const csg_wino_desc* d, const float* x, const float* packed, int64_t tile_off, int64_t tiles_total,
                        const float* bias, const float* mod_x, const float* mod_gamma, int64_t gamma_cs,
                        const float* mod_mean, const float* mod_invstd, float mod_slope, float* y, void* stream);

int32_t csg_wino4_conv_spade_supported(const csg_wino_desc* d);
int csg_wino4_conv_spade(const csg_wino_desc* d, const float* x, const float* packed, const float* bias, const float* mod_x,
                         float* gamma_out, int64_t gamma_cs, const float* mod_mean, const float* mod_invstd, float mod_slope,
                         float* y, void* stream);

int32_t csg_wino34_supported(const csg_wino_desc* d, int32_t pad);
int csg_wino34_pack_weights(const float* w, int64_t s_o, int64_t s_i, int64_t s_h, int64_t s_w, int64_t Cout, int64_t Cin,
                            int32_t backward_data, const float* sigma, float* packed, void* stream);
int64_t csg_wino34_conv_workspace(const csg_wino_desc* d, int32_t pad);
int csg_wino34_conv(const csg_wino_desc* d, int32_t pad, const float* x, const float* packed, const float* bias,
                    const float* residual, const float* gate, float gate_slope, float* y, float* workspace,
                    int64_t workspace_bytes, void* stream);

typedef struct csg_few_desc {
  int32_t B, IH, IW;
  int32_t Cin, x_cs;
  int32_t KH, KW, pad;
  int32_t cout_real;
  int32_t act;
  float slope;
  int32_t in_act;
  float in_slope;
} csg_few_desc;
int csg_conv_few_supported(const csg_few_desc* d);
int64_t csg_conv_few_fwd_workspace(const csg_few_desc* d);
int csg_conv_few_fwd(const csg_few_desc* d, const float* x, const float* w, const float* bias, float* y, float* workspace,
                     int64_t workspace_bytes, void* stream);
int csg_conv_few_bwd_data(const csg_few_desc* d, const float* dy, const float* w, float* dx, void* stream);
int64_t csg_conv_few_bwd_weight_workspace(const csg_few_desc* d);
int csg_conv_few_bwd_weight(const csg_few_desc* d, const float* x, const float* dy, float* dw, float* db,
                            float* workspace, int64_t workspace_bytes, void* stream);

typedef struct csg_gemm_desc {
  int64_t M, N, K;
  int64_t lda, ldb, ldy, ldg;
  int32_t act;
  float slope;
  float gate_slope;
} csg_gemm_desc;
int csg_gemm_supported(const csg_gemm_desc* d);
int csg_gemm_nt(const csg_gemm_desc* d, const float* a, const float* bw, const float* bias, const float* gate, float* y,
                void* stream);
int64_t csg_gemm_tn_workspace(int64_t M, int64_t N, int64_t K);
int csg_gemm_tn(int64_t M, int64_t N, int64_t K, const float* dy, int64_t ldy, const float* x, int64_t ldx, float* dw,
                float* db, float* workspace, int64_t workspace_bytes, void* stream);

int csg_act_bwd(const float* dy, const float* y, int64_t n, int32_t act, float slope, float* dpre, void* stream);
int csg_colsum(const float* x, int64_t rows, int64_t C, int64_t x_cs, float* out, double* partial, int64_t nchunk,
               void* stream);

int csg_norm_stats(const float* x, int64_t G, int64_t P, int64_t C, double* sums, double* partial, int64_t nchunk,
                   void* stream);
int csg_norm_finalize(const double* sums, int64_t G, int64_t C, double count, float eps, int32_t mode, float* mean,
                      float* invstd, float* running_mean, float* running_var, float momentum, void* stream);
int csg_norm_stats_finalize(const float* x, int64_t G, int64_t P, int64_t C, double* partial, int64_t nchunk, double count,
                            float eps, float* mean, float* invstd, float* running_mean, float* running_var,
                            float* running_mean2, float* running_var2, float momentum, void* stream);
int csg_norm_apply_fwd(const float* x, const float* mean, const float* invstd, const float* gb, float slope,
                       int64_t G, int64_t P, int64_t C, float* y, const float* gb2, float slope2, float* y2,
                       void* stream);
int csg_norm_apply_bwd_reduce(const float* dy, const float* x, const float* mean, const float* invstd,
                              const float* gb, const float* yact, float slope, int64_t G, int64_t P, int64_t C, float* dgb,
                              double* dsums, double* partial, int64_t nchunk, int64_t gb_cs, void* stream);
int csg_norm_apply_bwd_dx(const float* dy, const float* x, const float* mean, const float* invstd, const float* gb,
                          float slope, const double* dsums, double count, int64_t G, int64_t P, int64_t C, float* dx,
                          const float* dy2, const float* gb2, float slope2, const float* dgb, const float* dgb2,
                          int64_t gb_cs, void* stream);

int csg_nearest_resize_fwd(const float* x, int64_t B, int64_t IH, int64_t IW, int64_t C, int64_t OH, int64_t OW, float* y,
                           void* stream);
int csg_nearest_resize_bwd(const float* dy, int64_t B, int64_t IH, int64_t IW, int64_t C, int64_t OH, int64_t OW, float* dx,
                           void* stream);
int csg_upsample2x_fwd(const float* x, int64_t B, int64_t H, int64_t W, int64_t C, float* y, void* stream);
int csg_upsample2x_bwd(const float* dy, int64_t B, int64_t H, int64_t W, int64_t C, float* dx, void* stream);
int csg_avgpool3s2_fwd(const float* x, int64_t B, int64_t H, int64_t W, int64_t C, float* y, void* stream);
int csg_avgpool3s2_bwd(const float* dy, int64_t B, int64_t H, int64_t W, int64_t C, float* dx, void* stream);
int csg_avgpool3s2_bwd_add(const float* dy, int64_t B, int64_t H, int64_t W, int64_t C, const float* add, float* dx,
                           void* stream);

int csg_crop_fwd(const float* img, int64_t B, int64_t H, int64_t W, int64_t img_cs, int64_t C, const float* boxes,
                 const int64_t* img_idx, int64_t N, int64_t HH, int64_t WW, float* out, int64_t out_cs, void* stream);
int csg_crop_bwd(const float* dout, int64_t B, int64_t H, int64_t W, int64_t img_cs, int64_t C, const float* boxes,
                 const int64_t* img_idx, int64_t N, int64_t HH, int64_t WW, int64_t out_cs, float* dimg, void* stream);
int csg_crop_bwd_boxes(const float* dout, const float* img, int64_t B, int64_t H, int64_t W, int64_t img_cs, int64_t C,
                       const float* boxes, const int64_t* img_idx, int64_t N, int64_t HH, int64_t WW, int64_t out_cs,
                       float* dboxes, void* stream);

int csg_maxpool2_fwd(const float* x, int64_t B, int64_t H, int64_t W, int64_t C, float* y, void* stream);
int csg_maxpool2_bwd(const float* dy, const float* x, int64_t B, int64_t H, int64_t W, int64_t C, float* dx,
                     void* stream);
int csg_avgpool2_fwd(const float* x, int64_t B, int64_t H, int64_t W, int64_t C, float* y, void* stream);
int csg_avgpool2_bwd(const float* dy, int64_t B, int64_t H, int64_t W, int64_t C, float* dx, void* stream);
int64_t csg_l1_mean_workspace(int64_t n);
int csg_l1_mean_fwd(const float* a, const float* b, int64_t n, float* out, void* workspace, int64_t workspace_bytes,
                    void* stream);
int csg_l1_mean_bwd(const float* a, const float* b, const float* gout, int64_t n, float* da, void* stream);

typedef struct csg_hinge_item {
  const float* x;
  float* dx;
  int64_t sb, sh, sw;
  int64_t B, H, W;
} csg_hinge_item;
int csg_hinge_mean_fwd(const csg_hinge_item* items, int32_t n, int32_t kind, float* out, void* stream);
int csg_hinge_mean_bwd(const csg_hinge_item* items, int32_t n, int32_t kind, const float* gout, void* stream);

int64_t csg_canon_workspace(int64_t B);
int csg_canon_build(const int64_t* objs0, const float* boxes, const float* centers, const int64_t* n_objs,
                    int64_t B, int64_t O, const int32_t* pred_ids, int64_t image_id, int include_dummies,
                    int learned_transitivity, void* workspace, int64_t workspace_bytes, int64_t* counts,
                    void* stream);
int csg_canon_emit(const int64_t* objs0, const int64_t* n_objs, int64_t B, int64_t O, const int32_t* pred_ids,
                   int64_t image_id, int include_dummies, int learned_transitivity, const void* workspace,
                   const int64_t* counts, int64_t T, int64_t* triplets, int64_t* triplet_type, void* stream);
int csg_canon_converse(const int64_t* objs0, const int64_t* n_objs, int64_t B, int64_t O, const int32_t* pred_ids,
                       int64_t image_id, int include_dummies, int learned_transitivity, void* workspace,
                       const double* cdf, const double* uniforms, const int64_t* u_off, int64_t num_preds,
                       float* conv_counts, int64_t* counts, void* stream);

#define CSG_CANON_ROLE_OTHER (-1)
#define CSG_CANON_ROLE_PADDING (-2)
#define CSG_CANON_ROLE_IN_IMAGE (-3)
int64_t csg_canon_general_workspace(int64_t B, int64_t P, int64_t R);
int csg_canon_general_build(const int64_t* objs0, const float* boxes, const float* centers, const int64_t* n_objs,
                            int64_t B, int64_t O, const int64_t* rel, const int64_t* rel_counts, int64_t R,
                            const int32_t* roles, int64_t P, int64_t image_id, int include_dummies, void* workspace,
                            int64_t workspace_bytes, int64_t* counts, void* stream);
int csg_canon_general_converse(int64_t B, const int32_t* roles, int64_t P, void* workspace, int64_t workspace_bytes,
                               const double* cdf, const double* uniforms, const int64_t* u_off, float* conv_counts,
                               void* stream);
int csg_canon_general_close(int64_t B, const int32_t* roles, int64_t P, int learned_transitivity, void* workspace,
                            int64_t workspace_bytes, int64_t* counts, void* stream);
int csg_canon_general_emit(int64_t B, const int32_t* roles, int64_t P, const void* workspace, int64_t workspace_bytes,
                           const int64_t* counts, int64_t T, int64_t* triplets, int64_t* triplet_type, void* stream);

int64_t csg_spectral_norm_workspace(int64_t Cout, int64_t K);
int csg_spectral_norm_fwd(const float* w, float* u, float* v, int64_t Cout, int64_t K, int iterate, float eps,
                          float* w_eff, int64_t cl_Cin, float* sigma, float* u_used, float* v_used, void* workspace,
                          int64_t workspace_bytes, void* stream);
int csg_spectral_norm_bwd(const float* dweff, int64_t Cout, int64_t Cin, int64_t KH, int64_t KW, int64_t s0,
                          int64_t s1, int64_t s2, int64_t s3, const float* w, const float* u_used,
                          const float* v_used, const float* sigma, float* dw, void* workspace,
                          int64_t workspace_bytes, void* stream);

typedef struct csg_sn_fwd_item {
  const float* w;
  float* u;
  float* v;
  int64_t Cout, K;
  float* w_eff;
// ... 26 lines not shown
```

Measured before the change: 216.4 img/s.

## Fuse nearest 2x upsample into SPADE norm stats, modulation conv, and backward

Learned-shortcut SPADE residual blocks no longer materialize the 2x upsampled activation. Instead, norm statistics are computed on the low-resolution source with sums scaled by 4. The Winograd conv epilogue reads the modulated input through upsampled indexing, and the backward reduce and dx kernels read the source and sum the four child-pixel gradients. The goal is to cut HBM traffic and kernel launches for the upsample forward and backward at the largest generator resolutions. In exchange it adds index arithmetic and extra kernel variants, and the gradient summation order may differ slightly from the old path.

```diff
diff --git a/canonicalsg2im_amd/_lib.py b/canonicalsg2im_amd/_lib.py
--- a/canonicalsg2im_amd/_lib.py
+++ b/canonicalsg2im_amd/_lib.py
@@ -128,6 +128,14 @@
                                     c_p, c_p]),
     "csg_wino4_conv_spade_supported": (c_i32, [ctypes.POINTER(WinoDesc)]),
     "csg_wino4_conv_spade": (c_i32, [ctypes.POINTER(WinoDesc), c_p, c_p, c_p, c_p, c_p, c_i64, c_p, c_p, c_f32, c_p, c_p]),
+    "csg_wino4_conv_part_up2": (c_i32, [ctypes.POINTER(WinoDesc), c_p, c_p, c_i64, c_i64, c_p, c_p, c_p, c_i64, c_p, c_p, c_f32,
+                                        c_p, c_p]),
+    "csg_wino4_conv_spade_up2": (c_i32, [ctypes.POINTER(WinoDesc), c_p, c_p, c_p, c_p, c_p, c_i64, c_p, c_p, c_f32, c_p, c_p]),
+    "csg_norm_stats_finalize_up2": (c_i32, [c_p, c_i64, c_i64, c_p, c_i64, c_f64, c_f32, c_p, c_p, c_p, c_p, c_p, c_p, c_f32,
+                                            c_p]),
+    "csg_norm_apply_bwd_reduce_up2": (c_i32, [c_p, c_p, c_p, c_p, c_p, c_p, c_f32, c_i64, c_i64, c_i64, c_i64, c_p, c_p, c_p,
+                                              c_i64, c_p]),
+    "csg_norm_apply_bwd_dx_up2": (c_i32, [c_p, c_p, c_p, c_p, c_p, c_f64, c_i64, c_i64, c_i64, c_i64, c_p, c_p, c_p, c_p, c_p]),
     "csg_wino34_supported": (c_i32, [ctypes.POINTER(WinoDesc), c_i32]),
     "csg_wino34_pack_weights": (c_i32, [c_p, c_i64, c_i64, c_i64, c_i64, c_i64, c_i64, c_i32, c_p, c_p, c_p]),
     "csg_wino34_conv_workspace": (c_i64, [ctypes.POINTER(WinoDesc), c_i32]),
diff --git a/canonicalsg2im_amd/csrc/csg_api.hip b/canonicalsg2im_amd/csrc/csg_api.hip
--- a/canonicalsg2im_amd/csrc/csg_api.hip
+++ b/canonicalsg2im_amd/csrc/csg_api.hip
@@ -128,7 +128,7 @@
 
 extern "C" {
 
-int csg_version(void) { return 109; }
+int csg_version(void) { return 110; }
 const char* csg_last_error(void) { return csg::g_err; }
 
 int csg_prof_enable(int on) {
diff --git a/canonicalsg2im_amd/csrc/norm.hip b/canonicalsg2im_amd/csrc/norm.hip
--- a/canonicalsg2im_amd/csrc/norm.hip
+++ b/canonicalsg2im_amd/csrc/norm.hip
@@ -101,7 +101,8 @@
                                                                   double count, float eps, float* __restrict__ mean,
                                                                   float* __restrict__ invstd, float* __restrict__ rmean,
                                                                   float* __restrict__ rvar, float* __restrict__ rmean2,
-                                                                  float* __restrict__ rvar2, float momentum) {
+                                                                  float* __restrict__ rvar2, float momentum,
+                                                                  double rep) {
   __shared__ double sm[8][32];
   __shared__ double tot[32];
   const int cl = threadIdx.x & 31, rl = threadIdx.x >> 5;
@@ -132,7 +133,7 @@
   }
   __syncthreads();
   if (threadIdx.x < 16 && c < C) {
-    const double S = tot[threadIdx.x], SS = tot[threadIdx.x + 16];
+    const double S = tot[threadIdx.x] * rep, SS = tot[threadIdx.x + 16] * rep;
     const double m = S / count;
     double var = (SS - S * m) / count;
     if (var < 0.0) var = 0.0;
@@ -206,13 +207,14 @@
   }
 }
 
+template <bool UP>
 __global__ __launch_bounds__(256) void k_norm_bwd_reduce(const float* __restrict__ dy, const float* __restrict__ x,
                                                           const float* __restrict__ mean,
                                                           const float* __restrict__ invstd,
                                                           const float* __restrict__ gb,
                                                           const float* __restrict__ yact, float slope, int64_t P, int C,
                                                           int nchunk, float* __restrict__ dgb,
-                                                          double* __restrict__ partial, int gcs) {
+                                                          double* __restrict__ partial, int gcs, int H2, int W2) {
   extern __shared__ __attribute__((aligned(16))) double smd[];
   const int tid = threadIdx.x;
   const int chunk = blockIdx.x, g = blockIdx.y;
@@ -231,7 +233,13 @@
 #pragma unroll 2
       for (int64_t p = p0 + rr; p < p1; p += R) {
         const int64_t pix = (int64_t)g * P + p;
-        const float4 xv = ld4(x + pix * C + co);
+        int64_t xpix = pix;
+        if (UP) {
+          const unsigned t = (unsigned)p / (unsigned)W2, X = (unsigned)p - t * (unsigned)W2;
+          const unsigned b = t / (unsigned)H2, Y = t - b * (unsigned)H2;
+          xpix = ((int64_t)b * (H2 >> 1) + (Y >> 1)) * (W2 >> 1) + (X >> 1);
+        }
+        const float4 xv = ld4(x + xpix * C + co);
         float4 d = ld4(dy + pix * C + co);
         float4 xh = make_float4((xv.x - m.x) * r.x, (xv.y - m.y) * r.y, (xv.z - m.z) * r.z, (xv.w - m.w) * r.w);
         float4 dn = d;
@@ -333,6 +341,53 @@
   }
 }
 
+__device__ __forceinline__ float4 sum4_in_order(float4 a, float4 c, float4 d, float4 f) {
+#pragma clang fp contract(off)
+  return make_float4(a.x + c.x + d.x + f.x, a.y + c.y + d.y + f.y, a.z + c.z + d.z + f.z, a.w + c.w + d.w + f.w);
+}
+
+__global__ __launch_bounds__(256) void k_norm_bwd_dx_up2(const float* __restrict__ x, const float* __restrict__ mean,
+                                                          const float* __restrict__ invstd, const float* __restrict__ gb,
+                                                          const double* __restrict__ dsums, double inv_count, int H, int W,
+                                                          int C, int64_t n4, float* __restrict__ dx,
+                                                          const float* __restrict__ gb2, const float* __restrict__ dgb,
+                                                          const float* __restrict__ dgb2) {
+  const int Q = C >> 2;
+  for (int64_t e = (int64_t)blockIdx.x * blockDim.x + threadIdx.x; e < n4; e += (int64_t)gridDim.x * blockDim.x) {
+    const int64_t pix = e / Q;
+    const int q = (int)(e - pix * Q);
+    const int xw = (int)(pix % W);
+    const int64_t t = pix / W;
+    const int yh = (int)(t % H);
+    const int64_t bi = t / H;
+    const int co = q * 4;
+    const float4 xv = ld4(x + e * 4);
+    const float4 m = ld4(mean + co), r = ld4(invstd + co);
+    const float4 xh = make_float4((xv.x - m.x) * r.x, (xv.y - m.y) * r.y, (xv.z - m.z) * r.z, (xv.w - m.w) * r.w);
+    const float4 a = make_float4((float)(dsums[co] * inv_count), (float)(dsums[co + 1] * inv_count),
+                                 (float)(dsums[co + 2] * inv_count), (float)(dsums[co + 3] * inv_count));
+    const float4 b = make_float4((float)(dsums[C + co] * inv_count), (float)(dsums[C + co + 1] * inv_count),
+                                 (float)(dsums[C + co + 2] * inv_count), (float)(dsums[C + co + 3] * inv_count));
+    const int64_t op0 = (bi * 2 * H + 2 * yh) * 2 * W + 2 * xw;
+    float4 o[4];
+#pragma unroll
+    for (int j = 0; j < 4; ++j) {
+      const int64_t op = op0 + (j >> 1) * 2 * W + (j & 1);
+      const float4 ga = ld4(gb + op * C + co);
+      const float4 d = ld4(dgb + op * 2 * C + C + co);
+      float4 dn = make_float4(d.x * (1.f + ga.x), d.y * (1.f + ga.y), d.z * (1.f + ga.z), d.w * (1.f + ga.w));
+      if (gb2 != nullptr) {
+        const float4 ga2 = ld4(gb2 + op * C + co);
+        const float4 d2 = ld4(dgb2 + op * 2 * C + C + co);
+        dn.x += d2.x * (1.f + ga2.x); dn.y += d2.y * (1.f + ga2.y); dn.z += d2.z * (1.f + ga2.z); dn.w += d2.w * (1.f + ga2.w);
+      }
+      o[j].x = r.x * (dn.x - a.x - xh.x * b.x); o[j].y = r.y * (dn.y - a.y - xh.y * b.y);
+      o[j].z = r.z * (dn.z - a.z - xh.z * b.z); o[j].w = r.w * (dn.w - a.w - xh.w * b.w);
+    }
+    st4(dx + e * 4, sum4_in_order(o[0], o[1], o[2], o[3]));
+  }
+}
+
 __global__ void k_act_bwd(const float* __restrict__ dy, const float* __restrict__ y, int64_t n, int act, float slope,
                           float* __restrict__ dpre) {
   for (int64_t i = (int64_t)blockIdx.x * blockDim.x + threadIdx.x; i < n; i += (int64_t)gridDim.x * blockDim.x) {
@@ -515,8 +570,28 @@
   }
   ProfScope p(K_NORM_FINALIZE, (double)G * C * 24, s);
   CSG_LAUNCH(k_partial_reduce_finalize, dim3((unsigned)cdiv(C, 16), (unsigned)G), dim3(256), 0, s, partial, (int)C, (int)nchunk,
-             count, eps, mean, invstd, running_mean, running_var, running_mean2, running_var2, momentum);
+             count, eps, mean, invstd, running_mean, running_var, running_mean2, running_var2, momentum, 1.0);
   return check_launch("csg_norm_stats_finalize");
+}
+
+int csg_norm_stats_finalize_up2(const float* x, int64_t P, int64_t C, double* partial, int64_t nchunk, double count, float eps,
+                                float* mean, float* invstd, float* running_mean, float* running_var, float* running_mean2,
+                                float* running_var2, float momentum, void* stream) {
+  CSG_REQUIRE(P > 0 && C > 0 && C % 4 == 0 && count > 0, CSG_E_BADSHAPE, "csg_norm_stats_finalize_up2: bad shape P=%ld C=%ld",
+              (long)P, (long)C);
+  CSG_REQUIRE(nchunk >= 1 && nchunk <= 65535, CSG_E_BADSHAPE, "csg_norm_stats_finalize_up2: bad nchunk");
+  CSG_REQUIRE((running_mean == nullptr) == (running_var == nullptr) && (running_mean2 == nullptr) == (running_var2 == nullptr),
+              CSG_E_BADSHAPE, "csg_norm_stats_finalize_up2: running mean and variance come together");
+  hipStream_t s = (hipStream_t)stream;
+  {
+    ProfScope p(K_NORM_STATS, (double)P * C * 4, s);
+    CSG_LAUNCH(k_norm_stats_partial, dim3((unsigned)nchunk, 1), dim3(256), 256 * 8 * 8, s, x, P, (int)C, C, (int)nchunk,
+               partial);
+  }
+  ProfScope p(K_NORM_FINALIZE, (double)C * 24, s);
+  CSG_LAUNCH(k_partial_reduce_finalize, dim3((unsigned)cdiv(C, 16), 1), dim3(256), 0, s, partial, (int)C, (int)nchunk, count,
+             eps, mean, invstd, running_mean, running_var, running_mean2, running_var2, momentum, 4.0);
+  return check_launch("csg_norm_stats_finalize_up2");
 }
 
 int csg_norm_finalize(const double* sums, int64_t G, int64_t C, double count, float eps, int32_t mode, float* mean,
@@ -555,12 +630,32 @@
   hipStream_t s = (hipStream_t)stream;
   {
     ProfScope p(K_NORM_BWD_REDUCE, (double)G * P * C * 4 * (gb ? 6 : 2), s);
-    CSG_LAUNCH(k_norm_bwd_reduce, dim3((unsigned)nchunk, (unsigned)G), dim3(256), 256 * 8 * 8, s, dy, x, mean,
-                       invstd, gb, yact, slope, P, (int)C, (int)nchunk, dgb, partial, (int)gb_cs);
+    CSG_LAUNCH(k_norm_bwd_reduce<false>, dim3((unsigned)nchunk, (unsigned)G), dim3(256), 256 * 8 * 8, s, dy, x, mean,
+                       invstd, gb, yact, slope, P, (int)C, (int)nchunk, dgb, partial, (int)gb_cs, 0, 0);
   }
   CSG_LAUNCH(k_partial_reduce<double>, dim3((unsigned)cdiv(2 * C, 32), (unsigned)G), dim3(256), 0, s, partial,
                      (int)(2 * C), (int)nchunk, (int)(2 * C), dsums);
   return check_launch("csg_norm_apply_bwd_reduce");
+}
+
+int csg_norm_apply_bwd_reduce_up2(const float* dy, const float* x, const float* mean, const float* invstd, const float* gamma,
+                                  const float* yact, float slope, int64_t B, int64_t H, int64_t W, int64_t C, float* dgb,
+                                  double* dsums, double* partial, int64_t nchunk, void* stream) {
+  CSG_REQUIRE(B > 0 && H > 0 && W > 0 && C > 0 && C % 4 == 0 && B * 4 * H * W < (1ll << 31), CSG_E_BADSHAPE,
+              "csg_norm_apply_bwd_reduce_up2: bad shape");
+  CSG_REQUIRE(dy != nullptr && x != nullptr && gamma != nullptr && yact != nullptr && dgb != nullptr, CSG_E_BADSHAPE,
+              "csg_norm_apply_bwd_reduce_up2: needs dy, the source x, gamma, y and d(gamma || beta)");
+  CSG_REQUIRE(nchunk >= 1 && nchunk <= 65535, CSG_E_BADSHAPE, "csg_norm_apply_bwd_reduce_up2: bad nchunk");
+  hipStream_t s = (hipStream_t)stream;
+  const int64_t P = B * 4 * H * W;
+  {
+    ProfScope p(K_NORM_BWD_REDUCE, (double)P * C * 4 * 5.25, s);
+    CSG_LAUNCH(k_norm_bwd_reduce<true>, dim3((unsigned)nchunk, 1), dim3(256), 256 * 8 * 8, s, dy, x, mean, invstd, gamma, yact,
+               slope, P, (int)C, (int)nchunk, dgb, partial, (int)C, (int)(2 * H), (int)(2 * W));
+  }
+  CSG_LAUNCH(k_partial_reduce<double>, dim3((unsigned)cdiv(2 * C, 32), 1), dim3(256), 0, s, partial, (int)(2 * C),
+             (int)nchunk, (int)(2 * C), dsums);
+  return check_launch("csg_norm_apply_bwd_reduce_up2");
 }
 
 int csg_norm_apply_bwd_dx(const float* dy, const float* x, const float* mean, const float* invstd, const float* gb,
@@ -579,6 +674,21 @@
   return check_launch("csg_norm_apply_bwd_dx");
 }
 
+int csg_norm_apply_bwd_dx_up2(const float* x, const float* mean, const float* invstd, const float* gamma, const double* dsums,
+                              double count, int64_t B, int64_t H, int64_t W, int64_t C, float* dx, const float* gamma2,
+                              const float* dgb, const float* dgb2, void* stream) {
+  CSG_REQUIRE(B > 0 && H > 0 && W > 0 && C > 0 && C % 4 == 0 && count > 0, CSG_E_BADSHAPE,
+              "csg_norm_apply_bwd_dx_up2: bad shape");
+  CSG_REQUIRE(x != nullptr && gamma != nullptr && dgb != nullptr && dx != nullptr && (gamma2 == nullptr) == (dgb2 == nullptr),
+              CSG_E_BADSHAPE, "csg_norm_apply_bwd_dx_up2: needs the source x, gamma, d(gamma || beta); gamma2 and dgb2 come together");
+  hipStream_t s = (hipStream_t)stream;
+  const int64_t n4 = B * H * W * C / 4;
+  ProfScope p(K_NORM_BWD_DX, (double)n4 * 16 * (2 + 8 + (gamma2 ? 8 : 0)), s);
+  CSG_LAUNCH(k_norm_bwd_dx_up2, dim3(ew_grid(n4)), dim3(256), 0, s, x, mean, invstd, gamma, dsums, 1.0 / count, (int)H, (int)W,
+             (int)C, n4, dx, gamma2, dgb, dgb2);
+  return check_launch("csg_norm_apply_bwd_dx_up2");
+}
+
 int csg_act_bwd(const float* dy, const float* y, int64_t n, int32_t act, float slope, float* dpre, void* stream) {
   CSG_REQUIRE(n >= 0, CSG_E_BADSHAPE, "csg_act_bwd: bad n");
   if (n == 0) return CSG_OK;
diff --git a/canonicalsg2im_amd/csrc/wino4.hip b/canonicalsg2im_amd/csrc/wino4.hip
--- a/canonicalsg2im_amd/csrc/wino4.hip
+++ b/canonicalsg2im_amd/csrc/wino4.hip
@@ -35,6 +35,7 @@
   int mod, g_cs;
   int gb_off;
   float mod_slope;
+  int mod_up;
   const float* mod_mean;
   const float* mod_invstd;
   int nstage;
@@ -177,9 +178,12 @@
       if (MODE == 2) {
         mm = *(const float4*)(p.mod_mean + n);
         mr = *(const float4*)(p.mod_invstd + n);
+        const int64_t xrs = p.mod_up ? (int64_t)(p.Wo >> 1) * p.y_cs : rowstride;
+        const int64_t xoff =
+            p.mod_up ? (((int64_t)img * (p.Ho >> 1) + (oy >> 1)) * (p.Wo >> 1) + (ox >> 1)) * p.y_cs + n : off;
 #pragma unroll
         for (int a = 0; a < 4; ++a) {
-          mx[a] = *(const float4*)(res + off + a * rowstride);
+          mx[a] = *(const float4*)(res + xoff + (p.mod_up ? a >> 1 : a) * xrs);
           mg[a] = *(const float4*)(gate + (pix0 + (int64_t)a * p.Wo) * p.g_cs + n);
         }
       }
@@ -290,8 +294,11 @@
       const int64_t pix0 = ((int64_t)img * p.Ho + oy + 2 * half) * p.Wo + ox;
       const int64_t off = pix0 * p.y_cs + n;
       float4 mx[2];
-#pragma unroll
-      for (int r = 0; r < 2; ++r) mx[r] = *(const float4*)(xin + off + r * rowstride);
+      const int64_t xrs = p.mod_up ? 0 : rowstride;
+      const int64_t xoff =
+          p.mod_up ? (((int64_t)img * (p.Ho >> 1) + ((oy + 2 * half) >> 1)) * (p.Wo >> 1) + (ox >> 1)) * p.y_cs + n : off;
+#pragma unroll
+      for (int r = 0; r < 2; ++r) mx[r] = *(const float4*)(xin + xoff + r * xrs);
 #pragma unroll
       for (int r = 0; r < 2; ++r) {
         const csg_f32x2 gl = gl2[r], gh = gh2[r], bl = bl2[r], bh = bh2[r];
@@ -741,7 +748,7 @@
       Wino4Params pe = p;
 #define W4_F(f) pe.f = ka->p.f;
       W4_F(Cout) W4_F(y_cs) W4_F(Ho) W4_F(Wo) W4_F(act) W4_F(slope) W4_F(gate_slope) W4_F(mod) W4_F(g_cs) W4_F(gb_off) W4_F(mod_slope)
-      W4_F(mod_mean) W4_F(mod_invstd)
+      W4_F(mod_mean) W4_F(mod_invstd) W4_F(mod_up)
 #undef W4_F
       w4_epilogue<1>(acc, pe, smem + W4V_V0, tid_o, wave, grp, tid_o & 31, (tid_o >> 5) & 1, nt32, img, X0, Y0, ka->bias,
                      ka->res, ka->gate, ka->y);
@@ -789,6 +796,7 @@
   p.Q8 = (d->Cin + 7) / 8;
   p.act = d->act; p.slope = d->slope; p.gate_slope = 0.f;
   p.nt_off = 0; p.mod = 0; p.g_cs = 0; p.gb_off = 0; p.mod_slope = 1.f; p.mod_mean = nullptr; p.mod_invstd = nullptr;
+  p.mod_up = 0;
   p.nstage = d->Cin / W4_PS;
   p.ksplit = 1;
   p.sps = p.nstage;
@@ -1048,9 +1056,9 @@
                       workspace, y_final, (hipStream_t)stream, "csg_wino4_conv");
 }
 
-int csg_wino4_conv_part(const csg_wino_desc* d, const float* x, const float* packed, int64_t tile_off, int64_t tiles_total,
+static int w4_conv_part(const csg_wino_desc* d, const float* x, const float* packed, int64_t tile_off, int64_t tiles_total,
                         const float* bias, const float* mod_x, const float* mod_gamma, int64_t gamma_cs,
-                        const float* mod_mean, const float* mod_invstd, float mod_slope, float* y, void* stream) {
+                        const float* mod_mean, const float* mod_invstd, float mod_slope, float* y, void* stream, int up) {
   Wino4Params p;
   size_t shm = 0;
   int rc = w4_plan(d, 4, 1, p, shm, "csg_wino4_conv_part");
@@ -1071,12 +1079,28 @@
                     ((uintptr_t)mod_invstd % 16) == 0,
                 CSG_E_UNSUPPORTED, "csg_wino4_conv_part: pointers must be 16-byte aligned");
     p.mod = 1; p.g_cs = (int)gamma_cs; p.mod_slope = mod_slope; p.mod_mean = mod_mean; p.mod_invstd = mod_invstd;
-  }
+    p.mod_up = up;
+  }
+  CSG_REQUIRE(!up || mod_x != nullptr, CSG_E_BADSHAPE, "csg_wino4_conv_part_up2: the source form is the modulation's");
   CSG_REQUIRE(((uintptr_t)x % 16) == 0 && ((uintptr_t)packed % 16) == 0 && ((uintptr_t)y % 16) == 0 &&
                   (bias == nullptr || ((uintptr_t)bias % 16) == 0),
               CSG_E_UNSUPPORTED, "csg_wino4_conv_part: pointers must be 16-byte aligned");
   return w4_launch<4>(p, shm, K_WINO4_CONV, 2.0 * p.B * p.H * p.W * 9.0 * p.Cin * p.Cout, x, packed, bias, mod_x, mod_gamma, y,
                       nullptr, y, (hipStream_t)stream, "csg_wino4_conv_part");
+}
+
+int csg_wino4_conv_part(const csg_wino_desc* d, const float* x, const float* packed, int64_t tile_off, int64_t tiles_total,
+                        const float* bias, const float* mod_x, const float* mod_gamma, int64_t gamma_cs,
+                        const float* mod_mean, const float* mod_invstd, float mod_slope, float* y, void* stream) {
+  return w4_conv_part(d, x, packed, tile_off, tiles_total, bias, mod_x, mod_gamma, gamma_cs, mod_mean, mod_invstd, mod_slope, y,
+                      stream, 0);
+}
+
+int csg_wino4_conv_part_up2(const csg_wino_desc* d, const float* x, const float* packed, int64_t tile_off, int64_t tiles_total,
+                            const float* bias, const float* mod_x, const float* mod_gamma, int64_t gamma_cs,
+                            const float* mod_mean, const float* mod_invstd, float mod_slope, float* y, void* stream) {
+  return w4_conv_part(d, x, packed, tile_off, tiles_total, bias, mod_x, mod_gamma, gamma_cs, mod_mean, mod_invstd, mod_slope, y,
+                      stream, 1);
 }
 
 static int w4_spade_plan(const csg_wino_desc* d, Wino4Params& p, size_t& shm, const char* who) {
@@ -1102,9 +1126,9 @@
   return rc == CSG_OK ? 1 : 0;
 }
 
-int csg_wino4_conv_spade(const csg_wino_desc* d, const float* x, const float* packed, const float* bias, const float* mod_x,
+static int w4_conv_spade(const csg_wino_desc* d, const float* x, const float* packed, const float* bias, const float* mod_x,
                          float* gamma_out, int64_t gamma_cs, const float* mod_mean, const float* mod_invstd, float mod_slope,
-                         float* y, void* stream) {
+                         float* y, void* stream, int up) {
   Wino4Params p;
   size_t shm = 0;
   int rc = w4_spade_plan(d, p, shm, "csg_wino4_conv_spade");
@@ -1121,8 +1145,21 @@
                   ((uintptr_t)mod_x % 16) == 0 && ((uintptr_t)mod_mean % 16) == 0 && ((uintptr_t)mod_invstd % 16) == 0,
               CSG_E_UNSUPPORTED, "csg_wino4_conv_spade: pointers must be 16-byte aligned");
   p.g_cs = (int)gamma_cs; p.mod_slope = mod_slope; p.mod_mean = mod_mean; p.mod_invstd = mod_invstd;
+  p.mod_up = up;
   return w4_launch<4>(p, shm, K_WINO4_CONV, 2.0 * p.B * p.H * p.W * 9.0 * p.Cin * 2.0 * p.Cout, x, packed, bias, mod_x, gamma_out,
                       y, nullptr, y, (hipStream_t)stream, "csg_wino4_conv_spade");
 }
 
-}
+int csg_wino4_conv_spade(const csg_wino_desc* d, const float* x, const float* packed, const float* bias, const float* mod_x,
+                         float* gamma_out, int64_t gamma_cs, const float* mod_mean, const float* mod_invstd, float mod_slope,
+                         float* y, void* stream) {
+  return w4_conv_spade(d, x, packed, bias, mod_x, gamma_out, gamma_cs, mod_mean, mod_invstd, mod_slope, y, stream, 0);
+}
+
+int csg_wino4_conv_spade_up2(const csg_wino_desc* d, const float* x, const float* packed, const float* bias, const float* mod_x,
+                             float* gamma_out, int64_t gamma_cs, const float* mod_mean, const float* mod_invstd,
+                             float mod_slope, float* y, void* stream) {
+  return w4_conv_spade(d, x, packed, bias, mod_x, gamma_out, gamma_cs, mod_mean, mod_invstd, mod_slope, y, stream, 1);
+}
+
+}
diff --git a/canonicalsg2im_amd/ops.py b/canonicalsg2im_amd/ops.py
--- a/canonicalsg2im_amd/ops.py
+++ b/canonicalsg2im_amd/ops.py
@@ -1013,6 +1013,15 @@
 
 
 SPADE_JOINT = os.environ.get("CSG_SPADE_JOINT", "1") != "0"
+UPSAMPLE_FOLD = os.environ.get("CSG_UPSAMPLE_FOLD", "1") != "0"
+
+
+def spade_up2_eligible(B, Hs, Ws, nhidden, C, ks, training, sync=True):
+    if not (UPSAMPLE_FOLD and SPADE_FUSED and WINO_ENABLED and training and ks == 3 and C % 32 == 0):
+        return False
+    if _multi(_sync_world() if sync else 1, sync):
+        return False
+    return lib.csg_wino4_supported(_wino_desc(B, 2 * Hs, 2 * Ws, nhidden, C)) == 1
 
 
 class _SpadeFused(torch.autograd.Function):
@@ -1020,10 +1029,12 @@
     NARG = 7
 
     @staticmethod
-    def forward(ctx, x, eps, momentum, sync, *mods):
+    def forward(ctx, x, eps, momentum, sync, up2, *mods):
         K = len(mods) // _SpadeFused.NARG
         x = nhwc(_f32(x))
         B, C, H, W = x.shape
+        if up2:
+            H, W = 2 * H, 2 * W
         if C % 32 != 0:
             raise RuntimeError("spade_fused: C = %d must be a multiple of 32 (the modulation rides on 32-channel tiles)" % C)
         for k in range(K):
@@ -1035,18 +1046,23 @@
         dev = x.device
         world = _sync_world() if sync else 1
         multi = _multi(world, sync)
+        if up2 and multi:
+            raise RuntimeError("spade_fused: the source form (up2) serves one rank; materialise with upsample2x")
         count = float(P * world)
         mean = torch.empty(C, device=dev, dtype=torch.float32)
         invstd = torch.empty(C, device=dev, dtype=torch.float32)
-        nch = _chunks(P, 1)
+        nch = _chunks(P // 4 if up2 else P, 1)
         part = torch.empty(nch * 2 * C, device=dev, dtype=torch.float64)
         pending = sums = None
         if not multi:
             r0, r1 = (mods[3], mods[4]), ((mods[10], mods[11]) if K == 2 else (None, None))
-            check(lib.csg_norm_stats_finalize(ptr(x), 1, P, C, ptr(part), nch, count, eps, ptr(mean), ptr(invstd), ptr(r0[0]),
-                                              ptr(r0[1] if r0[0] is not None else None), ptr(r1[0]),
-                                              ptr(r1[1] if r1[0] is not None else None), momentum, stream()),
-                  "norm_stats_finalize")
+            rs = (ptr(r0[0]), ptr(r0[1] if r0[0] is not None else None), ptr(r1[0]), ptr(r1[1] if r1[0] is not None else None))
+            if up2:
+                check(lib.csg_norm_stats_finalize_up2(ptr(x), P // 4, C, ptr(part), nch, count, eps, ptr(mean), ptr(invstd),
+                                                      rs[0], rs[1], rs[2], rs[3], momentum, stream()), "norm_stats_finalize_up2")
+            else:
+                check(lib.csg_norm_stats_finalize(ptr(x), 1, P, C, ptr(part), nch, count, eps, ptr(mean), ptr(invstd),
+                                                  rs[0], rs[1], rs[2], rs[3], momentum, stream()), "norm_stats_finalize")
         else:
             sums = torch.empty(2 * C, device=dev, dtype=torch.float64)
             check(lib.csg_norm_stats(ptr(x), 1, P, C, ptr(sums), ptr(part), nch, stream()), "norm_stats")
@@ -1060,21 +1076,23 @@
             up = wino_pack(w, False, None, 4)
             plans.append(plan_conv(B, H, W, nh, 2 * C, 3, 3, 1, 1, has_bias=True,
                                    in_act=(ACT_LEAKY, in_slope) if in_slope is not None else None,
-                                   need=ctx.needs_input_grad[4 + 7 * k:7 + 7 * k]))
+                                   need=ctx.needs_input_grad[5 + 7 * k:8 + 7 * k]))
             pres.append(_take_dx_operand(plans[k], w))
             bd = b.detach().contiguous()
             gbuf = empty_nhwc(B, C, H, W, dev)
             d = _wino_desc(B, H, W, nh, C)
             d.y_cs = C
+            xf = 0.25 * C if up2 else C
             if joint and lib.csg_wino4_conv_spade_supported(d):
-                y = torch.empty_like(x)
-                _wino4_audit("spade_joint", B * H * W, nh + 3 * C, up)
-                check(lib.csg_wino4_conv_spade(d, ptr(actv), ptr(up), ptr(bd), ptr(x), ptr(gbuf), C, ptr(mean), ptr(invstd),
-                                               slope, ptr(y), stream()), "wino4_conv_spade")
+                y = empty_nhwc(B, C, H, W, dev)
+                _wino4_audit("spade_joint", B * H * W, nh + 2 * C + xf, up)
+                conv_spade = lib.csg_wino4_conv_spade_up2 if up2 else lib.csg_wino4_conv_spade
+                check(conv_spade(d, ptr(actv), ptr(up), ptr(bd), ptr(x), ptr(gbuf), C, ptr(mean), ptr(invstd),
+                                 slope, ptr(y), stream()), "wino4_conv_spade")
                 outs[k], groups[k] = y, [actv, w, gbuf, y]
                 continue
             _wino4_audit("spade_gamma", B * H * W, nh + C, up)
-            _wino4_audit("spade_beta", B * H * W, nh + 3 * C, up)
+            _wino4_audit("spade_beta", B * H * W, nh + 2 * C + xf, up)
             check(lib.csg_wino4_conv_part(d, ptr(actv), ptr(up), 0, 2 * C // 32, ptr(bd), None, None, 0, None, None, 1.0,
                                           ptr(gbuf), stream()), "wino4_conv_part(gamma)")
             launches.append((k, actv, w, up, bd, gbuf, nh, slope))
@@ -1085,20 +1103,21 @@
             check(lib.csg_norm_finalize(ptr(sums), 1, C, count, eps, 1, ptr(mean), ptr(invstd), ptr(rm),
                                         ptr(rv if rm is not None else None), momentum, stream()), "norm_finalize")
         for (k, actv, w, up, bd, gbuf, nh, slope) in launches:
-            y = torch.empty_like(x)
+            y = empty_nhwc(B, C, H, W, dev)
             d = _wino_desc(B, H, W, nh, C)
             d.y_cs = C
-            check(lib.csg_wino4_conv_part(d, ptr(actv), ptr(up), C // 32, 2 * C // 32, ptr(bd[C:]), ptr(x), ptr(gbuf), C,
-                                          ptr(mean), ptr(invstd), slope, ptr(y), stream()), "wino4_conv_part(beta)")
+            conv_part = lib.csg_wino4_conv_part_up2 if up2 else lib.csg_wino4_conv_part
+            check(conv_part(d, ptr(actv), ptr(up), C // 32, 2 * C // 32, ptr(bd[C:]), ptr(x), ptr(gbuf), C,
+                            ptr(mean), ptr(invstd), slope, ptr(y), stream()), "wino4_conv_part(beta)")
             outs[k], groups[k] = y, [actv, w, gbuf, y]
         ctx.save_for_backward(x, mean, invstd, *[t for g in groups for t in g])
-        ctx.cfg = (K, P, C, B, H, W, multi, count, eps, tuple(mods[k * 7 + 5] for k in range(K)))
+        ctx.cfg = (K, P, C, B, H, W, multi, count, eps, tuple(mods[k * 7 + 5] for k in range(K)), up2)
         ctx.plans, ctx.ut_pres = plans, pres
         return tuple(outs)
 
     @staticmethod
     def backward(ctx, *dys):
-        K, P, C, B, H, W, multi, count, eps, slopes = ctx.cfg
+        K, P, C, B, H, W, multi, count, eps, slopes, up2 = ctx.cfg
         sv = ctx.saved_tensors
         x, mean, invstd = sv[0], sv[1], sv[2]
         dev = x.device
@@ -1110,27 +1129,37 @@
         for k in range(K):
             actv, w, gbuf, y = sv[3 + 4 * k:7 + 4 * k]
             dgb = empty_nhwc(B, 2 * C, H, W, dev)
-            check(lib.csg_norm_apply_bwd_reduce(ptr(dys[k]), ptr(x), ptr(mean), ptr(invstd), ptr(gbuf), ptr(y), slopes[k], 1, P,
-                                                C, ptr(dgb), ptr(dsums[k]), ptr(part), nch, C, stream()), "norm_bwd_reduce")
+            if up2:
+                check(lib.csg_norm_apply_bwd_reduce_up2(ptr(dys[k]), ptr(x), ptr(mean), ptr(invstd), ptr(gbuf), ptr(y), slopes[k],
+                                                        B, H // 2, W // 2, C, ptr(dgb), ptr(dsums[k]), ptr(part), nch, stream()),
+                      "norm_bwd_reduce_up2")
+            else:
+                check(lib.csg_norm_apply_bwd_reduce(ptr(dys[k]), ptr(x), ptr(mean), ptr(invstd), ptr(gbuf), ptr(y), slopes[k], 1,
+                                                    P, C, ptr(dgb), ptr(dsums[k]), ptr(part), nch, C, stream()), "norm_bwd_reduce")
             dgbs.append(dgb)
         dx, both, pending = None, None, None
         if ctx.needs_input_grad[0]:
             both = dsums[0] + dsums[1] if K == 2 else dsums[0]
             pending = csg_dist.all_reduce_stats_async(_drop_clamped_invstd_term(both, invstd, eps, C)) if multi else None
-        grads = [None, None, None, None]
+        grads = [None, None, None, None, None]
         for k in range(K):
             actv, w, gbuf, y = sv[3 + 4 * k:7 + 4 * k]
-            need = ctx.needs_input_grad[4 + 7 * k:7 + 7 * k]
+            need = ctx.needs_input_grad[5 + 7 * k:8 + 7 * k]
             grads += list(_conv_bwd(ctx.plans[k], dgbs[k], actv, w, None, need, None, ctx.ut_pres[k])) + [None] * 4
         if ctx.needs_input_grad[0]:
             if pending is not None:
                 pending.wait()
             dx = torch.empty_like(x)
             two = K == 2
-            check(lib.csg_norm_apply_bwd_dx(ptr(dys[0]), ptr(x), ptr(mean), ptr(invstd), ptr(sv[5]), slopes[0], ptr(both), count,
-                                            1, P, C, ptr(dx), ptr(dys[1]) if two else None, ptr(sv[9]) if two else None,
-                                            slopes[1] if two else 1.0, ptr(dgbs[0]), ptr(dgbs[1]) if two else None, C, stream()),
-                  "norm_bwd_dx")
+            if up2:
+                check(lib.csg_norm_apply_bwd_dx_up2(ptr(x), ptr(mean), ptr(invstd), ptr(sv[5]), ptr(both), count, B, H // 2,
+                                                    W // 2, C, ptr(dx), ptr(sv[9]) if two else None, ptr(dgbs[0]),
+                                                    ptr(dgbs[1]) if two else None, stream()), "norm_bwd_dx_up2")
+            else:
+                check(lib.csg_norm_apply_bwd_dx(ptr(dys[0]), ptr(x), ptr(mean), ptr(invstd), ptr(sv[5]), slopes[0], ptr(both),
+                                                count, 1, P, C, ptr(dx), ptr(dys[1]) if two else None,
+                                                ptr(sv[9]) if two else None, slopes[1] if two else 1.0, ptr(dgbs[0]),
+                                                ptr(dgbs[1]) if two else None, C, stream()), "norm_bwd_dx")
             grads[0] = dx
         return tuple(grads)
 
@@ -1206,11 +1235,11 @@
                               None if in_slope is None else float(in_slope), float(eps), float(momentum), bool(sync))
 
 
-def spade_fused(x, mods, eps=1e-5, momentum=0.1, sync=True):
+def spade_fused(x, mods, eps=1e-5, momentum=0.1, sync=True, up2=False):
     flat = []
     for (actv, w, b, rm, rv, slope, in_slope) in mods:
         flat += [actv, w, b, rm, rv, float(slope), None if in_slope is None else float(in_slope)]
-    return list(_SpadeFused.apply(x, float(eps), float(momentum), bool(sync), *flat))
+    return list(_SpadeFused.apply(x, float(eps), float(momentum), bool(sync), bool(up2), *flat))
 
 
 def norm_act_pair(x, gb0, gb1, rm0, rv0, rm1, rv1, slope0, slope1, eps=1e-5, momentum=0.1, sync=True):
diff --git a/canonicalsg2im_amd/spade/models/networks/architecture.py b/canonicalsg2im_amd/spade/models/networks/architecture.py
--- a/canonicalsg2im_amd/spade/models/networks/architecture.py
+++ b/canonicalsg2im_amd/spade/models/networks/architecture.py
@@ -27,11 +27,13 @@
         if self.learned_shortcut:
             self.norm_s = SPADE(cfg, fin, opt.semantic_nc)
 
-    def forward(self, x, seg):
+    def forward(self, x, seg, up2=False):
         if self.learned_shortcut:
-            xs, h = spade_pair(self.norm_s, self.norm_0, x, seg, 1.0, 0.2)
+            xs, h = spade_pair(self.norm_s, self.norm_0, x, seg, 1.0, 0.2, up2=up2)
             x_s = self.conv_s(xs)
         else:
+            if up2:
+                x = ops.upsample2x(x)
             x_s, h = x, self.norm_0(x, seg, fused_slope=0.2)
         dx = self.conv_0(h)
         return self.conv_1(self.norm_1(dx, seg, fused_slope=0.2), residual=x_s)
diff --git a/canonicalsg2im_amd/spade/models/networks/generator.py b/canonicalsg2im_amd/spade/models/networks/generator.py
--- a/canonicalsg2im_amd/spade/models/networks/generator.py
+++ b/canonicalsg2im_amd/spade/models/networks/generator.py
@@ -76,7 +76,5 @@
         x = self.fc(seg.at(self.sw))
         no_upsample = {"head_0"} | (set() if self.opt.num_upsampling_layers in ('more', 'most') else {"G_middle_1"})
         for name in self._block_names:
-            if name not in no_upsample:
-                x = ops.upsample2x(x)
-            x = getattr(self, name)(x, seg)
+            x = getattr(self, name)(x, seg, up2=name not in no_upsample)
         return self.conv_img(x, pre_slope=2e-1)
diff --git a/canonicalsg2im_amd/spade/models/networks/normalization.py b/canonicalsg2im_amd/spade/models/networks/normalization.py
--- a/canonicalsg2im_amd/spade/models/networks/normalization.py
+++ b/canonicalsg2im_amd/spade/models/networks/normalization.py
@@ -148,11 +148,20 @@
         _joined(self, "_joined_w", self.mlp_gamma.weight, self.mlp_beta.weight)
         return self.__dict__.get("_joined_w")
 
-    def fused_operands(self, x, segmap, slope):
+    def fusable_up2(self, x):
+        pn = self.param_free_norm
+        wg = self.mlp_gamma.weight
+        return (isinstance(pn, (SynchronizedBatchNorm2d, LocalBatchNorm2d)) and not pn.affine and pn.training
+                and x.dim() == 4 and x.is_cuda
+                and ops.spade_up2_eligible(x.shape[0], x.shape[2], x.shape[3], wg.shape[1], wg.shape[0], wg.shape[2],
+                                           pn.training, getattr(pn, "sync", True)))
+
+    def fused_operands(self, x, segmap, slope, up2=False):
+        size = (2 * x.size(2), 2 * x.size(3)) if up2 else tuple(x.shape[2:])
         if isinstance(segmap, SegPyramid):
-            seg = segmap.at(x.size(2))
+            seg = segmap.at(size[0])
         else:
-            seg = segmap if segmap.shape[2:] == x.shape[2:] else ops.nearest_resize(segmap, x.shape[2:])
+            seg = segmap if tuple(segmap.shape[2:]) == size else ops.nearest_resize(segmap, size)
         sh = self.mlp_shared[0]
         actv = ops.conv2d(seg, sh.weight, sh.bias, 1, sh.padding[0], sh.act, sh.slope, grad_is_pre=True)
         w = _joined(self, "_joined_w", self.mlp_gamma.weight, self.mlp_beta.weight)
@@ -172,11 +181,18 @@
         return ops.conv2d(actv, w, b, 1, self.pw, in_act=(sh.act, sh.slope))
 
 
-def spade_pair(norm_a, norm_b, x, segmap, slope_a, slope_b):
+def spade_pair(norm_a, norm_b, x, segmap, slope_a, slope_b, up2=False):
     pa, pb = norm_a.param_free_norm, norm_b.param_free_norm
     same = (type(pa) is type(pb) and isinstance(pa, (SynchronizedBatchNorm2d, LocalBatchNorm2d)) and not pa.affine
             and not pb.affine and pa.training and pb.training and pa.eps == pb.eps and pa.momentum == pb.momentum
             and getattr(pa, "sync", True) == getattr(pb, "sync", True) and x.dim() == 4)
+    if up2:
+        if same and norm_a.fusable_up2(x) and norm_b.fusable_up2(x):
+            ya, yb = ops.spade_fused(x, [norm_a.fused_operands(x, segmap, slope_a, True),
+                                         norm_b.fused_operands(x, segmap, slope_b, True)],
+                                     pa.eps, pa.momentum, getattr(pa, "sync", True), up2=True)
+            return ya, yb
+        x = ops.upsample2x(x)
     if not same:
         return norm_a(x, segmap, fused_slope=slope_a), norm_b(x, segmap, fused_slope=slope_b)
     if norm_a.fusable(x) and norm_b.fusable(x):
diff --git a/include/csg_hip.h b/include/csg_hip.h
--- a/include/csg_hip.h
+++ b/include/csg_hip.h
@@ -150,6 +150,12 @@
 int csg_wino4_conv_spade(const csg_wino_desc* d, const float* x, const float* packed, const float* bias, const float* mod_x,
                          float* gamma_out, int64_t gamma_cs, const float* mod_mean, const float* mod_invstd, float mod_slope,
                          float* y, void* stream);
+int csg_wino4_conv_part_up2(const csg_wino_desc* d, const float* x, const float* packed, int64_t tile_off, int64_t tiles_total,
+                            const float* bias, const float* mod_x, const float* mod_gamma, int64_t gamma_cs,
+                            const float* mod_mean, const float* mod_invstd, float mod_slope, float* y, void* stream);
+int csg_wino4_conv_spade_up2(const csg_wino_desc* d, const float* x, const float* packed, const float* bias, const float* mod_x,
+                             float* gamma_out, int64_t gamma_cs, const float* mod_mean, const float* mod_invstd,
+                             float mod_slope, float* y, void* stream);
 
 int32_t csg_wino34_supported(const csg_wino_desc* d, int32_t pad);
 int csg_wino34_pack_weights(const float* w, int64_t s_o, int64_t s_i, int64_t s_h, int64_t s_w, int64_t Cout, int64_t Cin,
@@ -213,6 +219,15 @@
                           float slope, const double* dsums, double count, int64_t G, int64_t P, int64_t C, float* dx,
                           const float* dy2, const float* gb2, float slope2, const float* dgb, const float* dgb2,
                           int64_t gb_cs, void* stream);
+int csg_norm_stats_finalize_up2(const float* x, int64_t P, int64_t C, double* partial, int64_t nchunk, double count, float eps,
+                                float* mean, float* invstd, float* running_mean, float* running_var, float* running_mean2,
+                                float* running_var2, float momentum, void* stream);
+int csg_norm_apply_bwd_reduce_up2(const float* dy, const float* x, const float* mean, const float* invstd, const float* gamma,
+                                  const float* yact, float slope, int64_t B, int64_t H, int64_t W, int64_t C, float* dgb,
+                                  double* dsums, double* partial, int64_t nchunk, void* stream);
+int csg_norm_apply_bwd_dx_up2(const float* x, const float* mean, const float* invstd, const float* gamma, const double* dsums,
+                              double count, int64_t B, int64_t H, int64_t W, int64_t C, float* dx, const float* gamma2,
+                              const float* dgb, const float* dgb2, void* stream);
 
 int csg_nearest_resize_fwd(const float* x, int64_t B, int64_t IH, int64_t IW, int64_t C, int64_t OH, int64_t OW, float* y,
                            void* stream);
```

Measured after the change: 219.6 img/s (median of 6 runs). 1.01x the previous value.
